# fixstars/cuda-bundle-adjustment

Hardware: AMD Instinct MI355X
Metric: edges/sec (edge-iterations/s = E x LM iterations / wall, graph resident in HBM, every timed 10-iteration run from its own perturbed start) + 10-iter LM wall-clock (contract_wall: initialize()+optimize(10) after warm-up, C++ API) on KITTI-00-shaped graph; per-iter chi2 vs g2o-faithful oracle (higher is better)
Workload: dtype f64; 1 GPU; ba_kitti00-shaped synthetic stereo graph, 10-iteration LM runs, Huber; poses=1332, landmarks=133383, edges=561116, graphs=1, parallelism=single GPU

## Files before the change

### cuda-bundle-adjustment_amd/csrc/ba_edge.hip

```cpp

#include "ba_device.hpp"

namespace cubahip
{

__device__ __forceinline__ void residual_chi2_body(const DeviceGraph& g, Scalar* parts, Scalar* per_edge, int bid, int nb)
{
	Scalar acc = 0;
	for (int e = g.e_begin + bid * 256 + threadIdx.x; e < g.e_end; e += nb * 256)
	{
		const int pe = g.e_pose[e];
		const bool stereo = (pe & STEREO_BIT) != 0;
		const int ip = pe & ~STEREO_BIT;
		const int il = g.e_lm[e];
		Scalar q[4], t[3], cam[5], Xw[3], meas[3], r[3], Xc[3];
		load_pose(g, ip, q, t, cam);
#pragma unroll
		for (int i = 0; i < 3; i++) Xw[i] = g.Xw[3 * (size_t)il + i];
		meas[0] = g.e_mu[e]; meas[1] = g.e_mv[e]; meas[2] = g.e_mr[e];
		const Scalar ee = g.e_w[e] * edge_residual(q, t, cam, Xw, meas, stereo, r, Xc);
		const int kind = stereo ? g.rk[1].kind : g.rk[0].kind;
		const Scalar delta = stereo ? g.rk[1].delta : g.rk[0].delta;
		acc += robust_rho(kind, delta, ee);
		if (per_edge) per_edge[e] = ee;
	}
	acc = wave_sum(acc);
	__shared__ Scalar part[4];
	if ((threadIdx.x & 63) == 0) part[threadIdx.x >> 6] = acc;
	__syncthreads();
	if (threadIdx.x == 0) parts[bid] = part[0] + part[1] + part[2] + part[3];
}

__global__ __launch_bounds__(256) void residual_chi2_kernel(DeviceGraph g, Scalar* parts, Scalar* per_edge)
{
	residual_chi2_body(g, parts, per_edge, blockIdx.x, gridDim.x);
}

void launch_residual_chi2(const DeviceGraph& g, Scalar* parts, Scalar* slots, Scalar* per_edge, hipStream_t st, const DevicePoseFactors* pf)
{
	const int n = g.e_end - g.e_begin;
	const int grid = n > 0 ? min((n + 255) / 256, 2048) : 0;
	if (grid > 0) hipLaunchKernelGGL(residual_chi2_kernel, dim3(grid), dim3(256), 0, st, g, parts, per_edge);
	const int nPf = pose_factor_chi2_parts(pf);
	if (nPf > 0) launch_pose_factor_chi2(g, *pf, parts + grid, st);
	launch_reduce_parts(parts, grid + nPf, slots, st);
}

__device__ __forceinline__ void edge_hplT_x(const LaneEdge& le, const Scalar* xp, Scalar c[3])
{
	const EdgeLin& L = le.lin;
	Scalar v[3];
#pragma unroll
	for (int m = 0; m < 3; m++)
	{
		Scalar s = 0;
#pragma unroll
		for (int r = 0; r < 6; r++) s += L.JP[m][r] * xp[r];
		v[m] = le.wr * s;
	}
#pragma unroll
	for (int k = 0; k < 3; k++) c[k] = L.JL[0][k] * v[0] + L.JL[1][k] * v[1] + L.JL[2][k] * v[2];
}

__device__ __forceinline__ Scalar finish_landmark(const DeviceSystem& sys, int il, const Scalar csum[3], Scalar lambda)
{
	const Scalar* ls = sys.lm_sys + 9 * (size_t)il;
	Scalar inv[6], bl[3], cl[3], xl[3];
#pragma unroll
	for (int k = 0; k < 6; k++) inv[k] = ls[k];
#pragma unroll
	for (int k = 0; k < 3; k++) { bl[k] = ls[6 + k]; cl[k] = bl[k] - csum[k]; }
	Scalar sc = 0;
#pragma unroll
	for (int i = 0; i < 3; i++)
	{
		xl[i] = inv[sym3_idx(i, 0)] * cl[0] + inv[sym3_idx(i, 1)] * cl[1] + inv[sym3_idx(i, 2)] * cl[2];
		sys.xl[3 * (size_t)il + i] = xl[i];
		sc += xl[i] * (lambda * xl[i] + bl[i]);
	}
	return sc;
}

__global__ __launch_bounds__(LIN_BLOCK) void back_substitute_kernel(DeviceGraph g, DeviceStructure st, DeviceSystem sys, Scalar lambda)
{
	__shared__ Scalar lds_all[(LIN_BLOCK / WAVE) * WAVE * 3];
	const int lane = threadIdx.x & 63;
	const int wv = threadIdx.x >> 6;
	const int wave = blockIdx.x * (LIN_BLOCK / WAVE) + wv;
	if (wave >= st.nWaves) return;
	Scalar* lds = lds_all + wv * WAVE * 3;
	const int lm0 = st.wave_lm[2 * wave], lm1 = st.wave_lm[2 * wave + 1];
	const int e0 = g.lm_ptr[lm0], e1 = g.lm_ptr[lm1];
	const int e = e0 + lane;
	const bool valid = e < e1;
	int il = lm0, seg0 = 0, seg1 = 0;
	Scalar c[3] = { 0, 0, 0 };
	if (valid)
	{
		il = g.e_lm[e];
		if (il < g.Lf)
		{
			seg0 = g.lm_ptr[il] - e0;
			seg1 = g.lm_ptr[il + 1] - e0;
			const int ip = g.e_pose[e] & ~STEREO_BIT;
			if (ip < g.Pf)
			{
				LaneEdge le;
				linearize_edge(g, e, le);
				Scalar xp[6];
#pragma unroll
				for (int r = 0; r < 6; r++) xp[r] = sys.xp[6 * (size_t)ip + r];
				edge_hplT_x(le, xp, c);
			}
		}
	}
	const bool lmFree = valid && il < g.Lf;
#pragma unroll
	for (int k = 0; k < 3; k++) lds[lane * 3 + k] = c[k];
	wave_lds_sync();
	Scalar sc = 0;
	if (lmFree && lane == seg0)
	{
		Scalar cs[3] = { 0, 0, 0 };
		for (int j = seg0; j < seg1; j++)
		{
			cs[0] += lds[j * 3 + 0]; cs[1] += lds[j * 3 + 1]; cs[2] += lds[j * 3 + 2];
		}
		sc = finish_landmark(sys, il, cs, lambda);
	}
	sc = wave_sum(sc);
	if (lane == 0) sys.parts[wave] = sc;
}

__global__ __launch_bounds__(256) void big_back_substitute_kernel(DeviceGraph g, DeviceStructure st, DeviceSystem sys, Scalar lambda)
{
	__shared__ Scalar red[4][3];
	const int il = st.big_lm[blockIdx.x];
	if (il >= g.Lf)
	{
		if (threadIdx.x == 0) sys.parts[st.nWaves + blockIdx.x] = 0;
		return;
	}
	const int e0 = g.lm_ptr[il], e1 = g.lm_ptr[il + 1];
	Scalar acc[3] = { 0, 0, 0 };
	for (int e = e0 + threadIdx.x; e < e1; e += 256)
	{
		const int ip = g.e_pose[e] & ~STEREO_BIT;
		if (ip >= g.Pf) continue;
		LaneEdge le;
		linearize_edge(g, e, le);
		Scalar xp[6], c[3];
#pragma unroll
		for (int r = 0; r < 6; r++) xp[r] = sys.xp[6 * (size_t)ip + r];
		edge_hplT_x(le, xp, c);
		acc[0] += c[0]; acc[1] += c[1]; acc[2] += c[2];
	}
#pragma unroll
	for (int k = 0; k < 3; k++) acc[k] = wave_sum(acc[k]);
	if ((threadIdx.x & 63) == 0)
#pragma unroll
		for (int k = 0; k < 3; k++) red[threadIdx.x >> 6][k] = acc[k];
	__syncthreads();
	if (threadIdx.x == 0)
	{
		Scalar cs[3];
#pragma unroll
		for (int k = 0; k < 3; k++) cs[k] = red[0][k] + red[1][k] + red[2][k] + red[3][k];
		sys.parts[st.nWaves + blockIdx.x] = finish_landmark(sys, il, cs, lambda);
	}
}

static void launch_back_substitute_kernels(const DeviceGraph& g, const DeviceStructure& st, const DeviceSystem& sys, Scalar lambda, hipStream_t s)
{
	if (st.nWaves > 0)
	{
		const int grid = (st.nWaves + (LIN_BLOCK / WAVE) - 1) / (LIN_BLOCK / WAVE);
		hipLaunchKernelGGL(back_substitute_kernel, dim3(grid), dim3(LIN_BLOCK), 0, s, g, st, sys, lambda);
	}
	if (st.nBig > 0)
		hipLaunchKernelGGL(big_back_substitute_kernel, dim3(st.nBig), dim3(256), 0, s, g, st, sys, lambda);
}

void launch_back_substitute(const DeviceGraph& g, const DeviceStructure& st, const DeviceSystem& sys, Scalar lambda, hipStream_t s)
{
	if (g.Lf <= 0) return;
	launch_back_substitute_kernels(g, st, sys, lambda, s);
	launch_reduce_parts(sys.parts, st.nWaves + st.nBig, sys.slots + NSLOT, s);
}

__device__ __forceinline__ void pose_scale_body(const DeviceGraph& g, const DeviceSystem& sys, Scalar lambda, Scalar* parts, int bid, int nb)
{
	Scalar acc = 0;
	for (int i = bid * 256 + threadIdx.x; i < g.Pf * 6; i += nb * 256)
	{
		const Scalar x = sys.xp[i];
		acc += x * (lambda * x + sys.bp[i]);
	}
	acc = wave_sum(acc);
	if ((threadIdx.x & 63) == 0) parts[bid * 4 + (threadIdx.x >> 6)] = acc;
}

__global__ __launch_bounds__(256) void pose_scale_kernel(DeviceGraph g, DeviceSystem sys, Scalar lambda, Scalar* parts)
{
	pose_scale_body(g, sys, lambda, parts, blockIdx.x, gridDim.x);
}

__device__ __forceinline__ void lm_decide(double* st, Scalar* lamOut, double* ring, int ok, double sumLm, double Fhat, double sumPose)
{
#pragma clang fp contract(off)
	const double F = st[0], lam = st[1], nu = st[2];
	const bool halt = st[3] != 0.0;
	const int trial = (int)st[4];
	const double scale = (ok ? sumLm + sumPose : 0.0) + 1e-3;
	const double rho = ok ? (F - Fhat) / scale : -1.0;
	const bool acc = !halt && rho > 0;
	double lamN = lam, nuN = nu, Fn = F, rej = st[6];
	bool haltN = halt;
	if (!halt)
	{
		if (acc)
		{
			const double t = 2 * rho - 1;
			const double a = 1 - t * t * t;
			lamN = lam * fmax(1. / 3, fmin(a, 2. / 3));
			nuN = 2; Fn = Fhat; rej = 0;
		}
		else
		{
			lamN = lam * nu; nuN = nu * 2; rej += 1;
			if (!(rho < 0) && rho <= 0) haltN = true;
			if (rej >= st[7]) haltN = true;
			if (!(rho < 0)) rej = 0;
		}
		if (!(fabs(lamN) <= 1.7e308)) haltN = true;
	}
	double* rec = ring + (size_t)(trial % LM_RING) * LM_REC;
	rec[0] = ok ? Fhat : 0.0; rec[1] = scale; rec[2] = rho; rec[3] = lamN; rec[4] = Fn; rec[5] = acc ? 1.0 : 0.0; rec[6] = haltN ? 1.0 : 0.0; rec[7] = st[8] + (double)(trial + 1);
	st[0] = Fn; st[1] = lamN; st[2] = nuN; st[3] = haltN ? 1.0 : 0.0; st[4] = (double)(trial + 1); st[5] = acc ? 1.0 : 0.0; st[6] = rej;
	lamOut[0] = (Scalar)lamN;
}

__device__ __forceinline__ void reduce_report_body(const DeviceSystem& sys, const Scalar* pA, int nA, Scalar* oA, const Scalar* pB, int nB, Scalar* oB,
	const Scalar* pC, int nC, Scalar* oC, double* lmState, Scalar* lmLam, double* lmRing)
{
	__shared__ Scalar sh[3][16];
	const Scalar vA = wave_sum(parts_thread_sum(pA, nA)), vB = wave_sum(parts_thread_sum(pB, nB)), vC = wave_sum(parts_thread_sum(pC, nC));
	if ((threadIdx.x & 63) == 0) { sh[0][threadIdx.x >> 6] = vA; sh[1][threadIdx.x >> 6] = vB; sh[2][threadIdx.x >> 6] = vC; }
	__syncthreads();
	if (threadIdx.x < 64)
	{
		const bool in = threadIdx.x < 16;
		const Scalar tA = wave_sum(in ? sh[0][threadIdx.x] : Scalar(0)), tB = wave_sum(in ? sh[1][threadIdx.x] : Scalar(0)), tC = wave_sum(in ? sh[2][threadIdx.x] : Scalar(0));
		store_slot_group(oA, tA); store_slot_group(oB, tB); store_slot_group(oC, tC);
		if (lmState && threadIdx.x == 0) lm_decide(lmState, lmLam, lmRing, 1, (double)tA, (double)tB, (double)tC);
	}
	__threadfence_system();
	asm volatile("s_waitcnt vmcnt(0) lgkmcnt(0)" ::: "memory");
	__syncthreads();
	if (threadIdx.x == 0 && sys.host_flags) publish_report(sys);
}


__global__ __launch_bounds__(1024) void reduce_report_kernel(DeviceSystem sys, const Scalar* pA, int nA, Scalar* oA, const Scalar* pB, int nB, Scalar* oB,
	const Scalar* pC, int nC, Scalar* oC, double* lmState, Scalar* lmLam, double* lmRing)
{
	reduce_report_body(sys, pA, nA, oA, pB, nB, oB, pC, nC, oC, lmState, lmLam, lmRing);
}

__global__ __launch_bounds__(1024) void reduce_report_batch_kernel(const BatchEntry* __restrict__ tab)
{
	const BatchEntry& e = tab[blockIdx.x];
	const BatchTrial& t = e.t;
	if (!t.reportOn) return;
	reduce_report_body(e.sys, t.scParts, t.nA, e.sys.slots + NSLOT, t.chiParts, t.nA, e.sys.slots, t.scaleParts, 4 * t.nScale, e.sys.slots + 3 * NSLOT, t.lmState, t.lmLam, t.lmRing);
}

__global__ __launch_bounds__(256) void landmark_scale_kernel(DeviceGraph g, DeviceSystem sys, Scalar lambda, Scalar* parts)
{
	Scalar acc = 0;
	for (int i = blockIdx.x * 256 + threadIdx.x; i < g.Lf * 3; i += gridDim.x * 256)
	{
		const Scalar x = sys.xl[i];
		acc += x * (lambda * x + sys.lm_sys[9 * (size_t)(i / 3) + 6 + (i % 3)]);
	}
	acc = wave_sum(acc);
	if ((threadIdx.x & 63) == 0) parts[blockIdx.x * 4 + (threadIdx.x >> 6)] = acc;
}

void launch_pose_scale(const DeviceGraph& g, const DeviceSystem& sys, Scalar lambda, Scalar* slots, hipStream_t s)
{
	const int grid = g.Pf > 0 ? min((g.Pf * 6 + 255) / 256, 256) : 0;
	if (grid > 0) hipLaunchKernelGGL(pose_scale_kernel, dim3(grid), dim3(256), 0, s, g, sys, lambda, sys.parts);
	launch_reduce_parts(sys.parts, grid * 4, slots, s);
}

void launch_landmark_scale(const DeviceGraph& g, const DeviceSystem& sys, Scalar lambda, Scalar* slots, hipStream_t s)
{
	const int grid = g.Lf > 0 ? min((g.Lf * 3 + 255) / 256, 1024) : 0;
	if (grid > 0) hipLaunchKernelGGL(landmark_scale_kernel, dim3(grid), dim3(256), 0, s, g, sys, lambda, sys.parts);
	launch_reduce_parts(sys.parts, grid * 4, slots, s);
}

__global__ __launch_bounds__(256) void update_state_kernel(DeviceGraph g, DeviceSystem sys, int poseBlocks)
{
	if ((int)blockIdx.x < poseBlocks)
	{
		const int i = blockIdx.x * 256 + threadIdx.x;
		if (i >= g.Pf) return;
		Scalar upd[6], q[4], t[3];
#pragma unroll
		for (int k = 0; k < 6; k++) upd[k] = sys.xp[6 * (size_t)i + k];
#pragma unroll
		for (int k = 0; k < 4; k++) q[k] = g.q[4 * (size_t)i + k];
#pragma unroll
		for (int k = 0; k < 3; k++) t[k] = g.t[3 * (size_t)i + k];
		pose_exp_update(upd, q, t);
#pragma unroll
		for (int k = 0; k < 4; k++) g.q[4 * (size_t)i + k] = q[k];
#pragma unroll
		for (int k = 0; k < 3; k++) g.t[3 * (size_t)i + k] = t[k];
		return;
	}
	const int i = (blockIdx.x - poseBlocks) * 256 + threadIdx.x;
	if (i < g.Lf * 3) g.Xw[i] += sys.xl[i];
}

void launch_update_state(const DeviceGraph& g, const DeviceSystem& sys, hipStream_t s)
{
	const int pb = (g.Pf + 255) / 256, lb = (g.Lf * 3 + 255) / 256;
	if (pb + lb > 0) hipLaunchKernelGGL(update_state_kernel, dim3(pb + lb), dim3(256), 0, s, g, sys, pb);
}

__device__ __forceinline__ Scalar finish_landmark_x(const DeviceSystem& sys, int il, const Scalar csum[3], Scalar lambda, Scalar xl[3])
{
	const Scalar* ls = sys.lm_sys + 9 * (size_t)il;
	Scalar inv[6], bl[3], cl[3];
#pragma unroll
	for (int k = 0; k < 6; k++) inv[k] = ls[k];
#pragma unroll
	for (int k = 0; k < 3; k++) { bl[k] = ls[6 + k]; cl[k] = bl[k] - csum[k]; }
	Scalar sc = 0;
#pragma unroll
	for (int i = 0; i < 3; i++)
	{
		xl[i] = inv[sym3_idx(i, 0)] * cl[0] + inv[sym3_idx(i, 1)] * cl[1] + inv[sym3_idx(i, 2)] * cl[2];
		sys.xl[3 * (size_t)il + i] = xl[i];
		sc += xl[i] * (lambda * xl[i] + bl[i]);
	}
	return sc;
}

__device__ __forceinline__ Scalar updated_edge_rho(const DeviceGraph& g, const Scalar q0[4], const Scalar t0[3], const Scalar cam[5], const Scalar upd[6], bool poseFree,
	const Scalar Xn[3], const Scalar meas[3], Scalar w, bool stereo)
{
	Scalar q[4] = { q0[0], q0[1], q0[2], q0[3] }, t[3] = { t0[0], t0[1], t0[2] }, r[3], Xc[3];
	if (poseFree) pose_exp_update(upd, q, t);
	const Scalar ee = w * edge_residual(q, t, cam, Xn, meas, stereo, r, Xc);
	return robust_rho(stereo ? g.rk[1].kind : g.rk[0].kind, stereo ? g.rk[1].delta : g.rk[0].delta, ee);
}

__device__ __forceinline__ void update_pose_rows(const DeviceGraph& g, const DeviceSystem& sys, const Scalar* __restrict__ old, int i)
{
	Scalar upd[6], q[4], t[3];
#pragma unroll
	for (int k = 0; k < 6; k++) upd[k] = sys.xp[6 * (size_t)i + k];
#pragma unroll
	for (int k = 0; k < 4; k++) q[k] = old[4 * (size_t)i + k];
#pragma unroll
	for (int k = 0; k < 3; k++) t[k] = old[4 * (size_t)g.Pt + 3 * (size_t)i + k];
	pose_exp_update(upd, q, t);
#pragma unroll
	for (int k = 0; k < 4; k++) g.q[4 * (size_t)i + k] = q[k];
#pragma unroll
	for (int k = 0; k < 3; k++) g.t[3 * (size_t)i + k] = t[k];
}

__device__ __forceinline__ void trial_tail_body(const DeviceGraph& g, const DeviceStructure& st, const DeviceSystem& sys, Scalar lambda,
	const Scalar* __restrict__ old, Scalar* __restrict__ scParts, Scalar* __restrict__ chiParts, int nLmGroups, int poseBlocks, Scalar* __restrict__ scaleParts, int nScale)
{
	lambda = launch_lambda(sys, lambda);
	if ((int)blockIdx.x >= nLmGroups)
	{
		const int b = blockIdx.x - nLmGroups;
		if (b < poseBlocks)
		{
			const int i = b * LIN_BLOCK + threadIdx.x;
			if (i < g.Pf) update_pose_rows(g, sys, old, i);
		}
		else pose_scale_body(g, sys, lambda, scaleParts, b - poseBlocks, nScale);
		return;
	}
	__shared__ Scalar lds_all[(LIN_BLOCK / WAVE) * WAVE * 3];
	__shared__ Scalar wpart[2][LIN_BLOCK / WAVE];
	const int lane = threadIdx.x & 63;
	const int wv = threadIdx.x >> 6;
	const int wave = blockIdx.x * (LIN_BLOCK / WAVE) + wv;
	const bool waveOn = wave < st.nWaves;
	Scalar* lds = lds_all + wv * WAVE * 3;
	const Scalar* qo = old; const Scalar* to = old + 4 * (size_t)g.Pt; const Scalar* Xo = old + 7 * (size_t)g.Pt;
	const int lm0 = waveOn ? st.wave_lm[2 * wave] : 0, lm1 = waveOn ? st.wave_lm[2 * wave + 1] : 0;
	const int e0 = waveOn ? g.lm_ptr[lm0] : 0, e1 = waveOn ? g.lm_ptr[lm1] : 0;
	const int e = e0 + lane;
	const bool valid = waveOn && e < e1;
	int il = lm0, ip = 0, seg0 = 0, seg1 = 0;
	bool stereo = false, poseFree = false;
	Scalar q[4] = { 0, 0, 0, 1 }, t[3] = { 0, 0, 0 }, cam[5] = { 1, 1, 0, 0, 0 }, Xw[3] = { 0, 0, 1 }, meas[3] = { 0, 0, 0 }, xp[6] = { 0, 0, 0, 0, 0, 0 }, w = 0;
	Scalar c[3] = { 0, 0, 0 };
	if (valid)
	{
		const int pe = g.e_pose[e];
		stereo = (pe & STEREO_BIT) != 0;
		ip = pe & ~STEREO_BIT;
		il = g.e_lm[e];
		poseFree = ip < g.Pf;
#pragma unroll
		for (int i = 0; i < 4; i++) q[i] = qo[4 * (size_t)ip + i];
#pragma unroll
		for (int i = 0; i < 3; i++) t[i] = to[3 * (size_t)ip + i];
#pragma unroll
		for (int i = 0; i < 5; i++) cam[i] = g.cam[5 * (size_t)ip + i];
#pragma unroll
		for (int i = 0; i < 3; i++) Xw[i] = Xo[3 * (size_t)il + i];
		meas[0] = g.e_mu[e]; meas[1] = g.e_mv[e]; meas[2] = g.e_mr[e];
		w = g.e_w[e];
		if (poseFree)
		{
#pragma unroll
			for (int r = 0; r < 6; r++) xp[r] = sys.xp[6 * (size_t)ip + r];
		}
		if (il < g.Lf)
		{
			seg0 = g.lm_ptr[il] - e0;
			seg1 = g.lm_ptr[il + 1] - e0;
			if (poseFree)
			{
				LaneEdge le;
				Scalar Xc[3];
				const Scalar ss = edge_residual(q, t, cam, Xw, meas, stereo, le.lin.r, Xc);
				le.wr = w * robust_weight(stereo ? g.rk[1].kind : g.rk[0].kind, stereo ? g.rk[1].delta : g.rk[0].delta, w * ss);
				const Rot3 R = quat_to_rot(q[0], q[1], q[2], q[3]);
				edge_jacobians(Xc, R, cam, stereo, le.lin);
				edge_hplT_x(le, xp, c);
			}
		}
	}
	const bool lmFree = valid && il < g.Lf;
#pragma unroll
	for (int k = 0; k < 3; k++) lds[lane * 3 + k] = c[k];
	wave_lds_sync();
	Scalar sc = 0, xl[3] = { 0, 0, 0 };
	if (lmFree && lane == seg0)
	{
		Scalar cs[3] = { 0, 0, 0 };
		for (int j = seg0; j < seg1; j++)
		{
			cs[0] += lds[j * 3 + 0]; cs[1] += lds[j * 3 + 1]; cs[2] += lds[j * 3 + 2];
		}
		sc = finish_landmark_x(sys, il, cs, lambda, xl);
#pragma unroll
		for (int k = 0; k < 3; k++) g.Xw[3 * (size_t)il + k] = Xw[k] + xl[k];
	}
	wave_lds_sync();
	if (lmFree && lane == seg0)
	{
#pragma unroll
		for (int k = 0; k < 3; k++) lds[lane * 3 + k] = xl[k];
	}
	wave_lds_sync();
	Scalar rho = 0;
	if (valid)
	{
		Scalar Xn[3] = { Xw[0], Xw[1], Xw[2] };
		if (lmFree)
		{
#pragma unroll
			for (int k = 0; k < 3; k++) Xn[k] = Xw[k] + lds[seg0 * 3 + k];
		}
		rho = updated_edge_rho(g, q, t, cam, xp, poseFree, Xn, meas, w, stereo);
	}
	sc = wave_sum(sc); rho = wave_sum(rho);
	if (lane == 0) { wpart[0][wv] = sc; wpart[1][wv] = rho; }
	__syncthreads();
	if (threadIdx.x == 0)
	{
		scParts[blockIdx.x] = (wpart[0][0] + wpart[0][1]) + (wpart[0][2] + wpart[0][3]);
		chiParts[blockIdx.x] = (wpart[1][0] + wpart[1][1]) + (wpart[1][2] + wpart[1][3]);
	}
}


__global__ __launch_bounds__(LIN_BLOCK) void trial_tail_kernel(DeviceGraph g, DeviceStructure st, DeviceSystem sys, Scalar lambda,
	const Scalar* __restrict__ old, Scalar* __restrict__ scParts, Scalar* __restrict__ chiParts, int nLmGroups, int poseBlocks, Scalar* __restrict__ scaleParts, int nScale)
{
	trial_tail_body(g, st, sys, lambda, old, scParts, chiParts, nLmGroups, poseBlocks, scaleParts, nScale);
}

__global__ __launch_bounds__(LIN_BLOCK) void trial_tail_batch_kernel(const BatchEntry* __restrict__ tab)
{
	const BatchEntry& e = tab[blockIdx.y];
	const BatchTrial& t = e.t;
	if (blockIdx.x >= t.tailGrid) return;
	trial_tail_body(e.g, e.st, e.sys, Scalar(-1), t.old, t.scParts, t.chiParts, t.nLm, t.poseBlocks, t.scaleParts, t.nScale);
}

__global__ __launch_bounds__(256) void big_trial_tail_kernel(DeviceGraph g, DeviceStructure st, DeviceSystem sys, Scalar lambda,
	const Scalar* __restrict__ old, Scalar* __restrict__ scParts, Scalar* __restrict__ chiParts)
{
	__shared__ Scalar red[4][3];
	__shared__ Scalar xsh[3];
	__shared__ Scalar rsh[4];
	lambda = launch_lambda(sys, lambda);
	DeviceGraph go = g;
	go.q = const_cast<Scalar*>(old); go.t = go.q + 4 * (size_t)g.Pt; go.Xw = go.q + 7 * (size_t)g.Pt;
	const int il = st.big_lm[blockIdx.x];
	const int e0 = g.lm_ptr[il], e1 = g.lm_ptr[il + 1];
	const bool lmFree = il < g.Lf;
	Scalar acc[3] = { 0, 0, 0 };
	if (lmFree)
	{
		for (int e = e0 + threadIdx.x; e < e1; e += 256)
		{
			const int ip = g.e_pose[e] & ~STEREO_BIT;
			if (ip >= g.Pf) continue;
			LaneEdge le;
			linearize_edge(go, e, le);
			Scalar xp[6], c[3];
#pragma unroll
			for (int r = 0; r < 6; r++) xp[r] = sys.xp[6 * (size_t)ip + r];
			edge_hplT_x(le, xp, c);
			acc[0] += c[0]; acc[1] += c[1]; acc[2] += c[2];
		}
	}
#pragma unroll
	for (int k = 0; k < 3; k++) acc[k] = wave_sum(acc[k]);
	if ((threadIdx.x & 63) == 0)
#pragma unroll
		for (int k = 0; k < 3; k++) red[threadIdx.x >> 6][k] = acc[k];
	__syncthreads();
	if (threadIdx.x == 0)
	{
		Scalar xl[3] = { 0, 0, 0 }, sc = 0;
		if (lmFree)
		{
			Scalar cs[3];
#pragma unroll
			for (int k = 0; k < 3; k++) cs[k] = red[0][k] + red[1][k] + red[2][k] + red[3][k];
			sc = finish_landmark_x(sys, il, cs, lambda, xl);
#pragma unroll
			for (int k = 0; k < 3; k++) g.Xw[3 * (size_t)il + k] = go.Xw[3 * (size_t)il + k] + xl[k];
		}
		scParts[blockIdx.x] = sc;
#pragma unroll
		for (int k = 0; k < 3; k++) xsh[k] = xl[k];
	}
	__syncthreads();
	Scalar Xn[3];
#pragma unroll
	for (int k = 0; k < 3; k++) Xn[k] = go.Xw[3 * (size_t)il + k] + xsh[k];
	Scalar rho = 0;
	for (int e = e0 + threadIdx.x; e < e1; e += 256)
	{
		const int pe = g.e_pose[e];
		const bool stereo = (pe & STEREO_BIT) != 0;
		const int ip = pe & ~STEREO_BIT;
		Scalar q[4], t[3], cam[5], meas[3], xp[6];
		load_pose(go, ip, q, t, cam);
		meas[0] = g.e_mu[e]; meas[1] = g.e_mv[e]; meas[2] = g.e_mr[e];
		const bool poseFree = ip < g.Pf;
#pragma unroll
		for (int r = 0; r < 6; r++) xp[r] = poseFree ? sys.xp[6 * (size_t)ip + r] : Scalar(0);
		rho += updated_edge_rho(g, q, t, cam, xp, poseFree, Xn, meas, g.e_w[e], stereo);
	}
	rho = wave_sum(rho);
	if ((threadIdx.x & 63) == 0) rsh[threadIdx.x >> 6] = rho;
	__syncthreads();
	if (threadIdx.x == 0) chiParts[blockIdx.x] = (rsh[0] + rsh[1]) + (rsh[2] + rsh[3]);
}

size_t trial_tail_parts(const DeviceGraph& g, const DeviceStructure& st, int factorParts)
{
	const size_t a = (size_t)(st.nWaves + LIN_BLOCK / WAVE - 1) / (LIN_BLOCK / WAVE) + st.nBig;
	const size_t nA = (a + 63) / 64 * 64;
	return nA + (a + factorParts + 63) / 64 * 64 + 4 * 256 + 64;
}

void launch_trial_tail_fused(const DeviceGraph& g, const DeviceStructure& st, const DeviceSystem& sys, Scalar lambda, const Scalar* old, hipStream_t s,
	const LmDevice* decide, const DevicePoseFactors* pf)
{
	const int nLm = (st.nWaves + LIN_BLOCK / WAVE - 1) / (LIN_BLOCK / WAVE);
	const int nA = nLm + st.nBig;
	const int nPf = pose_factor_chi2_parts(pf);
	Scalar* scParts = sys.parts;
	Scalar* chiParts = sys.parts + (size_t)(nA + 63) / 64 * 64;
	Scalar* scaleParts = chiParts + (size_t)(nA + nPf + 63) / 64 * 64;
	const int poseBlocks = (g.Pf + LIN_BLOCK - 1) / LIN_BLOCK;
	const int nScale = g.Pf > 0 ? min((g.Pf * 6 + 255) / 256, 256) : 0;
	if (nLm + poseBlocks + nScale > 0)
		hipLaunchKernelGGL(trial_tail_kernel, dim3(nLm + poseBlocks + nScale), dim3(LIN_BLOCK), 0, s, g, st, sys, lambda, old, scParts, chiParts, nLm, poseBlocks, scaleParts, nScale);
	if (st.nBig > 0) hipLaunchKernelGGL(big_trial_tail_kernel, dim3(st.nBig), dim3(256), 0, s, g, st, sys, lambda, old, scParts + nLm, chiParts + nLm);
	if (nPf > 0) launch_pose_factor_chi2(g, *pf, chiParts + nA, s);
	hipLaunchKernelGGL(reduce_report_kernel, dim3(1), dim3(1024), 0, s, sys, scParts, nA, sys.slots + NSLOT, chiParts, nA + nPf, sys.slots, scaleParts, 4 * nScale, sys.slots + 3 * NSLOT,
		decide ? decide->state : (double*)nullptr, decide ? decide->lam : (Scalar*)nullptr, decide ? decide->ring : (double*)nullptr);
}

void batch_fill_tail(const DeviceGraph& g, const DeviceStructure& st, const DeviceSystem& sys, const Scalar* old, const LmDevice& lm, Scalar* state, size_t stateCount, BatchTrial& t)
{
	const int nLm = (st.nWaves + LIN_BLOCK / WAVE - 1) / (LIN_BLOCK / WAVE);
	const int nA = nLm + st.nBig;
	t.scParts = sys.parts;
	t.chiParts = sys.parts + (size_t)(nA + 63) / 64 * 64;
	t.scaleParts = t.chiParts + (size_t)(nA + 63) / 64 * 64;
	t.poseBlocks = (g.Pf + LIN_BLOCK - 1) / LIN_BLOCK;
	t.nScale = g.Pf > 0 ? min((g.Pf * 6 + 255) / 256, 256) : 0;
	t.nLm = nLm; t.nA = nA; t.old = old;
	t.tailGrid = (unsigned)(nLm + t.poseBlocks + t.nScale);
	t.lmState = lm.state; t.lmLam = lm.lam; t.lmRing = lm.ring; t.reportOn = 1;
	t.state = state; t.stateCount = stateCount;
	t.restoreGrid = (unsigned)std::min<size_t>(512, (stateCount + 255) / 256);
}

__global__ void lm_decide_failed_kernel(DeviceSystem sys, double* lmState, Scalar* lmLam, double* lmRing)
{
	if (threadIdx.x != 0) return;
	lm_decide(lmState, lmLam, lmRing, 0, 0.0, 0.0, 0.0);
	__threadfence_system();
	if (sys.host_flags) publish_report(sys);
}

void launch_lm_decide_failed(const DeviceSystem& sys, const LmDevice& lm, hipStream_t s)
{
	hipLaunchKernelGGL(lm_decide_failed_kernel, dim3(1), dim3(64), 0, s, sys, lm.state, lm.lam, lm.ring);
}

__global__ __launch_bounds__(256) void restore_if_rejected_batch_kernel(const BatchEntry* __restrict__ tab)
{
	const BatchTrial& t = tab[blockIdx.y].t;
	if (blockIdx.x >= t.restoreGrid || t.lmState[5] != 0.0) return;
	const size_t stride = (size_t)t.restoreGrid * 256;
	const Scalar* __restrict__ backup = t.backupDst;
	Scalar* __restrict__ state = t.state;
	for (size_t i = (size_t)blockIdx.x * 256 + threadIdx.x; i < t.stateCount; i += stride) state[i] = backup[i];
}

__global__ __launch_bounds__(256) void restore_if_rejected_kernel(Scalar* __restrict__ state, const Scalar* __restrict__ backup, size_t count, const double* lmState)
{
	if (lmState[5] != 0.0) return;
	const size_t stride = (size_t)gridDim.x * 256;
	for (size_t i = (size_t)blockIdx.x * 256 + threadIdx.x; i < count; i += stride) state[i] = backup[i];
}

void launch_restore_if_rejected(Scalar* state, const Scalar* backup, size_t count, const LmDevice& lm, hipStream_t s)
{
	const unsigned grid = (unsigned)std::min<size_t>(512, (count + 255) / 256);
	if (grid) hipLaunchKernelGGL(restore_if_rejected_kernel, dim3(grid), dim3(256), 0, s, state, backup, count, lm.state);
}

void launch_batch_tail(const BatchEntry* tab, int n, unsigned tailGridMax, unsigned restoreGridMax, hipStream_t s)
{
	if (tailGridMax) hipLaunchKernelGGL(trial_tail_batch_kernel, dim3(tailGridMax, n), dim3(LIN_BLOCK), 0, s, tab);
	hipLaunchKernelGGL(reduce_report_batch_kernel, dim3(n), dim3(1024), 0, s, tab);
	if (restoreGridMax) hipLaunchKernelGGL(restore_if_rejected_batch_kernel, dim3(restoreGridMax, n), dim3(256), 0, s, tab);
}

}
```

### cuda-bundle-adjustment_amd/csrc/ba_kernels.hpp

```cpp
#pragma once

#include <hip/hip_runtime.h>
#include <cstdint>
#include <vector>

#include "ba_math.hpp"

namespace cubahip
{

constexpr int PCG_SETUP_POSES = 64;
constexpr int NSLOT = 16;
constexpr int WAVE = 64;
constexpr int LIN_BLOCK = 256;
constexpr int STEREO_BIT = 0x40000000;

struct DeviceGraph
{
	int Pt = 0, Pf = 0, Lt = 0, Lf = 0, E = 0;
	int e_begin = 0, e_end = 0;
	Scalar *q = nullptr, *t = nullptr, *cam = nullptr, *Xw = nullptr;
	int *e_pose = nullptr, *e_lm = nullptr;
	Scalar *e_mu = nullptr, *e_mv = nullptr, *e_mr = nullptr, *e_w = nullptr;
	int* lm_ptr = nullptr;
	RobustKernel rk[2] = { { 0, 0 }, { 0, 0 } };
};

constexpr int BP_HEAVY = 64;

struct DeviceStructure
{
	int nWaves = 0;
	int* wave_lm = nullptr;
	int nBig = 0;
	int* big_lm = nullptr;
	int nblk = 0;
	int *hsc_rowptr = nullptr, *hsc_colind = nullptr;
	int *adj_ptr = nullptr, *adj_blk = nullptr, *adj_col = nullptr;
	int2* ell = nullptr;
	int ell_m = 0, ell_over = 0;
	int* hsc_blkrow = nullptr;
	int nOd = 0;
	int nDiagProd = 0;
	int* od_blocks = nullptr;
	int inv_rows8 = 1;
	int nHeavy = 0;
	int *prod_ea = nullptr, *prod_eb = nullptr;
	const int *prod_beg = nullptr, *prod_end = nullptr, *pe_beg = nullptr, *pe_end = nullptr;
	int* prod_lm = nullptr;
	int* pe_edge = nullptr;
	int nCb = 0;
	int *cb_I = nullptr, *cb_J = nullptr, *cb_ptr = nullptr, *cb_blk = nullptr;
	Scalar *cb_wi = nullptr, *cb_wj = nullptr;
	Scalar* e_rec = nullptr;
	int mixed = 0;
};

int spmv_rows_for(int Pf);

struct DeviceSystem
{
	Scalar* hsc = nullptr;
	Scalar* bsc = nullptr;
	Scalar* bp = nullptr;
	Scalar* lm_sys = nullptr;
	Scalar* lm_inv = nullptr;
	Scalar* xp = nullptr;
	Scalar* xl = nullptr;
	Scalar* parts = nullptr;
	Scalar* slots = nullptr;
	unsigned long long* maxdiag = nullptr;
	int* fail = nullptr;
	Scalar *minv = nullptr, *r = nullptr, *z = nullptr, *p0 = nullptr, *p1 = nullptr, *ap = nullptr;
	Scalar *rz = nullptr, *pq = nullptr;
	int rzStride = 0, pqStride = 0;
	int nrz0 = 0, nrz = 0, npq = 0;
	int* done = nullptr;
	int* iters = nullptr;
	int* host_flags = nullptr;
	int* ticket = nullptr;
	int* kbase = nullptr;
	int agg = 0;
	int nc = 0;
	Scalar inv_agg = 0;
	int cl = 1;
	Scalar* acinv = nullptr;
	float* acinv32 = nullptr;
	Scalar* gj_pivots = nullptr;
	Scalar* rc = nullptr;
	Scalar* hrow = nullptr;
	int spmv_rows = 2;
	Scalar* qpart = nullptr;
	Scalar* r2 = nullptr;
	const Scalar* lam_dev = nullptr;
	int upper = 0;
	Scalar* tq = nullptr;
	int* lowpos = nullptr;
};

enum { POSE_FACTOR_KERNEL_NONE = 0, POSE_FACTOR_KERNEL_HUBER = 1, POSE_FACTOR_KERNEL_TUKEY = 2, POSE_FACTOR_KERNEL_CAUCHY = 3 };

struct DevicePriors
{
	int n = 0;
	int nPoses = 0;
	const int* pose_ptr = nullptr;
	const int* pose_id = nullptr;
	const int* pose = nullptr;
	const Scalar *qbar = nullptr, *tbar = nullptr;
	const Scalar* info = nullptr;
	Scalar* chi = nullptr;
	const int* rk_kind = nullptr;
	const Scalar* rk_delta = nullptr;
};

constexpr int REL_REC = 90;
struct DeviceRelPoses
{
	int n = 0;
	int nActive = 0;
	int nBlocks = 0;
	int nPoses = 0;
	const int *pose_i = nullptr, *pose_j = nullptr;
	const int* blk_ptr = nullptr;
	const int* blk_id = nullptr;
	const int* pose_ptr = nullptr;
	const int* pose_id = nullptr;
	const int* pose_item = nullptr;
	const Scalar *q = nullptr, *t = nullptr;
	const Scalar* info = nullptr;
	Scalar* rec = nullptr;
	Scalar* chi = nullptr;
	const int* rk_kind = nullptr;
	const Scalar* rk_delta = nullptr;
};

struct DevicePoseFactors { DevicePriors priors; DeviceRelPoses rel; };
void launch_pose_factor_linearize(const DeviceGraph& g, const DeviceStructure& st, const DeviceSystem& sys, const DevicePoseFactors& pf, int mode, hipStream_t s);
void launch_pose_factor_chi2(const DeviceGraph& g, const DevicePoseFactors& pf, Scalar* parts, hipStream_t s);
int pose_factor_chi2_parts(const DevicePoseFactors* pf);

void launch_residual_chi2(const DeviceGraph& g, Scalar* parts, Scalar* slots, Scalar* per_edge, hipStream_t st, const DevicePoseFactors* pf = nullptr);

struct BlockPassRange { int begin, end, heavy; };
void launch_linearize_dm(const DeviceGraph& g, const DeviceStructure& st, const DeviceSystem& sys, int mode, Scalar lambda, hipStream_t s,
	const Scalar* backupSrc = nullptr, Scalar* backupDst = nullptr, size_t backupCount = 0, const BlockPassRange* range = nullptr);
void launch_block_pass(const DeviceGraph& g, const DeviceStructure& st, const DeviceSystem& sys, const BlockPassRange& range, hipStream_t s);

void launch_pose_maxdiag(const DeviceGraph& g, const DeviceStructure& st, const DeviceSystem& sys, hipStream_t s);

void launch_back_substitute(const DeviceGraph& g, const DeviceStructure& st, const DeviceSystem& sys, Scalar lambda, hipStream_t s);

void launch_pose_scale(const DeviceGraph& g, const DeviceSystem& sys, Scalar lambda, Scalar* slots, hipStream_t s);
struct LmDevice;
void launch_trial_tail_fused(const DeviceGraph& g, const DeviceStructure& st, const DeviceSystem& sys, Scalar lambda, const Scalar* old, hipStream_t s,
	const LmDevice* decide = nullptr, const DevicePoseFactors* pf = nullptr);
size_t trial_tail_parts(const DeviceGraph& g, const DeviceStructure& st, int factorParts = 0);
constexpr int LM_REC = 8, LM_RING = 64;
struct LmDevice { double* state = nullptr; Scalar* lam = nullptr; double* ring = nullptr; };
void launch_lm_decide_failed(const DeviceSystem& sys, const LmDevice& lm, hipStream_t s);
void launch_restore_if_rejected(Scalar* state, const Scalar* backup, size_t count, const LmDevice& lm, hipStream_t s);
void launch_landmark_scale(const DeviceGraph& g, const DeviceSystem& sys, Scalar lambda, Scalar* slots, hipStream_t s);

void launch_update_state(const DeviceGraph& g, const DeviceSystem& sys, hipStream_t s);

void launch_pcg_setup(const DeviceGraph& g, const DeviceStructure& st, const DeviceSystem& sys, Scalar lambda, hipStream_t s);
void launch_pcg_spmv(const DeviceGraph& g, const DeviceStructure& st, const DeviceSystem& sys, int k, int maxIter, Scalar tol2, hipStream_t s);
void launch_pcg_update(const DeviceGraph& g, const DeviceStructure& st, const DeviceSystem& sys, int k, int maxIter, Scalar tol2, hipStream_t s);
Scalar* launch_coarse_setup(const DeviceGraph& g, const DeviceStructure& st, const DeviceSystem& sys, Scalar* work0, Scalar* work1, hipStream_t s, hipEvent_t assembled = nullptr);
Scalar* launch_dense_inverse(Scalar* work0, Scalar* work1, int n, Scalar* pivots, hipStream_t s);
void launch_coarse_finish(const Scalar* swept, Scalar* dst, int n, hipStream_t s);
struct GjJob { Scalar* buf[2]; Scalar* piv[2]; int n, tiles; };
void launch_coarse_assemble(const DeviceGraph& g, const DeviceStructure& st, const DeviceSystem& sys, Scalar* work0, hipStream_t s);
void launch_dense_inverse_batch(const GjJob* jobs, int m, int nMax, hipStream_t s);
void launch_pcg2_fused(const DeviceGraph& g, const DeviceSystem& sys, int k, int kOut, int maxIter, Scalar tol2, int doUpdate, hipStream_t s);
int spmv_upper_grid(int Pf);
int pcg_rows_max_aggregate();
int pcg_rows_entries_per_thread(const DeviceSystem& sys);
void launch_build_lowpos(const DeviceGraph& g, const DeviceStructure& st, int* lowpos, hipStream_t s);
void launch_pcg_upper_iteration(const DeviceGraph& g, const DeviceStructure& st, const DeviceSystem& sys, int k, int maxIter, Scalar tol2, hipStream_t s, int which = 7);
void launch_pcg_advance(const DeviceSystem& sys, int n, hipStream_t s, Scalar tol2 = Scalar(-1));
void launch_coarse_to_fp32(const Scalar* swept, float* dst, int n, hipStream_t s);
void launch_pcg_iteration(const DeviceGraph& g, const DeviceStructure& st, const DeviceSystem& sys, int k, int maxIter, Scalar tol2, hipStream_t s);

struct LmDevice;
struct BatchTrial
{
	unsigned lmGroups = 0, lmGrid = 0; const Scalar* backupSrc = nullptr; Scalar* backupDst = nullptr; size_t backupCount = 0;
	int poseGroups = 0; unsigned schurGrid = 0;
	int nSetup = 0; size_t expandTotal = 0; unsigned nExpand = 0; const Scalar* copySrc = nullptr; Scalar* copyDst = nullptr; size_t copyPairs = 0; unsigned setupGrid = 0;
	int fusedOn = 0;
	const Scalar* old = nullptr; Scalar *scParts = nullptr, *chiParts = nullptr, *scaleParts = nullptr; int nLm = 0, poseBlocks = 0, nScale = 0; unsigned tailGrid = 0; int nA = 0;
	double* lmState = nullptr; Scalar* lmLam = nullptr; double* lmRing = nullptr; int reportOn = 0;
	Scalar* state = nullptr; size_t stateCount = 0; unsigned restoreGrid = 0;
};
struct BatchEntry
{
	DeviceGraph g; DeviceStructure st; DeviceSystem sys;
	int maxIter = 0;
	int gridSpmv = 0;
	BatchTrial t;
};
void batch_fill_linearize(const DeviceGraph& g, const DeviceStructure& st, const Scalar* backupSrc, Scalar* backupDst, size_t backupCount, BatchTrial& t);
void launch_batch_linearize(const BatchEntry* tab, int n, unsigned lmGridMax, unsigned schurGridMax, bool mixed, hipStream_t s);
void batch_fill_setup(const DeviceGraph& g, const DeviceStructure& st, const DeviceSystem& sys, const Scalar* copySrc, Scalar* copyDst, size_t copyCount, BatchTrial& t);
void launch_batch_setup(const BatchEntry* tab, int n, unsigned gridMax, hipStream_t s);
void launch_batch_first_precond(const BatchEntry* tab, int n, const DeviceSystem& sys0, int ncMax, size_t ldsMax, Scalar tol2, hipStream_t s);
void batch_fill_tail(const DeviceGraph& g, const DeviceStructure& st, const DeviceSystem& sys, const Scalar* old, const LmDevice& lm, Scalar* state, size_t stateCount, BatchTrial& t);
void launch_batch_tail(const BatchEntry* tab, int n, unsigned tailGridMax, unsigned restoreGridMax, hipStream_t s);
int batch_kernel_class(const DeviceGraph& g, const DeviceSystem& sys);
size_t batch_pcg2_lds_bytes(const DeviceSystem& sys);
void launch_pcg_batch_iteration(const BatchEntry* tab, int n, const DeviceGraph& g0, const DeviceSystem& sys0, int gridSpmvMax, int ncMax, size_t ldsMax, int k, Scalar tol2, hipStream_t s);
void launch_pcg_batch_advance(const BatchEntry* tab, int n, int iters, hipStream_t s, Scalar tol2);

hipError_t graph_add_pcg_chunk(hipGraph_t graph, const DeviceGraph& g, const DeviceStructure& st, const DeviceSystem& sys, int chunk, int maxIter, Scalar tol2, int report);

void launch_hsc_expand(const DeviceGraph& g, const DeviceStructure& st, const DeviceSystem& sys, hipStream_t s);
void launch_pcg_setup_expand(const DeviceGraph& g, const DeviceStructure& st, const DeviceSystem& sys, Scalar lambda, hipStream_t s,
	const Scalar* copySrc = nullptr, Scalar* copyDst = nullptr, size_t copyCount = 0);

constexpr int SC_T = 32;
constexpr int SC_TP = 5;
constexpr int SC_TT = SC_T * SC_T;

struct SparseCholPlan
{
	int Pf = 0, T = 0, nTiles = 0, nLevels = 0, slack = 0;
	std::vector<int> posOfSeg, segOfPos;
	std::vector<int> colPtr;
	std::vector<int> rowIdx, colOfTile;
	std::vector<int> gPtr;
	std::vector<int> gather;
	std::vector<int> wgRec;
	std::vector<int> lvlPtr, lvlTiles;
	std::vector<int> lvlColPtr, lvlCols;
	std::vector<int> blkTile;
	long long entries = 0;
	size_t tileBytes() const { return sizeof(Scalar) * (size_t)SC_TT * ((size_t)2 * nTiles + 1); }
	double secondsEstimate() const;
};
bool sparse_chol_plan(int Pf, const int* rowptr, const int* colind, int slack, size_t maxTiles, SparseCholPlan& out);

struct SparseChol
{
	Scalar* tiles = nullptr;
	Scalar* tilesT = nullptr;
	Scalar* y = nullptr;
	Scalar* rinv = nullptr;
	const int *colPtr = nullptr, *rowIdx = nullptr, *colOfTile = nullptr, *gPtr = nullptr, *gather = nullptr;
	const int *wgRec = nullptr, *lvlCols = nullptr, *blkTile = nullptr, *posOfSeg = nullptr;
	int* fail = nullptr;
	int T = 0, Pf = 0, nTiles = 0;
};
void launch_sparse_chol_fill(const DeviceStructure& st, const DeviceSystem& sys, const SparseChol& d, hipStream_t s);
void launch_sparse_chol_solve(const SparseChol& d, const SparseCholPlan& plan, Scalar* x, hipStream_t s);
void launch_sparse_chol_factor(const SparseChol& d, const SparseCholPlan& plan, hipStream_t s);

struct SelInvPlan
{
	int nLevels = 0;
	std::vector<int> stepPtr;
	std::vector<int> offRec;
	std::vector<int> colStepPtr, cols;
	std::vector<int> gather;
	long long products = 0;
	size_t sigmaBytes() const;
	int nTiles = 0;
};
bool selinv_plan(const SparseCholPlan& p, SelInvPlan& out);

struct SelInv
{
	Scalar* sigma = nullptr;
	const int *offRec = nullptr, *gather = nullptr, *cols = nullptr;
};
void launch_selinv(const SparseChol& d, const SparseCholPlan& plan, const SelInvPlan& sp, const SelInv& v, hipStream_t s);
void launch_selinv_extract(const DeviceStructure& st, const SparseChol& d, const SelInv& v, Scalar* pose_cov, Scalar* blk_cov, int Pf, hipStream_t s);
void launch_landmark_covariance(const DeviceGraph& g, const DeviceStructure& st, const DeviceSystem& sys, const SparseChol& d, const SelInv& v,
	Scalar* w_scratch, Scalar* lm_cov, hipStream_t s);

void launch_diag_inverse(const SparseChol& d, hipStream_t s);
void launch_edge_w(const DeviceGraph& g, Scalar* W, hipStream_t s);

struct PairRequest
{
	int nBlocks = 0;
	std::vector<int> rhsPtr, rhsPos;
	std::vector<int> leftPtr, leftPos;
	std::vector<int> poseRec;
	std::vector<int> lmRec;
	std::vector<int> pairRec;
};
void pair_pack(const SparseCholPlan& p, int n, const int* kindA, const int* idxA, const int* kindB, const int* idxB,
	const std::vector<int>& lmPtr, const std::vector<int>& ePose, PairRequest& rq);
struct PairPlan
{
	int b0 = 0, b1 = 0, nLevels = 0, T = 0;
	std::vector<int> fwdPtr, fwdCols;
	std::vector<int> bwdPtr, bwdCols;
	std::vector<int> slotPtr, slotCols;
	std::vector<int> slotOf;
	std::vector<int> fLvlPtr, fRec;
	std::vector<int> fGather;
	std::vector<int> bLvlPtr, bRec;
	std::vector<int> bGather;
	size_t slots() const { return slotCols.size(); }
};
size_t pair_block_slots(const SparseCholPlan& p, const PairRequest& rq, int b);
bool pair_plan(const SparseCholPlan& p, const PairRequest& rq, int b0, int b1, PairPlan& out);
struct PairDev
{
	Scalar* X = nullptr;
	const int *fRec = nullptr, *fGather = nullptr, *bRec = nullptr, *bGather = nullptr, *slotOf = nullptr, *rhsPos = nullptr;
	int T = 0;
};

void launch_collect_eval(const DeviceSystem& sys, Scalar* out3, hipStream_t s);

void launch_pcg_report(const DeviceSystem& sys, hipStream_t s);

}
```

### cuda-bundle-adjustment_amd/csrc/ba_linearize.hip

```cpp

#include "ba_device.hpp"

namespace cubahip
{

constexpr int REC = 8;

__device__ __forceinline__ double tag_encode(int tag, double) { return __longlong_as_double((long long)tag); }
__device__ __forceinline__ float tag_encode(int tag, float) { return __int_as_float(tag); }
__device__ __forceinline__ int tag_decode(double v) { return (int)__double_as_longlong(v); }
__device__ __forceinline__ int tag_decode(float v) { return __float_as_int(v); }
__device__ __forceinline__ bool sign_flag(double v) { return __double_as_longlong(v) < 0; }
__device__ __forceinline__ bool sign_flag(float v) { return __float_as_int(v) < 0; }
__device__ __forceinline__ double abs_value(double v) { return __builtin_fabs(v); }
__device__ __forceinline__ float abs_value(float v) { return __builtin_fabsf(v); }

template <typename ET>
__device__ __forceinline__ void write_record(Scalar* base, size_t e, const Scalar Xc[3], Scalar wr, const Scalar r[3], int il, bool stereo)
{
	ET* rec = reinterpret_cast<ET*>(base) + REC * e;
	const ET w = (ET)wr;
	rec[0] = (ET)Xc[0]; rec[1] = (ET)Xc[1]; rec[2] = (ET)Xc[2]; rec[3] = stereo ? -w : w;
	rec[4] = (ET)r[0]; rec[5] = (ET)r[1]; rec[6] = (ET)r[2];
	rec[7] = tag_encode(il, ET());
}

template <typename ET>
__device__ __forceinline__ void load_pose_as(const DeviceGraph& g, int ip, ET q[4], ET cam[5])
{
#pragma unroll
	for (int i = 0; i < 4; i++) q[i] = (ET)g.q[4 * (size_t)ip + i];
#pragma unroll
	for (int i = 0; i < 5; i++) cam[i] = (ET)g.cam[5 * (size_t)ip + i];
}

template <int MODE, typename ET>
__device__ __forceinline__ void lm_pass_body(const DeviceGraph& g, const DeviceStructure& st, const DeviceSystem& sys, Scalar lambda,
	unsigned nLmGroups, const Scalar* __restrict__ backupSrc, Scalar* __restrict__ backupDst, size_t backupCount, unsigned gridX)
{
	__shared__ Scalar lds_all[(LIN_BLOCK / WAVE) * WAVE * 9];
	if (blockIdx.x >= nLmGroups)
	{
		const size_t stride = (size_t)(gridX - nLmGroups) * LIN_BLOCK;
		for (size_t i = (size_t)(blockIdx.x - nLmGroups) * LIN_BLOCK + threadIdx.x; i < backupCount; i += stride) backupDst[i] = backupSrc[i];
		return;
	}
	lambda = launch_lambda(sys, lambda);
	const int lane = threadIdx.x & 63;
	const int wv = threadIdx.x >> 6;
	const int wave = blockIdx.x * (LIN_BLOCK / WAVE) + wv;
	if (wave >= st.nWaves) return;
	Scalar* lds = lds_all + wv * WAVE * 9;
	const int lm0 = st.wave_lm[2 * wave], lm1 = st.wave_lm[2 * wave + 1];
	const int e0 = g.lm_ptr[lm0], e1 = g.lm_ptr[lm1];
	const int e = e0 + lane;
	const bool valid = e < e1;
	int il = lm0, seg0 = 0, seg1 = 0;
	Scalar h[9] = { 0, 0, 0, 0, 0, 0, 0, 0, 0 };
	if (valid)
	{
		const int pe = g.e_pose[e];
		const bool stereo = (pe & STEREO_BIT) != 0;
		const int ip = pe & ~STEREO_BIT;
		il = g.e_lm[e];
		Scalar q[4], t[3], cam[5], Xw[3], meas[3], Xc[3];
		EdgeLin L;
		load_pose(g, ip, q, t, cam);
#pragma unroll
		for (int i = 0; i < 3; i++) Xw[i] = g.Xw[3 * (size_t)il + i];
		meas[0] = g.e_mu[e]; meas[1] = g.e_mv[e]; meas[2] = g.e_mr[e];
		const Scalar w = g.e_w[e];
		const Scalar ss = edge_residual(q, t, cam, Xw, meas, stereo, L.r, Xc);
		const int kind = stereo ? g.rk[1].kind : g.rk[0].kind;
		const Scalar delta = stereo ? g.rk[1].delta : g.rk[0].delta;
		const Scalar wr = w * robust_weight(kind, delta, w * ss);
		write_record<ET>(st.e_rec, (size_t)e, Xc, wr, L.r, il, stereo);
		if (il < g.Lf)
		{
			const Rot3 R = quat_to_rot(q[0], q[1], q[2], q[3]);
			edge_jacobians(Xc, R, cam, stereo, L);
#pragma unroll
			for (int i = 0; i < 3; i++)
			{
#pragma unroll
				for (int j = i; j < 3; j++)
					h[sym3_idx(i, j)] = wr * (L.JL[0][i] * L.JL[0][j] + L.JL[1][i] * L.JL[1][j] + L.JL[2][i] * L.JL[2][j]);
				h[6 + i] = wr * (L.JL[0][i] * L.r[0] + L.JL[1][i] * L.r[1] + L.JL[2][i] * L.r[2]);
			}
			seg0 = g.lm_ptr[il] - e0;
			seg1 = g.lm_ptr[il + 1] - e0;
		}
	}
#pragma unroll
	for (int k = 0; k < 9; k++) lds[lane * 9 + k] = h[k];
	wave_lds_sync();
	const bool head = valid && il < g.Lf && lane == seg0;
	Scalar m = 0;
	if (head)
	{
		Scalar H[9] = { 0, 0, 0, 0, 0, 0, 0, 0, 0 };
		for (int j = seg0; j < seg1; j++)
#pragma unroll
			for (int k = 0; k < 9; k++) H[k] += lds[j * 9 + k];
		Scalar* ls = sys.lm_sys + 9 * (size_t)il;
		if (MODE == 0)
		{
#pragma unroll
			for (int k = 0; k < 9; k++) ls[k] = H[k];
			m = fmax(H[0], fmax(H[3], H[5]));
		}
		else
		{
			Scalar inv[6];
			H[0] += lambda; H[3] += lambda; H[5] += lambda;
			sym3_inverse(H, inv);
#pragma unroll
			for (int k = 0; k < 6; k++) ls[k] = inv[k];
			if (st.inv_rows8)
			{
				Scalar* li = sys.lm_inv + 8 * (size_t)il;
#pragma unroll
				for (int k = 0; k < 6; k++) li[k] = inv[k];
				li[6] = 0; li[7] = 0;
			}
#pragma unroll
			for (int k = 0; k < 3; k++) ls[6 + k] = H[6 + k];
		}
	}
	if (MODE == 0)
	{
		m = wave_max(m);
		if (lane == 0) atomic_max_nonneg(sys.maxdiag + (wave & 63), m);
	}
}


template <int MODE, typename ET>
__global__ __launch_bounds__(LIN_BLOCK) void lm_pass_kernel(DeviceGraph g, DeviceStructure st, DeviceSystem sys, Scalar lambda,
	unsigned nLmGroups, const Scalar* __restrict__ backupSrc, Scalar* __restrict__ backupDst, size_t backupCount)
{
	lm_pass_body<MODE, ET>(g, st, sys, lambda, nLmGroups, backupSrc, backupDst, backupCount, gridDim.x);
}

template <typename ET>
__global__ __launch_bounds__(LIN_BLOCK) void lm_pass_batch_kernel(const BatchEntry* __restrict__ tab)
{
	const BatchEntry& e = tab[blockIdx.y];
	if (blockIdx.x >= e.t.lmGrid) return;
	lm_pass_body<1, ET>(e.g, e.st, e.sys, Scalar(-1), e.t.lmGroups, e.t.backupSrc, e.t.backupDst, e.t.backupCount, e.t.lmGrid);
}

template <int MODE, typename ET>
__global__ __launch_bounds__(256) void big_lm_pass_kernel(DeviceGraph g, DeviceStructure st, DeviceSystem sys, Scalar lambda)
{
	__shared__ Scalar red[4][9];
	lambda = launch_lambda(sys, lambda);
	const int il = st.big_lm[blockIdx.x];
	const int e0 = g.lm_ptr[il], e1 = g.lm_ptr[il + 1];
	Scalar acc[9] = { 0, 0, 0, 0, 0, 0, 0, 0, 0 };
	for (int e = e0 + threadIdx.x; e < e1; e += 256)
	{
		LaneEdge le;
		linearize_edge(g, e, le);
		Scalar q[4], t[3], cam[5], Xw[3], Xc[3];
		load_pose(g, le.ip, q, t, cam);
#pragma unroll
		for (int i = 0; i < 3; i++) Xw[i] = g.Xw[3 * (size_t)il + i];
		quat_rotate(q, Xw, Xc);
		Xc[0] += t[0]; Xc[1] += t[1]; Xc[2] += t[2];
		write_record<ET>(st.e_rec, (size_t)e, Xc, le.wr, le.lin.r, il, le.stereo);
		if (il < g.Lf)
		{
			const EdgeLin& L = le.lin;
#pragma unroll
			for (int i = 0; i < 3; i++)
			{
#pragma unroll
				for (int j = i; j < 3; j++)
					acc[sym3_idx(i, j)] += le.wr * (L.JL[0][i] * L.JL[0][j] + L.JL[1][i] * L.JL[1][j] + L.JL[2][i] * L.JL[2][j]);
				acc[6 + i] += le.wr * (L.JL[0][i] * L.r[0] + L.JL[1][i] * L.r[1] + L.JL[2][i] * L.r[2]);
			}
		}
	}
#pragma unroll
	for (int k = 0; k < 9; k++) acc[k] = wave_sum(acc[k]);
	if ((threadIdx.x & 63) == 0)
#pragma unroll
		for (int k = 0; k < 9; k++) red[threadIdx.x >> 6][k] = acc[k];
	__syncthreads();
	if (threadIdx.x == 0 && il < g.Lf)
	{
		Scalar H[9];
#pragma unroll
		for (int k = 0; k < 9; k++) H[k] = red[0][k] + red[1][k] + red[2][k] + red[3][k];
		Scalar* ls = sys.lm_sys + 9 * (size_t)il;
		if (MODE == 0)
		{
#pragma unroll
			for (int k = 0; k < 9; k++) ls[k] = H[k];
			atomic_max_nonneg(sys.maxdiag, fmax(H[0], fmax(H[3], H[5])));
		}
		else
		{
			Scalar inv[6];
			H[0] += lambda; H[3] += lambda; H[5] += lambda;
			sym3_inverse(H, inv);
#pragma unroll
			for (int k = 0; k < 6; k++) ls[k] = inv[k];
			if (st.inv_rows8)
			{
				Scalar* li = sys.lm_inv + 8 * (size_t)il;
#pragma unroll
				for (int k = 0; k < 6; k++) li[k] = inv[k];
				li[6] = 0; li[7] = 0;
			}
#pragma unroll
			for (int k = 0; k < 3; k++) ls[6 + k] = H[6 + k];
		}
	}
}

template <typename ET>
struct CameraFrameEdge { ET X[3]; ET k00, k02, k11, k12, k22; ET d00, d02, d11, d12, d22; ET w; bool stereo; };

template <typename ET>
__device__ __forceinline__ void camera_frame_edge(const ET* rec, const ET cam[5], CameraFrameEdge<ET>& c)
{
	const ET X = rec[0], Y = rec[1], Z = rec[2], ws = rec[3];
	c.stereo = sign_flag(ws);
	c.w = abs_value(ws);
	c.X[0] = X; c.X[1] = Y; c.X[2] = Z;
	const ET invZ = 1 / Z, invZZ = invZ * invZ;
	c.d00 = -cam[0] * invZ; c.d02 = cam[0] * X * invZZ; c.d11 = -cam[1] * invZ; c.d12 = cam[1] * Y * invZZ;
	c.d22 = c.stereo ? c.d02 - cam[4] * invZZ : ET(0);
	c.k00 = c.w * (c.stereo ? 2 * c.d00 * c.d00 : c.d00 * c.d00);
	c.k02 = c.w * (c.d00 * c.d02 + (c.stereo ? c.d00 * c.d22 : ET(0)));
	c.k11 = c.w * c.d11 * c.d11; c.k12 = c.w * c.d11 * c.d12;
	c.k22 = c.w * (c.d02 * c.d02 + c.d12 * c.d12 + c.d22 * c.d22);
}

template <typename ET>
__device__ __forceinline__ void camera_frame_m(const CameraFrameEdge<ET>& c, const Rot3T<ET>& R, ET (&M)[3][3])
{
#pragma unroll
	for (int j = 0; j < 3; j++)
	{
		M[0][j] = c.k00 * R.m[0][j] + c.k02 * R.m[2][j];
		M[1][j] = c.k11 * R.m[1][j] + c.k12 * R.m[2][j];
		M[2][j] = c.k02 * R.m[0][j] + c.k12 * R.m[1][j] + c.k22 * R.m[2][j];
	}
}

template <int MODE, typename ET>
__device__ __forceinline__ void pose_pass_body(const DeviceGraph& g, const DeviceStructure& st, const DeviceSystem& sys, int bid)
{
	const int lane = threadIdx.x & 63;
	const int ip = bid * 4 + (threadIdx.x >> 6);
	if (ip >= g.Pf) return;
	ET q[4], cam[5];
	load_pose_as<ET>(g, ip, q, cam);
	const Rot3T<ET> R = quat_to_rot(q[0], q[1], q[2], q[3]);
	Scalar acc[33];
#pragma unroll
	for (int k = 0; k < 33; k++) acc[k] = 0;
	const int p1 = st.pe_end[ip];
	for (int p = st.pe_beg[ip] + lane; p < p1; p += 64)
	{
		const ET* rec = reinterpret_cast<const ET*>(st.e_rec) + REC * (size_t)st.pe_edge[p];
		CameraFrameEdge<ET> c;
		camera_frame_edge<ET>(rec, cam, c);
		const ET r0 = rec[4], r1 = rec[5], r2 = c.stereo ? rec[6] : ET(0);
		const int il = tag_decode(rec[7]);
		ET S[6] = { c.k00, 0, c.k02, c.k11, c.k12, c.k22 };
		ET v[3] = { c.w * c.d00 * (r0 + r2), c.w * c.d11 * r1, c.w * (c.d02 * r0 + c.d12 * r1 + c.d22 * r2) };
		ET vs[3] = { v[0], v[1], v[2] };
		if (MODE == 1 && il < g.Lf)
		{
			const Scalar* ls = sys.lm_sys + 9 * (size_t)il;
			ET M[3][3], P[3][3], inv[6], bl[3];
#pragma unroll
			for (int k = 0; k < 6; k++) inv[k] = (ET)ls[k];
#pragma unroll
			for (int k = 0; k < 3; k++) bl[k] = (ET)ls[6 + k];
			camera_frame_m<ET>(c, R, M);
#pragma unroll
			for (int i = 0; i < 3; i++)
#pragma unroll
				for (int k = 0; k < 3; k++)
					P[i][k] = M[i][0] * inv[sym3_idx(0, k)] + M[i][1] * inv[sym3_idx(1, k)] + M[i][2] * inv[sym3_idx(2, k)];
#pragma unroll
			for (int i = 0; i < 3; i++)
			{
#pragma unroll
				for (int j = i; j < 3; j++)
					S[sym3_idx(i, j)] -= P[i][0] * M[j][0] + P[i][1] * M[j][1] + P[i][2] * M[j][2];
				vs[i] -= P[i][0] * bl[0] + P[i][1] * bl[1] + P[i][2] * bl[2];
			}
		}
		const ET X = c.X[0], Y = c.X[1], Z = c.X[2];
		ET U[3][3];
#pragma unroll
		for (int j = 0; j < 3; j++)
		{
			const ET s0 = S[sym3_idx(0, j)], s1 = S[sym3_idx(1, j)], s2 = S[sym3_idx(2, j)];
			U[0][j] = Y * s2 - Z * s1;
			U[1][j] = Z * s0 - X * s2;
			U[2][j] = X * s1 - Y * s0;
		}
#pragma unroll
		for (int i = 0; i < 3; i++)
		{
			const ET t[3] = { Y * U[i][2] - Z * U[i][1], Z * U[i][0] - X * U[i][2], X * U[i][1] - Y * U[i][0] };
#pragma unroll
			for (int j = i; j < 3; j++) acc[j * (j + 1) / 2 + i] += (Scalar)t[j];
#pragma unroll
			for (int j = 0; j < 3; j++) acc[(3 + j) * (4 + j) / 2 + i] += (Scalar)U[i][j];
#pragma unroll
			for (int j = i; j < 3; j++) acc[(3 + j) * (4 + j) / 2 + 3 + i] += (Scalar)S[sym3_idx(i, j)];
		}
		acc[21] += (Scalar)(Y * v[2] - Z * v[1]); acc[22] += (Scalar)(Z * v[0] - X * v[2]); acc[23] += (Scalar)(X * v[1] - Y * v[0]);
		acc[24] += (Scalar)v[0]; acc[25] += (Scalar)v[1]; acc[26] += (Scalar)v[2];
		if (MODE == 1)
		{
			acc[27] += (Scalar)(Y * vs[2] - Z * vs[1]); acc[28] += (Scalar)(Z * vs[0] - X * vs[2]); acc[29] += (Scalar)(X * vs[1] - Y * vs[0]);
			acc[30] += (Scalar)vs[0]; acc[31] += (Scalar)vs[1]; acc[32] += (Scalar)vs[2];
		}
	}
#pragma unroll
	for (int k = 0; k < 33; k++) acc[k] = wave_sum(acc[k]);
	if (lane == 0)
	{
		Scalar* blk = sys.hsc + 36 * (size_t)st.hsc_rowptr[ip];
#pragma unroll
		for (int c = 0; c < 6; c++)
		{
#pragma unroll
			for (int r = 0; r <= c; r++) blk[c * 6 + r] = acc[c * (c + 1) / 2 + r];
			sys.bp[6 * (size_t)ip + c] = acc[21 + c];
			if (MODE == 1) sys.bsc[6 * (size_t)ip + c] = acc[27 + c];
		}
	}
}

constexpr int BP_GROUP = 16;

template <int MODE, typename ET>
__global__ __launch_bounds__(256) void pose_pass_kernel(DeviceGraph g, DeviceStructure st, DeviceSystem sys)
{
	pose_pass_body<MODE, ET>(g, st, sys, blockIdx.x);
}

template <typename ET>
struct ProductOperand { ET X[3]; ET M[3][3]; };

template <typename ET>
__device__ __forceinline__ void product_operand(const ET* rec, const Rot3T<ET>& R, const ET cam[5], ProductOperand<ET>& o)
{
	CameraFrameEdge<ET> c;
	camera_frame_edge<ET>(rec, cam, c);
	o.X[0] = c.X[0]; o.X[1] = c.X[1]; o.X[2] = c.X[2];
	camera_frame_m<ET>(c, R, o.M);
}

template <typename ET>
__device__ __forceinline__ void product_accumulate(const ProductOperand<ET>& A, const ProductOperand<ET>& B, const ET inv[6], ET (&T)[6][6])
{
	ET P[3][3], W[3][6];
#pragma unroll
	for (int i = 0; i < 3; i++)
#pragma unroll
		for (int k = 0; k < 3; k++)
			P[i][k] = A.M[i][0] * inv[sym3_idx(0, k)] + A.M[i][1] * inv[sym3_idx(1, k)] + A.M[i][2] * inv[sym3_idx(2, k)];
#pragma unroll
	for (int i = 0; i < 3; i++)
	{
#pragma unroll
		for (int j = 0; j < 3; j++) W[i][3 + j] = P[i][0] * B.M[j][0] + P[i][1] * B.M[j][1] + P[i][2] * B.M[j][2];
		W[i][0] = B.X[1] * W[i][5] - B.X[2] * W[i][4];
		W[i][1] = B.X[2] * W[i][3] - B.X[0] * W[i][5];
		W[i][2] = B.X[0] * W[i][4] - B.X[1] * W[i][3];
	}
#pragma unroll
	for (int c = 0; c < 6; c++)
	{
		T[0][c] += A.X[1] * W[2][c] - A.X[2] * W[1][c];
		T[1][c] += A.X[2] * W[0][c] - A.X[0] * W[2][c];
		T[2][c] += A.X[0] * W[1][c] - A.X[1] * W[0][c];
		T[3][c] += W[0][c]; T[4][c] += W[1][c]; T[5][c] += W[2][c];
	}
}

template <typename ET, int GROUP>
__device__ __forceinline__ void block_pass_group(const DeviceGraph& g, const DeviceStructure& st, const DeviceSystem& sys, int grp, int gl)
{
	const int blk0 = grp >= 0 ? st.od_blocks[grp] : -1;
	const bool on = blk0 >= 0;
	const int blk = on ? blk0 : 0;
	const int a = on ? st.hsc_blkrow[blk] : 0, b = on ? st.hsc_colind[blk] : 0;
	ET qa[4], cama[5], qb[4], camb[5];
	load_pose_as<ET>(g, a, qa, cama);
	load_pose_as<ET>(g, b, qb, camb);
	const Rot3T<ET> Ra = quat_to_rot(qa[0], qa[1], qa[2], qa[3]);
	const Rot3T<ET> Rb = quat_to_rot(qb[0], qb[1], qb[2], qb[3]);
	ET T[6][6];
#pragma unroll
	for (int r = 0; r < 6; r++)
#pragma unroll
		for (int c = 0; c < 6; c++) T[r][c] = 0;
	const ET* recs = reinterpret_cast<const ET*>(st.e_rec);
	const int p1 = on ? st.prod_end[blk] : 0;
	for (int p = (on ? st.prod_beg[blk] : 0) + gl; p < p1; p += GROUP)
	{
		const ET* ra = recs + REC * (size_t)st.prod_ea[p];
		const ET* rb = recs + REC * (size_t)st.prod_eb[p];
		const Scalar* li = st.inv_rows8 ? sys.lm_inv + 8 * (size_t)st.prod_lm[p] : sys.lm_sys + 9 * (size_t)st.prod_lm[p];
		ET inv[6];
#pragma unroll
		for (int k = 0; k < 6; k++) inv[k] = (ET)li[k];
		ProductOperand<ET> A, B;
		product_operand<ET>(ra, Ra, cama, A);
		product_operand<ET>(rb, Rb, camb, B);
		product_accumulate<ET>(A, B, inv, T);
	}
	Scalar Ts[6][6];
#pragma unroll
	for (int r = 0; r < 6; r++)
#pragma unroll
		for (int c = 0; c < 6; c++)
		{
			Scalar v = (Scalar)T[r][c];
			if (GROUP == 64) v = wave_sum(v);
			else { v += __shfl_xor(v, 1); v += __shfl_xor(v, 2); v += __shfl_xor(v, 4); v += __shfl_xor(v, 8); }
			Ts[r][c] = v;
		}
	if (!on) return;
	Scalar* dst = sys.hsc + 36 * (size_t)blk;
	if (a != b)
	{
#pragma unroll
		for (int c = 0; c < 6; c++)
#pragma unroll
			for (int r = 0; r < 6; r++)
				if (GROUP == 64 ? (c * 6 + r) == gl : (c * 6 + r) % GROUP == gl) dst[c * 6 + r] = -Ts[r][c];
	}
	else if (gl == 0)
	{
#pragma unroll
		for (int c = 0; c < 6; c++)
#pragma unroll
			for (int r = 0; r <= c; r++) dst[c * 6 + r] -= Ts[r][c] + Ts[c][r];
	}
}

__host__ __device__ __forceinline__ int block_pass_heavy_groups(int nHeavy) { return (nHeavy + 3) / 4; }
__host__ __device__ __forceinline__ int block_pass_groups(int nOd, int nHeavy) { return block_pass_heavy_groups(nHeavy) + ((nOd - nHeavy) * BP_GROUP + 255) / 256; }

template <typename ET>
__device__ __forceinline__ void block_pass_body(const DeviceGraph& g, const DeviceStructure& st, const DeviceSystem& sys, int bid)
{
	const int nh = block_pass_heavy_groups(st.nHeavy);
	if (bid < nh)
	{
		const int grp = bid * 4 + (threadIdx.x >> 6);
		block_pass_group<ET, 64>(g, st, sys, grp < st.nHeavy ? grp : -1, threadIdx.x & 63);
	}
	else
	{
		const int grp = st.nHeavy + ((bid - nh) * 256 + threadIdx.x) / BP_GROUP;
		block_pass_group<ET, BP_GROUP>(g, st, sys, grp < st.nOd ? grp : -1, threadIdx.x & (BP_GROUP - 1));
	}
}

template <typename ET>
__global__ __launch_bounds__(256) void block_pass_kernel(DeviceGraph g, DeviceStructure st, DeviceSystem sys)
{
	block_pass_body<ET>(g, st, sys, blockIdx.x);
}

template <typename ET>
__global__ __launch_bounds__(256) void schur_pass_kernel(DeviceGraph g, DeviceStructure st, DeviceSystem sys, int nPoseGroups)
{
	if ((int)blockIdx.x < nPoseGroups) pose_pass_body<1, ET>(g, st, sys, blockIdx.x);
	else block_pass_body<ET>(g, st, sys, blockIdx.x - nPoseGroups);
}

template <typename ET>
__global__ __launch_bounds__(256) void schur_pass_batch_kernel(const BatchEntry* __restrict__ tab)
{
	const BatchEntry& e = tab[blockIdx.y];
	if (blockIdx.x >= e.t.schurGrid) return;
	if ((int)blockIdx.x < e.t.poseGroups) pose_pass_body<1, ET>(e.g, e.st, e.sys, blockIdx.x);
	else block_pass_body<ET>(e.g, e.st, e.sys, blockIdx.x - e.t.poseGroups);
}

static DeviceStructure block_pass_view(const DeviceStructure& st, const BlockPassRange& r)
{
	DeviceStructure v = st;
	v.od_blocks = st.od_blocks + r.begin; v.nOd = r.end - r.begin; v.nHeavy = r.heavy;
	return v;
}

template <typename ET>
static void launch_linearize_dm_t(const DeviceGraph& g, const DeviceStructure& stAll, const DeviceSystem& sys, int mode, Scalar lambda, hipStream_t s,
	const Scalar* backupSrc, Scalar* backupDst, size_t backupCount, const BlockPassRange* range)
{
	const DeviceStructure st = range ? block_pass_view(stAll, *range) : stAll;
	if (st.nWaves > 0)
	{
		const unsigned grid = (st.nWaves + (LIN_BLOCK / WAVE) - 1) / (LIN_BLOCK / WAVE);
		const unsigned nCopy = backupSrc ? (unsigned)std::min<size_t>(512, (backupCount + LIN_BLOCK - 1) / LIN_BLOCK) : 0;
		if (mode == 0) hipLaunchKernelGGL((lm_pass_kernel<0, ET>), dim3(grid + nCopy), dim3(LIN_BLOCK), 0, s, g, st, sys, lambda, grid, backupSrc, backupDst, backupCount);
		else hipLaunchKernelGGL((lm_pass_kernel<1, ET>), dim3(grid + nCopy), dim3(LIN_BLOCK), 0, s, g, st, sys, lambda, grid, backupSrc, backupDst, backupCount);
	}
	else if (backupSrc && backupCount)
		(void)hipMemcpyAsync(backupDst, backupSrc, backupCount * sizeof(Scalar), hipMemcpyDeviceToDevice, s);
	if (st.nBig > 0)
	{
		if (mode == 0) hipLaunchKernelGGL((big_lm_pass_kernel<0, ET>), dim3(st.nBig), dim3(256), 0, s, g, st, sys, lambda);
		else hipLaunchKernelGGL((big_lm_pass_kernel<1, ET>), dim3(st.nBig), dim3(256), 0, s, g, st, sys, lambda);
	}
	const int nbp = block_pass_groups(st.nOd, st.nHeavy);
	if (mode == 1 && g.Pf > 0 && st.nOd > 0 && st.nDiagProd == 0)
	{
		const int np = (g.Pf + 3) / 4;
		hipLaunchKernelGGL((schur_pass_kernel<ET>), dim3(np + nbp), dim3(256), 0, s, g, st, sys, np);
		return;
	}
	if (g.Pf > 0)
	{
		if (mode == 0) hipLaunchKernelGGL((pose_pass_kernel<0, ET>), dim3((g.Pf + 3) / 4), dim3(256), 0, s, g, st, sys);
		else hipLaunchKernelGGL((pose_pass_kernel<1, ET>), dim3((g.Pf + 3) / 4), dim3(256), 0, s, g, st, sys);
	}
	if (mode == 1 && st.nOd > 0)
		hipLaunchKernelGGL((block_pass_kernel<ET>), dim3(nbp), dim3(256), 0, s, g, st, sys);
}

void launch_linearize_dm(const DeviceGraph& g, const DeviceStructure& st, const DeviceSystem& sys, int mode, Scalar lambda, hipStream_t s,
	const Scalar* backupSrc, Scalar* backupDst, size_t backupCount, const BlockPassRange* range)
{
	if (st.mixed && sizeof(Scalar) == 8) launch_linearize_dm_t<float>(g, st, sys, mode, lambda, s, backupSrc, backupDst, backupCount, range);
	else launch_linearize_dm_t<Scalar>(g, st, sys, mode, lambda, s, backupSrc, backupDst, backupCount, range);
}

void batch_fill_linearize(const DeviceGraph& g, const DeviceStructure& st, const Scalar* backupSrc, Scalar* backupDst, size_t backupCount, BatchTrial& t)
{
	t.lmGroups = (st.nWaves + (LIN_BLOCK / WAVE) - 1) / (LIN_BLOCK / WAVE);
	const unsigned nCopy = backupSrc ? (unsigned)std::min<size_t>(512, (backupCount + LIN_BLOCK - 1) / LIN_BLOCK) : 0;
	t.lmGrid = t.lmGroups + nCopy;
	t.backupSrc = backupSrc; t.backupDst = backupDst; t.backupCount = backupCount;
	t.poseGroups = (g.Pf + 3) / 4;
	t.schurGrid = (unsigned)(t.poseGroups + block_pass_groups(st.nOd, st.nHeavy));
}

void launch_batch_linearize(const BatchEntry* tab, int n, unsigned lmGridMax, unsigned schurGridMax, bool mixed, hipStream_t s)
{
	if (mixed && sizeof(Scalar) == 8)
	{
		hipLaunchKernelGGL((lm_pass_batch_kernel<float>), dim3(lmGridMax, n), dim3(LIN_BLOCK), 0, s, tab);
		hipLaunchKernelGGL((schur_pass_batch_kernel<float>), dim3(schurGridMax, n), dim3(256), 0, s, tab);
	}
	else
	{
		hipLaunchKernelGGL((lm_pass_batch_kernel<Scalar>), dim3(lmGridMax, n), dim3(LIN_BLOCK), 0, s, tab);
		hipLaunchKernelGGL((schur_pass_batch_kernel<Scalar>), dim3(schurGridMax, n), dim3(256), 0, s, tab);
	}
}

void launch_block_pass(const DeviceGraph& g, const DeviceStructure& stAll, const DeviceSystem& sys, const BlockPassRange& range, hipStream_t s)
{
	if (range.end <= range.begin) return;
	const DeviceStructure st = block_pass_view(stAll, range);
	const int nbp = block_pass_groups(st.nOd, st.nHeavy);
	if (st.mixed && sizeof(Scalar) == 8) hipLaunchKernelGGL((block_pass_kernel<float>), dim3(nbp), dim3(256), 0, s, g, st, sys);
	else hipLaunchKernelGGL((block_pass_kernel<Scalar>), dim3(nbp), dim3(256), 0, s, g, st, sys);
}

__global__ __launch_bounds__(256) void pose_maxdiag_kernel(DeviceGraph g, DeviceStructure st, DeviceSystem sys)
{
	const int i = blockIdx.x * 256 + threadIdx.x;
	Scalar m = 0;
	if (i < g.Pf * 6)
	{
		const int p = i / 6, k = i % 6;
		m = sys.hsc[36 * (size_t)st.hsc_rowptr[p] + k * 7];
	}
	m = wave_max(m);
	if ((threadIdx.x & 63) == 0) atomic_max_nonneg(sys.maxdiag, m);
}

void launch_pose_maxdiag(const DeviceGraph& g, const DeviceStructure& st, const DeviceSystem& sys, hipStream_t s)
{
	if (g.Pf <= 0) return;
	hipLaunchKernelGGL(pose_maxdiag_kernel, dim3((g.Pf * 6 + 255) / 256), dim3(256), 0, s, g, st, sys);
}

}
```

### cuda-bundle-adjustment_amd/csrc/ba_lm.hip

```cpp
#include "ba_solver.hpp"

using namespace cubahip;

void cuba_hip_solver::graphWorker()
{
	(void)hipSetDevice(device);
	std::unique_lock<std::mutex> lk(gb.m);
	for (;;)
	{
		gb.cv.wait(lk, [&] { return gb.stop || !gb.jobs.empty() || !gb.trash.empty(); });
		if (gb.stop) return;
		if (gb.jobs.empty())
		{
			std::vector<hipGraphExec_t> t; t.swap(gb.trash);
			gb.busy = true;
			lk.unlock();
			for (hipGraphExec_t e : t) (void)hipGraphExecDestroy(e);
			lk.lock();
			gb.busy = false;
			gb.cv.notify_all();
			continue;
		}
		GraphJob j = gb.jobs.front(); gb.jobs.pop_front();
		gb.busy = true;
		lk.unlock();
		const auto t0 = Clock::now();
		hipGraph_t graph = nullptr; hipGraphExec_t exec = nullptr;
		bool ok = hipGraphCreate(&graph, 0) == hipSuccess && graph_add_pcg_chunk(graph, j.g, j.st, j.sys, j.chunk, j.maxIter, j.tol2, 1) == hipSuccess &&
			hipGraphInstantiate(&exec, graph, nullptr, nullptr, 0) == hipSuccess;
		if (graph) (void)hipGraphDestroy(graph);
		if (!ok) (void)hipGetLastError();
		const double dt = std::chrono::duration<double>(Clock::now() - t0).count();
		lk.lock();
		gb.busy = false;
		if (ok && j.gen == gb.gen) { gb.ready[std::make_pair(j.chunk, j.acinv)] = exec; gb.builds++; gb.seconds.store(gb.seconds.load() + dt); }
		else if (exec) (void)hipGraphExecDestroy(exec);
		gb.cv.notify_all();
	}
}

hipGraphExec_t cuba_hip_solver::pcgGraphIfReady(int chunk, int maxIter, Scalar tol2)
{
	if (pcgGraphTol2 != tol2 || pcgGraphMaxIter != maxIter) { dropPcgGraph(); pcgGraphTol2 = tol2; pcgGraphMaxIter = maxIter; }
	const auto key = std::make_pair(chunk, (const Scalar*)sys.acinv);
	auto it = pcgGraphs.find(key);
	if (it != pcgGraphs.end()) return it->second;
	std::lock_guard<std::mutex> lk(gb.m);
	for (auto& kv : gb.ready) pcgGraphs[kv.first] = kv.second;
	gb.ready.clear();
	it = pcgGraphs.find(key);
	if (it != pcgGraphs.end()) return it->second;
	if (!gb.requested.count(key))
	{
		gb.requested[key] = 1;
		gb.jobs.push_back(GraphJob{ chunk, (const Scalar*)sys.acinv, g, st, sys, maxIter, tol2, gb.gen });
		if (!gb.th.joinable()) gb.th = std::thread([this] { graphWorker(); });
		gb.cv.notify_all();
	}
	return nullptr;
}

void cuba_hip_solver::dropPcgGraph()
{
	{
		std::lock_guard<std::mutex> lk(gb.m);
		gb.gen++;
		gb.jobs.clear(); gb.requested.clear();
		const bool offload = gb.th.joinable() && !gb.stop;
		for (auto& kv : gb.ready) { if (offload) gb.trash.push_back(kv.second); else (void)hipGraphExecDestroy(kv.second); }
		gb.ready.clear();
		for (auto& kv : pcgGraphs) { if (offload) gb.trash.push_back(kv.second); else (void)hipGraphExecDestroy(kv.second); }
		if (offload && !gb.trash.empty()) gb.cv.notify_all();
	}
	pcgGraphs.clear();
	batchRequests.clear();
	graphsOrderedFor = nullptr;
}

void cuba_hip_solver::ensureOverlapObjects()
{
	if (gjStream) return;
	int prioLow = 0, prioHigh = 0;
	HIP_TRY(hipDeviceGetStreamPriorityRange(&prioLow, &prioHigh));
	HIP_TRY(hipStreamCreateWithPriority(&gjStream, hipStreamNonBlocking, prioLow));
	HIP_TRY(hipEventCreateWithFlags(&evSetup, hipEventDisableTiming));
	HIP_TRY(hipEventCreateWithFlags(&evAssembled, hipEventDisableTiming));
	HIP_TRY(hipEventCreateWithFlags(&evInverse, hipEventDisableTiming));
	HIP_TRY(hipEventCreateWithFlags(&evFirstInv, hipEventDisableTiming));
	HIP_TRY(hipEventRecord(evFirstInv, gjStream));
}

void cuba_hip_solver::waitReport()
{
	volatile int* flags = (volatile int*)((char*)h_pinned + 1024);
	{
		const auto t0 = Clock::now();
		for (long spins = 0; flags[3] != expectedTicket; spins++)
			if ((spins & 0xfff) == 0xfff && std::chrono::duration<double>(Clock::now() - t0).count() > 2.0) break;
		if (flags[3] == expectedTicket)
		{
			std::atomic_thread_fence(std::memory_order_acquire);
			return;
		}
	}
	sync();
	std::atomic_thread_fence(std::memory_order_acquire);
	expectedTicket = flags[3];
}

void cuba_hip_solver::downloadAsDouble(const Scalar* dsrc, double* hdst, size_t n)
{
	if (!n) return;
	if (sizeof(Scalar) == sizeof(double))
	{
		HIP_TRY(hipMemcpyAsync(hdst, dsrc, n * sizeof(double), hipMemcpyDeviceToHost, stream));
		sync();
		return;
	}
	std::vector<Scalar> tmp(n);
	HIP_TRY(hipMemcpyAsync(tmp.data(), dsrc, n * sizeof(Scalar), hipMemcpyDeviceToHost, stream));
	sync();
	for (size_t i = 0; i < n; i++) hdst[i] = (double)tmp[i];
}

void cuba_hip_solver::uploadFromDouble(Scalar* ddst, const double* hsrc, size_t n)
{
	if (!n) return;
	std::vector<Scalar> tmp(hsrc, hsrc + n);
	HIP_TRY(hipMemcpyAsync(ddst, tmp.data(), n * sizeof(Scalar), hipMemcpyHostToDevice, stream));
	sync();
}

double cuba_hip_solver::computeErrors()
{
	need();
	StageTimer tm(this, 2);
	launch_residual_chi2(g, d_parts.data(), slotsDev, nullptr, stream, poseFactors());
	return readSlots(0);
}

void cuba_hip_solver::linearize(int mode, double lam, bool withBackup)
{
	waitAssembled();
	const bool parts = mode == 1 && !redParts.empty();
	launch_linearize_dm(g, st, sys, mode, lam, stream, withBackup ? d_state.data() : nullptr, d_backup.data(), d_state.size(), parts ? &redParts[0].od : nullptr);
	if (parts && !partsByCaller)
		for (size_t c = 1; c < redParts.size(); c++) launch_block_pass(g, st, sys, redParts[c].od, stream);
	if (poseFactors()) launch_pose_factor_linearize(g, st, sys, pf, mode, stream);
}

void cuba_hip_solver::schurPart(int part, size_t ranges[4])
{
	need();
	if (part < 0 || part >= schurParts()) throw ArgError{ "cuba_hip_schur_part: no such part" };
	if (part == 0)
	{
		StageTimer tm(this, 4);
		zeroReduced();
		partsByCaller = true;
		try { linearize(1, lambda, false); } catch (...) { partsByCaller = false; throw; }
		partsByCaller = false;
	}
	else
	{
		StageTimer tm(this, 4);
		launch_block_pass(g, st, sys, redParts[part].od, stream);
	}
	const size_t nblk = (size_t)st.nblk;
	ranges[0] = redParts.empty() ? 0 : 36 * redParts[part].blkBegin;
	ranges[1] = redParts.empty() ? 36 * nblk : 36 * (redParts[part].blkEnd - redParts[part].blkBegin);
	ranges[2] = part == 0 ? 36 * nblk : 0;
	ranges[3] = part == 0 ? d_red.size() - 36 * nblk : 0;
}

void cuba_hip_solver::assemble()
{
	need();
	StageTimer tm(this, 3);
	zeroReduced(true);
	d_maxdiag.zero(stream);
	linearize(0, 0.0);
}

void cuba_hip_solver::maxDiagonalParts(double* posePart, double* lmPart)
{
	need();
	const double* hD = (const double*)hostStage();
	HIP_TRY(hipMemcpyAsync(hostStage(), d_maxdiag.data(), 8 * 64, hipMemcpyDeviceToHost, stream));
	sync();
	double v = 0;
	for (int i = 0; i < 64; i++) v = std::max(v, hD[i]);
	*lmPart = v;
	d_maxdiag.zero(stream);
	launch_pose_maxdiag(g, st, sys, stream);
	HIP_TRY(hipMemcpyAsync(hostStage(), d_maxdiag.data(), 8 * 64, hipMemcpyDeviceToHost, stream));
	sync();
	v = 0;
	for (int i = 0; i < 64; i++) v = std::max(v, hD[i]);
	*posePart = v;
}

void cuba_hip_solver::scaleParts(double lam, double* posePart, double* lmPart)
{
	need();
	launch_pose_scale(g, sys, lam, slotsDev + 3 * NSLOT, stream);
	launch_landmark_scale(g, sys, lam, slotsDev + 2 * NSLOT, stream);
	sync();
	double a = 0, b = 0;
	for (int i = 0; i < NSLOT; i++) { b += slot(2 * NSLOT + i); a += slot(3 * NSLOT + i); }
	*posePart = a; *lmPart = b;
}

double cuba_hip_solver::maxDiagonal()
{
	need();
	StageTimer tm(this, 3);
	zeroReduced(true);
	d_maxdiag.zero(stream);
	linearize(0, 0.0);
	launch_pose_maxdiag(g, st, sys, stream);
	HIP_TRY(hipMemcpyAsync(hostStage(), d_maxdiag.data(), 8 * 64, hipMemcpyDeviceToHost, stream));
	sync();
	double v = 0;
	for (int i = 0; i < 64; i++) v = std::max(v, ((const double*)hostStage())[i]);
	return v;
}

void cuba_hip_solver::schur(bool withBackup)
{
	need();
	StageTimer tm(this, 4);
	zeroReduced();
	linearize(1, lambda, withBackup);
}

bool cuba_hip_solver::solveReduced() { return retryWithFp64Inverse(solveReducedOnce()); }

bool cuba_hip_solver::retryWithFp64Inverse(bool ok)
{
	if (ok || !lastSolveBrokeDown || lastFailCode != 2 || !fp32Inverse() || sys.agg <= 0) return ok;
	precondFp32 = false; sys.acinv32 = nullptr;
	dropPcgGraph();
	coarseValid = false; firstInvValid = false; firstInvPending = false;
	cntFp32Fallbacks++;
	if (std::getenv("CUBA_HIP_DEBUG")) std::fprintf(stderr, "[cuba_hip] PCG broke down with the fp32-stored coarse inverse: repeating the solve with fp64 storage\n");
	const int64_t directBefore = cntDirect;
	const bool ok2 = solveReducedOnce();
	if (!ok2 || cntDirect != directBefore)
	{
		precondFp32 = true; sys.acinv32 = d_coarse32[0].data();
		dropPcgGraph();
		coarseValid = false; firstInvValid = false; firstInvPending = false;
	}
	return ok2;
}

int cuba_hip_solver::pcgBudget(int maxIter) const
{
	const int it = directAfter > 0 ? directAfter : std::min(384, std::max(128, Pf / 4));
	return std::min(maxIter, std::max(4, it / 4 * 4));
}

bool cuba_hip_solver::ensureDirectPlan()
{
	if (directPlanValid) return !directRefused;
	const auto t0 = Clock::now();
	ensureHostPattern();
	if (!sparse_chol_plan(Pf, h_rowptr.data(), h_colind.data(), directSlack, (size_t)std::max(1, directMaxTiles), directPlan))
	{
		directPlanValid = true; directRefused = true;
		char buf[200];
		std::snprintf(buf, sizeof buf, "exact reduced solve unavailable: the factor of the %d-pose reduced matrix needs more than direct_max_tiles = %d tiles", Pf, directMaxTiles);
		lastError = buf;
		return false;
	}
	const SparseCholPlan& p = directPlan;
	{
		size_t freeB = 0, totalB = 0;
		const size_t have = sizeof(Scalar) * (d_scTiles.size() + d_scTilesT.size());
		if (hipMemGetInfo(&freeB, &totalB) == hipSuccess && p.tileBytes() > have && p.tileBytes() - have > freeB)
		{
			directPlanValid = true; directRefused = true;
			char buf[200];
			std::snprintf(buf, sizeof buf, "exact reduced solve unavailable: the factor of the %d-pose reduced matrix needs %.1f MB, %.1f MB of device memory are free",
				Pf, p.tileBytes() / 1e6, freeB / 1e6);
			lastError = buf;
			return false;
		}
		(void)hipGetLastError();
	}
	std::vector<int> ints;
	auto put = [&](const std::vector<int>& v) { const size_t o = ints.size(); ints.insert(ints.end(), v.begin(), v.end()); while (ints.size() % 4) ints.push_back(0); return o; };
	const size_t oColPtr = put(p.colPtr), oRowIdx = put(p.rowIdx), oColOf = put(p.colOfTile), oGPtr = put(p.gPtr), oGather = put(p.gather),
		oWgRec = put(p.wgRec), oLvlCols = put(p.lvlCols), oBlkTile = put(p.blkTile), oPos = put(p.posOfSeg);
	d_scInts.upload(ints, stream);
	d_scTiles.resize((size_t)SC_TT * ((size_t)p.nTiles + 1)); d_scTilesT.resize((size_t)SC_TT * std::max(1, p.nTiles));
	d_scY.resize((size_t)SC_T * p.T); d_scRinv.resize((size_t)SC_T * p.T); d_scFail.resize(1);
	sync();
	SparseChol& d = directDev;
	d.tiles = d_scTiles.data(); d.tilesT = d_scTilesT.data(); d.y = d_scY.data(); d.rinv = d_scRinv.data(); d.fail = d_scFail.data();
	const int* base = d_scInts.data();
	d.colPtr = base + oColPtr; d.rowIdx = base + oRowIdx; d.colOfTile = base + oColOf; d.gPtr = base + oGPtr; d.gather = base + oGather;
	d.wgRec = base + oWgRec; d.lvlCols = base + oLvlCols; d.blkTile = base + oBlkTile; d.posOfSeg = base + oPos;
	d.T = p.T; d.Pf = Pf; d.nTiles = p.nTiles;
	directPlanValid = true;
	directPlanBuilds++;
	directPlanSeconds = std::chrono::duration<double>(Clock::now() - t0).count();
	if (std::getenv("CUBA_HIP_DEBUG"))
		std::fprintf(stderr, "[cuba_hip] exact reduced solve, symbolic phase: %d poses -> %d tile columns, %d tiles (%.1f MB), %d levels, %lld tile products, slack %d, %.2f ms\n",
			Pf, p.T, p.nTiles, p.tileBytes() / 1e6, p.nLevels, p.entries, p.slack, 1e3 * directPlanSeconds);
	return true;
}

bool cuba_hip_solver::solveDirect()
{
	if (!ensureDirectPlan()) return false;
	const auto t0 = Clock::now();
	launch_sparse_chol_fill(st, sys, directDev, stream);
	launch_sparse_chol_solve(directDev, directPlan, sys.xp, stream);
	int* hflag = (int*)hostStage();
	HIP_TRY(hipMemcpyAsync(hflag, directDev.fail, sizeof(int), hipMemcpyDeviceToHost, stream));
	sync();
	directSeconds = std::chrono::duration<double>(Clock::now() - t0).count();
	cntDirect++;
	directSticky = true;
	coarseValid = false;
	if (std::getenv("CUBA_HIP_DEBUG"))
		std::fprintf(stderr, "[cuba_hip] exact reduced solve: %d unknowns, %.3f ms, lambda %.3e%s\n", 6 * Pf, 1e3 * directSeconds, lambda, *hflag ? " -- NON-POSITIVE PIVOT" : "");
	if (*hflag)
	{
		cntDirectFailed++;
		lastError = "exact reduced solve: non-positive pivot (the damped reduced matrix is not positive definite)";
		return false;
	}
	return true;
}

bool cuba_hip_solver::solveBegin(SolveCtx& sc)
{
	lastSolveBrokeDown = false;
	need();
	if (Pf == 0) { sc.result = true; return true; }
	const int maxIter = sc.maxIter = maxIterAlloc;
	const Scalar tol2 = sc.tol2 = pcgTol * pcgTol;
	if (failDirty) { d_fail.zero(stream); failDirty = false; }
	const bool twoLevel = sc.twoLevel = sys.agg > 0;
	const bool direct = sc.direct = directUsable();
	if (direct && (directSticky || directAlways))
	{
		launch_pcg_setup(g, st, sys, lambda, stream);
		failDirty = true;
		coarseValid = false;
		if (pcgHistory.size() >= 65536) pcgHistory.erase(pcgHistory.begin(), pcgHistory.begin() + 32768);
		pcgHistory.push_back(0);
		sc.result = solveDirect();
		return true;
	}
	sc.budget = direct && !acceptUnconverged ? pcgBudget(maxIter) : maxIter;
	const size_t invCount = (size_t)36 * sys.cl * sys.cl * sys.nc * sys.nc;
	bool takeInverse = false;
	if (twoLevel && coarseValid && pendingInv >= 0)
	{
		HIP_TRY(hipStreamWaitEvent(stream, evInverse, 0));
		takeInverse = true; pendingInv = -1;
	}
	const bool deferred = sc.deferLaunch && twoLevel && coarseValid;
	{
		const bool f32 = fp32Inverse();
		const Scalar* cpSrc = !takeInverse ? nullptr : f32 ? reinterpret_cast<const Scalar*>(d_coarse32[1].data()) : d_coarse[0].data();
		Scalar* cpDst = f32 ? reinterpret_cast<Scalar*>(d_coarse32[0].data()) : d_coarse[2].data();
		const size_t cpCount = f32 ? inv32Count() / 2 : invCount;
		if (deferred) { sc.deferred = true; sc.copySrc = cpSrc; sc.copyDst = cpDst; sc.copyCount = cpCount; }
		else launch_pcg_setup_expand(g, st, sys, lambda, stream, cpSrc, cpDst, cpCount);
	}
	if (twoLevel)
	{
		const int gjSteps = (6 * sys.cl * sys.nc + 31) / 32, first = gjSteps & 1;
		{
			ensureOverlapObjects();
			const size_t invBytes = sizeof(Scalar) * (size_t)36 * sys.cl * sys.cl * sys.nc * sys.nc;
			if (!coarseValid && heuristics && firstInvValid)
			{
				HIP_TRY(hipStreamWaitEvent(stream, evFirstInv, 0));
				if (fp32Inverse()) HIP_TRY(hipMemcpyAsync(d_coarse32[0].data(), d_firstInv32.data(), inv32Count() * sizeof(float), hipMemcpyDeviceToDevice, stream));
				else HIP_TRY(hipMemcpyAsync(d_coarse[2].data(), d_firstInv.data(), invBytes, hipMemcpyDeviceToDevice, stream));
				pendingInv = -1;
				coarseValid = true; sideAge = overlapPeriod(); firstInvPending = true;
			}
			else if (!coarseValid)
			{
				drainInversion();
				(void)launch_coarse_setup(g, st, sys, d_coarse[first].data(), d_coarse[1 - first].data(), stream);
				if (fp32Inverse()) launch_coarse_to_fp32(d_coarse[0].data(), d_coarse32[0].data(), 6 * sys.cl * sys.nc, stream);
				else launch_coarse_finish(d_coarse[0].data(), d_coarse[2].data(), 6 * sys.cl * sys.nc, stream);
				coarseValid = true; cntCoarseRefresh++; cntCoarseInline++; sideAge = 0;
				if (heuristics)
				{
					if (fp32Inverse()) d_firstInv32.resize(inv32Count()); else d_firstInv.resize(invCount);
					sideAge = overlapPeriod(); firstInvPending = true;
				}
			}
			sys.acinv = d_coarse[2].data();
			const bool regular = ++sideAge >= overlapPeriod();
			if (regular) sideAge = 0;
			if (regular)
			{
				if (!deferred) HIP_TRY(hipEventRecord(evSetup, stream));
				if (sc.deferCoarse)
				{
					sc.deferCoarse->push_back(CoarseJob{ this, first, firstInvPending, !deferred });
					if (firstInvPending) { firstInvPending = false; firstInvValid = true; }
				}
				else
				{
					HIP_TRY(hipStreamWaitEvent(gjStream, evSetup, 0));
					(void)launch_coarse_setup(g, st, sys, d_coarse[first].data(), d_coarse[1 - first].data(), gjStream, evAssembled);
					if (fp32Inverse()) launch_coarse_to_fp32(d_coarse[0].data(), d_coarse32[1].data(), 6 * sys.cl * sys.nc, gjStream);
					else launch_coarse_finish(d_coarse[0].data(), d_coarse[0].data(), 6 * sys.cl * sys.nc, gjStream);
					if (firstInvPending)
					{
						if (fp32Inverse()) HIP_TRY(hipMemcpyAsync(d_firstInv32.data(), d_coarse32[1].data(), inv32Count() * sizeof(float), hipMemcpyDeviceToDevice, gjStream));
						else HIP_TRY(hipMemcpyAsync(d_firstInv.data(), d_coarse[0].data(), invBytes, hipMemcpyDeviceToDevice, gjStream));
						HIP_TRY(hipEventRecord(evFirstInv, gjStream));
						firstInvPending = false; firstInvValid = true;
					}
					HIP_TRY(hipEventRecord(evInverse, gjStream));
				}
				pendingInv = 0;
				assemblePending = true; cntCoarseRefresh++;
			}
		}
		if (!deferred) launch_pcg2_fused(g, sys, 0, 0, maxIter, tol2, 0, stream);
	}
	const bool graphs = sc.graphs = useGraph && !sc.batched && g_liveHandles.load(std::memory_order_relaxed) <= 1;
	if (useGraph && !graphs && (!pcgGraphs.empty() || graphsOrderedFor)) dropPcgGraph();
	if (graphs && pcgGraphs.empty() && graphsOrderedFor != (const void*)sys.acinv)
	{
		for (int c = 64; c >= 4; c /= 2) (void)pcgGraphIfReady(c, maxIter, tol2);
		graphsOrderedFor = (const void*)sys.acinv;
	}
	sc.hInts = (volatile int*)((char*)h_pinned + 1024);
	sc.tSolve0 = Clock::now();
	int predicted = 32;
	if (runIters.size() >= 2)
	{
		const double a = runIters[runIters.size() - 2], b = runIters.back();
		const double lin = b + std::max(0.0, b - a), geo = b * std::min(1.35, std::max(1.0, b / std::max(1.0, a)));
		predicted = (int)std::max(lin, geo) + 1;
	}
	else if (runIters.size() == 1) predicted = (int)(1.35 * runIters[0]) + 2;
	else if (firstSolveIters > 0) predicted = firstSolveIters + 1;
	{
		const size_t k = runIters.size();
		if (heuristics && k < prevRunIters.size() && std::equal(runIters.begin(), runIters.end(), prevRunIters.begin())) predicted = prevRunIters[k];
	}
	sc.predicted = predicted;
	return false;
}

bool cuba_hip_solver::solveBrokeDown(SolveCtx& sc)
{
	lastSolveBrokeDown = true; lastFailCode = sc.hInts[0];
	cntPcgIters += sc.hInts[1]; coarseValid = false; firstInvValid = false; firstInvPending = false; failDirty = true;
	if (sc.direct && lastFailCode != 1 && !(lastFailCode == 2 && fp32Inverse() && sc.twoLevel))
	{
		if (pcgHistory.size() >= 65536) pcgHistory.erase(pcgHistory.begin(), pcgHistory.begin() + 32768);
		pcgHistory.push_back(-sc.hInts[1]);
		d_fail.zero(stream); failDirty = false;
		return solveDirect();
	}
	return false;
}

bool cuba_hip_solver::solveReducedOnce()
{
	StageTimer tm(this, 6);
	SolveCtx sc;
	if (solveBegin(sc)) return sc.result;
	const int maxIter = sc.maxIter; const Scalar tol2 = sc.tol2; const bool graphs = sc.graphs; const int predicted = sc.predicted;
	bool converged = false;
	int k0 = 0, looks = 0, eagerIters = 0;
	int target = (predicted + 3) / 4 * 4;
	while (k0 < sc.budget && !converged)
	{
		int todo = std::max(4, std::min(target, sc.budget) - k0);
		while (todo > 0)
		{
			int c = graphs ? 256 : todo;
			for (; graphs && c > 4 && c > todo; c >>= 1) {}
			if (graphs && todo > c && todo % 4 == 0 && todo <= 128 && pcgGraphMaxIter == maxIter && pcgGraphTol2 == tol2)
			{
				if ((pcgGraphs.count(std::make_pair(todo, (const Scalar*)sys.acinv)) || ++batchRequests[todo] >= 2) && pcgGraphIfReady(todo, maxIter, tol2)) c = todo;
			}
			hipGraphExec_t exec = graphs ? pcgGraphIfReady(c, maxIter, tol2) : nullptr;
			if (exec) { HIP_TRY(hipGraphLaunch(exec, stream)); noteReport(); }
			else
			{
				for (int k = 0; k < c; k++) enqueuePcgIteration(k, maxIter, tol2, stream);
				launch_pcg_advance(sys, c, stream, tol2); noteReport();
				if (graphs) { eagerIters += c; cntPcgPlain += c; }
			}
			k0 += c; todo -= c;
		}
		waitReport();
		if (sc.hInts[0] != 0) return solveBrokeDown(sc);
		if (sc.hInts[2] != 0 || sc.hInts[1] < std::min(k0, maxIter)) converged = true;
		target = k0 + ((looks == 0 && k0 <= 96) ? 4 : std::max(8, k0 / 8 / 4 * 4));
		looks++; cntPcgLooks++; cntHostLooks++;
	}
	sc.converged = converged; sc.k0 = k0; sc.looks = looks; sc.eagerIters = eagerIters;
	return solveEnd(sc);
}

bool cuba_hip_solver::solveEnd(SolveCtx& sc)
{
	const int maxIter = sc.maxIter; const bool direct = sc.direct; const bool converged = sc.converged;
	const int k0 = sc.k0, looks = sc.looks, eagerIters = sc.eagerIters, predicted = sc.predicted;
	const auto tSolve1 = Clock::now();
	if (std::getenv("CUBA_HIP_DEBUG"))
	{
		std::vector<Scalar> part((size_t)std::max(1, sys.nrz0));
		HIP_TRY(hipMemcpyAsync(part.data(), sys.rz, sizeof(Scalar) * part.size(), hipMemcpyDeviceToHost, stream));
		sync();
		double rz0 = 0; for (Scalar v : part) rz0 += (double)v;
		std::fprintf(stderr, "[cuba_hip] PCG: %d iterations, %d enqueued (%d as plain launches), %d host looks (prediction %d), lambda %.3e, r0.z0 %.6e, solve %.3f ms, graphs built so far %lld\n",
			sc.hInts[1], k0, eagerIters, looks, predicted, lambda, rz0, 1e3 * std::chrono::duration<double>(tSolve1 - sc.tSolve0).count(), (long long)gb.builds.load());
	}
	const int itersDone = sc.itersDone >= 0 ? sc.itersDone : sc.hInts[1];
	cntPcgIters += itersDone; cntPcgEnqueued += k0;
	if (runIters.empty()) firstSolveIters = itersDone;
	runIters.push_back(itersDone);
	if (pcgHistory.size() >= 65536) pcgHistory.erase(pcgHistory.begin(), pcgHistory.begin() + 32768);
	pcgHistory.push_back(converged ? itersDone : -itersDone);
	if (!converged)
	{
		cntPcgUnconverged++;
		coarseValid = false;
		if (direct && !acceptUnconverged) return solveDirect();
		char buf[160];
		std::snprintf(buf, sizeof buf, "PCG stopped at max_iter = %d without reaching pcg_tol = %g", maxIter, pcgTol);
		lastError = buf;
		return acceptUnconverged;
	}
	return true;
}

void cuba_hip_solver::backSubstitute()
{
	need();
	StageTimer tm(this, 4);
	launch_back_substitute(g, st, sys, lambda, stream);
}

bool cuba_hip_solver::solve()
{
	schur();
	if (!solveReduced()) return false;
	backSubstitute();
	return true;
}

void cuba_hip_solver::update()
{
	need();
	StageTimer tm(this, 7);
	launch_update_state(g, sys, stream);
}

double cuba_hip_solver::computeScale(double lam)
{
	need();
	double a = 0, b = 0;
	scaleParts(lam, &a, &b);
	return a + b;
}

void cuba_hip_solver::lmRunBegin(LmRun& r, int niter, double* chi2Out)
{
	const double tau = 1e-5;
	if (!h_lmRing)
	{
		HIP_TRY(hipHostMalloc((void**)&h_lmRing, sizeof(double) * LM_RING * LM_REC, hipHostMallocMapped | hipHostMallocCoherent));
		HIP_TRY(hipHostGetDevicePointer((void**)&lmRingDev, h_lmRing, 0));
	}
	coarseValid = false;
	startRunHistory();
	r = LmRun();
	r.niter = niter; r.chi2Out = chi2Out; r.stop = niter <= 0;
	r.F = computeErrors();
	r.lam = tau * maxDiagonal();
	{
		double* st8 = reinterpret_cast<double*>(hostStage());
		st8[0] = r.F; st8[1] = r.lam; st8[2] = 2.0; st8[3] = 0.0; st8[4] = 0.0; st8[5] = 1.0; st8[6] = 0.0; st8[7] = (double)LmRun::maxq;
		r.tagBase = 65536.0 * (double)(++lmRunNonce); st8[8] = r.tagBase;
		Scalar* l1 = reinterpret_cast<Scalar*>(st8 + 12);
		l1[0] = (Scalar)r.lam;
		HIP_TRY(hipMemcpyAsync(d_lmState.data(), st8, sizeof(double) * 9, hipMemcpyHostToDevice, stream));
		HIP_TRY(hipMemcpyAsync(d_lamS.data(), l1, sizeof(Scalar), hipMemcpyHostToDevice, stream));
	}
	r.lm.state = d_lmState.data(); r.lm.lam = d_lamS.data(); r.lm.ring = lmRingDev;
}

void cuba_hip_solver::lmAbsorb(LmRun& r, int upto)
{
	std::atomic_thread_fence(std::memory_order_acquire);
	for (; r.seen < upto && !r.stop; r.seen++)
	{
		const volatile double* rec = h_lmRing + (size_t)(r.seen % LM_RING) * LM_REC;
		const double tag = r.tagBase + (double)(r.seen + 1);
		if (rec[7] != tag)
		{
			cntLateRecords++;
			sync();
			std::atomic_thread_fence(std::memory_order_acquire);
			if (rec[7] != tag) throw StateError{ "the device's decision record of an LM trial never arrived" };
		}
		const bool acc = rec[5] != 0.0;
		const double rho = rec[2];
		r.lam = rec[3]; r.F = rec[4];
		if (acc) r.rejRun = 0; else r.rejRun++;
		const bool iterationEnds = acc || r.rejRun == LmRun::maxq || !(rho < 0);
		if (!iterationEnds) continue;
		if (r.chi2Out) r.chi2Out[r.done] = r.F;
		r.done++;
		if (r.done == r.niter || r.rejRun == LmRun::maxq || rho <= 0 || !std::isfinite(r.lam)) r.stop = true;
		r.rejRun = 0;
	}
}

bool cuba_hip_solver::lmBeforeTrial(LmRun& r)
{
	if (r.stop) return false;
	if (r.enq > r.seen)
	{
		const bool safe = r.done + 1 < r.niter && r.rejRun + 1 < LmRun::maxq;
		if (!safe) { waitReport(); cntHostLooks++; lmAbsorb(r, r.enq); if (r.stop) return false; }
	}
	cntTrials++;
	lambda = -1.0;
	return true;
}

bool cuba_hip_solver::lmAfterSolveHost(LmRun& r)
{
	lmAbsorb(r, r.enq);
	if (r.stop) { cntTrials--; return false; }
	return true;
}

bool cuba_hip_solver::lmAfterSolve(LmRun& r, bool ok)
{
	if (!lmAfterSolveHost(r)) return false;
	if (ok) launch_trial_tail_fused(g, st, sys, (Scalar)-1, d_backup.data(), stream, &r.lm, poseFactors());
	else launch_lm_decide_failed(sys, r.lm, stream);
	noteReport();
	launch_restore_if_rejected(d_state.data(), d_backup.data(), d_state.size(), r.lm, stream);
	r.enq++;
	(void)hipStreamQuery(stream);
	return true;
}

int cuba_hip_solver::lmRunEnd(LmRun& r)
{
	if (r.seen < r.enq) { waitReport(); cntHostLooks++; lmAbsorb(r, r.enq); }
	lambda = r.lam;
	return r.done;
}

int cuba_hip_solver::optimizeDeviceDecision(int niter, double* chi2Out)
{
	LmRun r;
	lmRunBegin(r, niter, chi2Out);
	while (lmBeforeTrial(r))
	{
		schur(true);
		const bool ok = solveReduced();
		if (!lmAfterSolve(r, ok)) break;
	}
	return lmRunEnd(r);
}

bool cuba_hip_solver::fullyBatchable() const
{
	return batchable() && st.nBig == 0 && st.nDiagProd == 0 && st.nOd > 0 && st.nWaves > 0 && redParts.empty() && !poseFactors();
}

bool cuba_hip_solver::batchable() const
{
	return !profile && partHi < 0 && Pf > 0 && Lf > 0 && E > 0 && trial_tail_parts(g, st, poseFactorParts()) <= d_parts.size() && batch_kernel_class(g, sys) >= 0;
}

void cuba_hip_solver::launchCoarseJobs(std::vector<CoarseJob>& jobs, hipEvent_t common)
{
	if (jobs.empty()) return;
	ensureOverlapObjects();
	hipStream_t side = gjStream;
	const int m = (int)jobs.size();
	if (!h_gjTab) { HIP_TRY(hipHostMalloc((void**)&h_gjTab, sizeof(GjJob) * CUBA_HIP_BATCH_MAX, hipHostMallocDefault)); HIP_TRY(hipEventCreateWithFlags(&evGjTab, hipEventDisableTiming)); HIP_TRY(hipEventRecord(evGjTab, side)); }
	d_gjTab.resize(sizeof(GjJob) * CUBA_HIP_BATCH_MAX);
	HIP_TRY(hipEventSynchronize(evGjTab));
	int nMax = 0;
	for (int a = 0; a < m; a++)
	{
		cuba_hip_solver* h = jobs[a].h;
		const int Nc = 6 * h->sys.cl * h->sys.nc;
		HIP_TRY(hipStreamWaitEvent(side, jobs[a].ownEvent || !common ? h->evSetup : common, 0));
		launch_coarse_assemble(h->g, h->st, h->sys, h->d_coarse[jobs[a].first].data(), side);
		GjJob& j = h_gjTab[a];
		j.buf[0] = h->d_coarse[jobs[a].first].data(); j.buf[1] = h->d_coarse[1 - jobs[a].first].data();
		j.piv[0] = h->sys.gj_pivots; j.piv[1] = h->sys.gj_pivots + 32 * 32;
		j.n = Nc; j.tiles = (Nc + 31) / 32;
		nMax = std::max(nMax, Nc);
	}
	for (int a = 0; a < m; a++) HIP_TRY(hipEventRecord(jobs[a].h->evAssembled, side));
	HIP_TRY(hipMemcpyAsync(d_gjTab.data(), h_gjTab, sizeof(GjJob) * m, hipMemcpyHostToDevice, side));
	HIP_TRY(hipEventRecord(evGjTab, side));
	launch_dense_inverse_batch(reinterpret_cast<const GjJob*>(d_gjTab.data()), m, nMax, side);
	for (int a = 0; a < m; a++)
	{
		cuba_hip_solver* h = jobs[a].h;
		const int Nc = 6 * h->sys.cl * h->sys.nc;
		const size_t invBytes = sizeof(Scalar) * (size_t)Nc * Nc;
		if (h->fp32Inverse()) launch_coarse_to_fp32(h->d_coarse[0].data(), h->d_coarse32[1].data(), Nc, side);
		else launch_coarse_finish(h->d_coarse[0].data(), h->d_coarse[0].data(), Nc, side);
		if (jobs[a].firstInvCopy)
		{
			if (h->fp32Inverse()) HIP_TRY(hipMemcpyAsync(h->d_firstInv32.data(), h->d_coarse32[1].data(), h->inv32Count() * sizeof(float), hipMemcpyDeviceToDevice, side));
			else HIP_TRY(hipMemcpyAsync(h->d_firstInv.data(), h->d_coarse[0].data(), invBytes, hipMemcpyDeviceToDevice, side));
			HIP_TRY(hipEventRecord(h->evFirstInv, side));
		}
		HIP_TRY(hipEventRecord(h->evInverse, side));
	}
	jobs.clear();
}

static int cuba_hip_optimize_batch_full(cuba_hip_solver** hs, int n, int niter, double* chi2, int* nDone)
{
	cuba_hip_solver* lead = hs[0];
	hipStream_t bs = lead->stream;
	struct StreamGuard
	{
		cuba_hip_solver** hs; int n; std::vector<hipStream_t> own;
		StreamGuard(cuba_hip_solver** h, int m, hipStream_t s) : hs(h), n(m), own((size_t)m)
		{
			for (int i = 0; i < n; i++) { own[i] = hs[i]->stream; (void)hipStreamSynchronize(own[i]); hs[i]->stream = s; }
		}
		~StreamGuard() { if (n > 0) (void)hipStreamSynchronize(hs[0]->stream); for (int i = 0; i < n; i++) hs[i]->stream = own[i]; }
	} streamGuard(hs, n, bs);
	std::vector<cuba_hip_solver::LmRun> runs((size_t)n);
	std::vector<cuba_hip_solver::SolveCtx> ctx((size_t)n);
	lead->ensureOverlapObjects();
	std::vector<cuba_hip_solver::CoarseJob> coarseJobs;
	if (lead->h_batchTab && lead->batchTabEntries < 3 * CUBA_HIP_BATCH_MAX) { (void)hipHostFree(lead->h_batchTab); lead->h_batchTab = nullptr; }
	if (!lead->h_batchTab) { HIP_TRY(hipHostMalloc((void**)&lead->h_batchTab, sizeof(BatchEntry) * CUBA_HIP_BATCH_MAX * 3, hipHostMallocDefault)); lead->batchTabEntries = 3 * CUBA_HIP_BATCH_MAX; }
	lead->d_batchTab.resize(sizeof(BatchEntry) * CUBA_HIP_BATCH_MAX * 3);
	BatchEntry* hTab[3]; const BatchEntry* dTab[3];
	for (int k = 0; k < 3; k++) { hTab[k] = lead->h_batchTab + (size_t)k * CUBA_HIP_BATCH_MAX; dTab[k] = reinterpret_cast<const BatchEntry*>(lead->d_batchTab.data()) + (size_t)k * CUBA_HIP_BATCH_MAX; }
	auto upload = [&](int k, int m) { HIP_TRY(hipMemcpyAsync(const_cast<BatchEntry*>(dTab[k]), hTab[k], sizeof(BatchEntry) * m, hipMemcpyHostToDevice, bs)); };
	for (int i = 0; i < n; i++) hs[i]->lmRunBegin(runs[i], niter, chi2 ? chi2 + (size_t)i * niter : nullptr);
	const bool mixed = hs[0]->st.mixed != 0;
	std::vector<int> act;
	std::vector<char> okv((size_t)n), inPcg((size_t)n);
	int batchSolves = 0;
	for (;;)
	{
		act.clear();
		for (int i = 0; i < n; i++) if (hs[i]->lmBeforeTrial(runs[i])) act.push_back(i);
		if (act.empty()) break;
		const int m = (int)act.size();
		unsigned lmMax = 0, schurMax = 0;
		for (int a = 0; a < m; a++)
		{
			cuba_hip_solver* h = hs[act[a]];
			h->zeroReduced();
			BatchEntry& e = hTab[0][a];
			e = BatchEntry();
			e.g = h->g; e.st = h->st; e.sys = h->sys;
			batch_fill_linearize(h->g, h->st, h->d_state.data(), h->d_backup.data(), h->d_state.size(), e.t);
			lmMax = std::max(lmMax, e.t.lmGrid); schurMax = std::max(schurMax, e.t.schurGrid);
		}
		upload(0, m);
		launch_batch_linearize(dTab[0], m, lmMax, schurMax, mixed, bs);
		unsigned setupMax = 0; int gridSpmvMax = 0, ncMax = 0; size_t ldsMax = 0; int target = 4, budgetMax = 0, nPcg = 0, nFused = 0;
		Scalar tol2 = 0;
		for (int a = 0; a < m; a++)
		{
			const int i = act[a];
			cuba_hip_solver* h = hs[i];
			ctx[i] = cuba_hip_solver::SolveCtx(); ctx[i].batched = true; ctx[i].deferCoarse = &coarseJobs; ctx[i].deferLaunch = true;
			BatchEntry& e = hTab[1][a];
			e = BatchEntry();
			const bool finished = h->solveBegin(ctx[i]);
			e.g = h->g; e.st = h->st; e.sys = h->sys;
			if (finished) { okv[i] = ctx[i].result; inPcg[i] = 0; continue; }
			inPcg[i] = 1; nPcg++;
			tol2 = ctx[i].tol2;
			e.maxIter = ctx[i].maxIter;
			e.gridSpmv = (h->g.Pf + h->sys.spmv_rows - 1) / h->sys.spmv_rows;
			if (ctx[i].deferred) { batch_fill_setup(h->g, h->st, h->sys, ctx[i].copySrc, ctx[i].copyDst, ctx[i].copyCount, e.t); e.t.fusedOn = 1; nFused++; }
			setupMax = std::max(setupMax, e.t.setupGrid);
			gridSpmvMax = std::max(gridSpmvMax, e.gridSpmv); ncMax = std::max(ncMax, h->sys.nc); ldsMax = std::max(ldsMax, batch_pcg2_lds_bytes(h->sys));
			target = std::max(target, (ctx[i].predicted + 3) / 4 * 4); budgetMax = std::max(budgetMax, ctx[i].budget);
		}
		if (nPcg > 0)
		{
			upload(1, m);
			if (nFused > 0) launch_batch_setup(dTab[1], m, setupMax, bs);
			HIP_TRY(hipEventRecord(lead->evSetup, bs));
			lead->launchCoarseJobs(coarseJobs, lead->evSetup);
			if (nFused > 0) launch_batch_first_precond(dTab[1], m, lead->sys, ncMax, ldsMax, tol2, bs);
			int k0 = 0, looks = 0;
			std::vector<char> conv((size_t)n, 0), broke((size_t)n, 0);
			bool all = false;
			while (k0 < budgetMax && !all)
			{
				int todo = std::max(4, std::min(target, budgetMax) - k0);
				while (todo > 0)
				{
					const int c = todo;
					for (int k = 0; k < c; k++) launch_pcg_batch_iteration(dTab[1], m, lead->g, lead->sys, gridSpmvMax, ncMax, ldsMax, k, tol2, bs);
					launch_pcg_batch_advance(dTab[1], m, c, bs, tol2);
					for (int i : act) if (inPcg[i]) hs[i]->noteReport();
					k0 += c; todo -= c;
				}
				all = true;
				for (int i : act)
				{
					if (!inPcg[i]) continue;
					cuba_hip_solver* h = hs[i];
					h->waitReport();
					const volatile int* f = ctx[i].hInts;
					if (f[0] != 0) broke[i] = 1;
					else if (f[2] != 0 || f[1] < std::min(k0, ctx[i].maxIter)) conv[i] = 1;
					if (!broke[i] && !conv[i] && k0 < ctx[i].budget) all = false;
					h->cntPcgLooks++; h->cntHostLooks++;
				}
				target = k0 + ((looks == 0 && k0 <= 96) ? 4 : std::max(8, k0 / 8 / 4 * 4));
				looks++;
			}
			for (int i : act)
			{
				if (!inPcg[i]) continue;
				cuba_hip_solver::SolveCtx& sc = ctx[i];
				sc.k0 = std::min(k0, std::max(sc.budget, 4)); sc.looks = looks; sc.eagerIters = 0;
				sc.converged = conv[i] != 0 && sc.hInts[1] <= sc.budget;
				if (!sc.converged && !broke[i]) sc.itersDone = std::min((int)sc.hInts[1], sc.budget);
				okv[i] = hs[i]->retryWithFp64Inverse(broke[i] ? hs[i]->solveBrokeDown(sc) : hs[i]->solveEnd(sc));
			}
			batchSolves++;
		}
		else lead->launchCoarseJobs(coarseJobs, nullptr);
		unsigned tailMax = 0, restoreMax = 0;
		for (int a = 0; a < m; a++)
		{
			const int i = act[a];
			cuba_hip_solver* h = hs[i];
			BatchEntry& e = hTab[2][a];
			e = BatchEntry();
			e.g = h->g; e.st = h->st; e.sys = h->sys;
			if (!h->lmAfterSolveHost(runs[i])) continue;
			batch_fill_tail(h->g, h->st, h->sys, h->d_backup.data(), runs[i].lm, h->d_state.data(), h->d_state.size(), e.t);
			e.t.backupDst = h->d_backup.data();
			if (!okv[i])
			{
				launch_lm_decide_failed(h->sys, runs[i].lm, bs);
				e.t.tailGrid = 0; e.t.reportOn = 0;
			}
			tailMax = std::max(tailMax, e.t.tailGrid); restoreMax = std::max(restoreMax, e.t.restoreGrid);
			h->noteReport();
			runs[i].enq++;
		}
		upload(2, m);
		launch_batch_tail(dTab[2], m, tailMax, restoreMax, bs);
		(void)hipStreamQuery(bs);
	}
	for (int i = 0; i < n; i++) nDone[i] = hs[i]->lmRunEnd(runs[i]);
	return batchSolves;
}

int cuba_hip_optimize_batch_impl(cuba_hip_solver** hs, int n, int niter, double* chi2, int* nDone)
{
	bool together = n > 1;
	for (int i = 0; i < n; i++) hs[i]->need();
	for (int i = 0; i < n && together; i++)
		together = hs[i]->batchable() && hs[i]->device == hs[0]->device && batch_kernel_class(hs[i]->g, hs[i]->sys) == batch_kernel_class(hs[0]->g, hs[0]->sys) &&
			hs[i]->pcgTol == hs[0]->pcgTol && (i == 0 || hs[i]->stream != hs[0]->stream);
	if (!together)
	{
		for (int i = 0; i < n; i++) nDone[i] = hs[i]->optimize(niter, chi2 ? chi2 + (size_t)i * niter : nullptr);
		return 0;
	}
	bool full = true;
	for (int i = 0; i < n && full; i++) full = hs[i]->fullyBatchable() && hs[i]->st.mixed == hs[0]->st.mixed;
	if (full) return cuba_hip_optimize_batch_full(hs, n, niter, chi2, nDone);
	cuba_hip_solver* lead = hs[0];
	hipStream_t bs = lead->stream;
	std::vector<cuba_hip_solver::LmRun> runs((size_t)n);
	std::vector<cuba_hip_solver::SolveCtx> ctx((size_t)n);
	std::vector<hipEvent_t>& evJoin = lead->batchEvents;
	while ((int)evJoin.size() < n + 1) { hipEvent_t e; HIP_TRY(hipEventCreateWithFlags(&e, hipEventDisableTiming)); evJoin.push_back(e); }
	hipEvent_t evFork = evJoin[n];
	if (!lead->h_batchTab) { HIP_TRY(hipHostMalloc((void**)&lead->h_batchTab, sizeof(BatchEntry) * CUBA_HIP_BATCH_MAX * 3, hipHostMallocDefault)); lead->batchTabEntries = 3 * CUBA_HIP_BATCH_MAX; }
	lead->d_batchTab.resize(sizeof(BatchEntry) * CUBA_HIP_BATCH_MAX * 3);
	BatchEntry* hTab = lead->h_batchTab;
	const BatchEntry* dTab = reinterpret_cast<const BatchEntry*>(lead->d_batchTab.data());
	lead->ensureOverlapObjects();
	std::vector<cuba_hip_solver::CoarseJob> coarseJobs;
	for (int i = 0; i < n; i++) hs[i]->lmRunBegin(runs[i], niter, chi2 ? chi2 + (size_t)i * niter : nullptr);
	std::vector<int> act, inPcg;
	std::vector<char> okv((size_t)n);
	int batchSolves = 0;
	for (;;)
	{
		act.clear();
		for (int i = 0; i < n; i++) if (hs[i]->lmBeforeTrial(runs[i])) act.push_back(i);
		if (act.empty()) break;
		inPcg.clear();
		for (int i : act)
		{
			hs[i]->schur(true);
			ctx[i] = cuba_hip_solver::SolveCtx(); ctx[i].batched = true; ctx[i].deferCoarse = &coarseJobs;
			if (hs[i]->solveBegin(ctx[i])) okv[i] = ctx[i].result; else inPcg.push_back(i);
		}
		lead->launchCoarseJobs(coarseJobs);
		if (!inPcg.empty())
		{
			const int m = (int)inPcg.size();
			int gridSpmvMax = 0, ncMax = 0; size_t ldsMax = 0; int target = 4, budgetMax = 0;
			for (int a = 0; a < m; a++)
			{
				cuba_hip_solver* h = hs[inPcg[a]];
				BatchEntry& e = hTab[a];
				e.g = h->g; e.st = h->st; e.sys = h->sys; e.maxIter = ctx[inPcg[a]].maxIter;
				e.gridSpmv = (h->g.Pf + h->sys.spmv_rows - 1) / h->sys.spmv_rows;
				gridSpmvMax = std::max(gridSpmvMax, e.gridSpmv); ncMax = std::max(ncMax, h->sys.nc); ldsMax = std::max(ldsMax, batch_pcg2_lds_bytes(h->sys));
				target = std::max(target, (ctx[inPcg[a]].predicted + 3) / 4 * 4); budgetMax = std::max(budgetMax, ctx[inPcg[a]].budget);
				if (h != lead) { HIP_TRY(hipEventRecord(evJoin[a], h->stream)); HIP_TRY(hipStreamWaitEvent(bs, evJoin[a], 0)); }
			}
			HIP_TRY(hipMemcpyAsync(lead->d_batchTab.data(), hTab, sizeof(BatchEntry) * m, hipMemcpyHostToDevice, bs));
			const Scalar tol2 = ctx[inPcg[0]].tol2;
			int k0 = 0, looks = 0;
			std::vector<char> conv((size_t)m, 0), broke((size_t)m, 0);
			bool all = false;
			while (k0 < budgetMax && !all)
			{
				int todo = std::max(4, std::min(target, budgetMax) - k0);
				while (todo > 0)
				{
					const int c = todo;
					for (int k = 0; k < c; k++) launch_pcg_batch_iteration(dTab, m, lead->g, lead->sys, gridSpmvMax, ncMax, ldsMax, k, tol2, bs);
					launch_pcg_batch_advance(dTab, m, c, bs, tol2);
					for (int a = 0; a < m; a++) hs[inPcg[a]]->noteReport();
					k0 += c; todo -= c;
				}
				all = true;
				for (int a = 0; a < m; a++)
				{
					cuba_hip_solver* h = hs[inPcg[a]];
					h->waitReport();
					const volatile int* f = ctx[inPcg[a]].hInts;
					if (f[0] != 0) broke[a] = 1;
					else if (f[2] != 0 || f[1] < std::min(k0, ctx[inPcg[a]].maxIter)) conv[a] = 1;
					if (!broke[a] && !conv[a] && k0 < ctx[inPcg[a]].budget) all = false;
					h->cntPcgLooks++; h->cntHostLooks++;
				}
				target = k0 + ((looks == 0 && k0 <= 96) ? 4 : std::max(8, k0 / 8 / 4 * 4));
				looks++;
			}
			HIP_TRY(hipEventRecord(evFork, bs));
			for (int a = 0; a < m; a++)
			{
				const int i = inPcg[a];
				cuba_hip_solver* h = hs[i];
				if (h != lead) HIP_TRY(hipStreamWaitEvent(h->stream, evFork, 0));
				cuba_hip_solver::SolveCtx& sc = ctx[i];
				sc.k0 = std::min(k0, std::max(sc.budget, 4)); sc.looks = looks; sc.eagerIters = 0;
				sc.converged = conv[a] != 0 && sc.hInts[1] <= sc.budget;
				if (!sc.converged && !broke[a]) sc.itersDone = std::min((int)sc.hInts[1], sc.budget);
				okv[i] = h->retryWithFp64Inverse(broke[a] ? h->solveBrokeDown(sc) : h->solveEnd(sc));
// ... 180 lines not shown
```

### cuda-bundle-adjustment_amd/csrc/ba_setup.hip

```cpp
#include "ba_solver.hpp"

using namespace cubahip;

void cuba_hip_solver::finishValues()
{
	if (!valuesPending) return;
	valuesPending = false;
	HIP_TRY(hipStreamWaitEvent(stream, evValues, 0));
	topo::launch_gather_edges(d_perm.data(), d_rawEp.data(), d_rawEl.data(), d_rawDim.data(), d_rawMeas.data(), d_rawOmega.data(), E,
		nullptr, nullptr, d_mu.data(), d_mv.data(), d_mr.data(), d_w.data(), stream);
	sortedValuesValid = true;
}

void cuba_hip_solver::setGraph(int Pt_, int Pf_, int Lt_, int Lf_, const double* q, const double* t, const double* cam, const double* Xw,
	int E_, const int32_t* ep, const int32_t* el, const uint8_t* edim, const double* meas, const double* omega, bool deferValues, int ownLo, int ownHi)
{
	const bool ranged = ownHi >= 0;
	if (ranged && (ownLo < 0 || ownHi > Lt_ || ownLo > ownHi)) throw ArgError{ "bad landmark range" };
	if (ranged) deferValues = false;
	if (valuesPending) { HIP_TRY(hipStreamSynchronize(upStream)); valuesPending = false; sortedValuesValid = false; }
	deferredUpload = false;
	if (Pt_ < 0 || Lt_ < 0 || E_ < 0 || Pf_ < 0 || Pf_ > Pt_ || Lf_ < 0 || Lf_ > Lt_) throw ArgError{ "bad vertex counts" };
	if (Pt_ >= STEREO_BIT) throw ArgError{ "too many poses" };
	if (sizeof(Scalar) == 4 && Lt_ >= (1 << 23)) throw ArgError{ "fp32 build: at most 2^23 - 1 landmarks" };
// ... 359 lines not shown
			const uint32_t c = (uint32_t)(ent[x].key >> 32); const uint32_t id = (uint32_t)ent[x].key;
			if (c != last) { k++; h_colind[k] = (int)c; blkRow[k] = i; prodPtr[k] = (int)out; last = c; }
			if (!id) continue;
			if ((long long)id - 1 >= idLo && (long long)id - 1 < idHi) { prodEa[out] = ent[x].ea; prodEb[out] = ent[x].eb; out++; }
		}
	});
	prodPtr[nblk] = (int)nprodLocal;
	lap("structure: Hsc pattern + product blocks");
	std::vector<int> adjPtr(Pf + 1, 0);
	for (int i = 0; i < Pf; i++)
		for (int k = h_rowptr[i]; k < h_rowptr[i + 1]; k++)
		{
			adjPtr[i + 1]++;
			if (h_colind[k] != i) adjPtr[h_colind[k] + 1]++;
		}
	for (int i = 0; i < Pf; i++) adjPtr[i + 1] += adjPtr[i];
	std::vector<int> adjBlk(adjPtr[Pf]), adjCol(adjPtr[Pf]);
	{
		std::vector<int> cur(adjPtr.begin(), adjPtr.end() - 1);
		for (int i = 0; i < Pf; i++)
			for (int k = h_rowptr[i]; k < h_rowptr[i + 1]; k++)
			{
				const int j = h_colind[k];
				if (j != i) { adjBlk[cur[j]] = k | (int)0x80000000; adjCol[cur[j]] = i; cur[j]++; }
			}
		for (int i = 0; i < Pf; i++)
			for (int k = h_rowptr[i]; k < h_rowptr[i + 1]; k++) { adjBlk[cur[i]] = k; adjCol[cur[i]] = h_colind[k]; cur[i]++; }
	}
	lap("structure: adjacency");
	g.e_begin = h_lmptr[lo]; g.e_end = h_lmptr[hi];
	{
		int maxCnt = 0;
		for (int k = 0; k < nblk; k++) maxCnt = std::max(maxCnt, prodPtr[k + 1] - prodPtr[k]);
		std::vector<int> start(maxCnt + 2, 0);
		for (int k = 0; k < nblk; k++) { const int c = prodPtr[k + 1] - prodPtr[k]; if (c > 0) start[maxCnt - c + 1]++; }
		for (int c = 0; c <= maxCnt; c++) start[c + 1] += start[c];
		odBlocks.resize(start[maxCnt + 1]);
		for (int k = 0; k < nblk; k++) { const int c = prodPtr[k + 1] - prodPtr[k]; if (c > 0) odBlocks[start[maxCnt - c]++] = k; }
		if (rowGroupedBlocks(nprodLocal))
		{
			std::vector<int> cntOf(nblk);
			for (int k = 0; k < nblk; k++) cntOf[k] = prodPtr[k + 1] - prodPtr[k];
			odBlocks = rowGroupedOrder(blkRow.data(), h_colind.data(), cntOf.data(), nblk);
		}
	}
	lap("structure: product lists");
	std::vector<int> pePtr(Pf + 1, 0), peEdge;
	const bool wholeGraph = g.e_begin == 0 && g.e_end == E;
	if (!wholeGraph)
	{
		for (int i = g.e_begin; i < g.e_end; i++) if (h_epose[i] < Pf) pePtr[h_epose[i] + 1]++;
		for (int i = 0; i < Pf; i++) pePtr[i + 1] += pePtr[i];
		peEdge.resize(pePtr[Pf]);
		std::vector<int> cur(pePtr.begin(), pePtr.end() - 1);
		for (int i = g.e_begin; i < g.e_end; i++) if (h_epose[i] < Pf) peEdge[cur[h_epose[i]]++] = i;
	}
	lap("structure: pose edge lists");
	std::vector<int> waveLm, bigLm;
	{
		int start = -1, cnt = 0;
		auto flush = [&](int end) { if (start >= 0 && cnt > 0) { waveLm.push_back(start); waveLm.push_back(end); } start = -1; cnt = 0; };
		for (int l = lo; l < hi; l++)
		{
			if ((l - lo) % topo::WAVE_CHUNK == 0) flush(l);
			const int n = h_lmptr[l + 1] - h_lmptr[l];
			if (n > WAVE)
			{
				flush(l);
				bigLm.push_back(l);
				continue;
			}
			if (n == 0) continue;
			if (start >= 0 && cnt + n > WAVE) flush(l);
			if (start < 0) start = l;
			cnt += n;
		}
		flush(hi);
	}

	lap("structure: wave list");
	d_waveLm.upload(waveLm, stream); d_bigLm.upload(bigLm, stream);
	d_rowptr.upload(h_rowptr, stream); d_colind.upload(h_colind, stream);
	d_adjPtr.upload(adjPtr, stream); d_adjBlk.upload(adjBlk, stream); d_adjCol.upload(adjCol, stream);
	int ellM = 0, ellOver = 0;
	{
		int maxRow = 0;
		for (int i = 0; i < Pf; i++) maxRow = std::max(maxRow, adjPtr[i + 1] - adjPtr[i]);
		const int M = std::min(3, (maxRow + 19) / 20);
		ellM = M; ellOver = maxRow > 20 * M;
		std::vector<int2> ell((size_t)Pf * M * 20, int2{ 0, -1 });
		for (int i = 0; i < Pf; i++)
		{
			const int n = std::min(adjPtr[i + 1] - adjPtr[i], 20 * M);
			for (int e = 0; e < n; e++) ell[(size_t)i * M * 20 + e] = int2{ adjBlk[adjPtr[i] + e], adjCol[adjPtr[i] + e] };
		}
		d_ell.upload(ell, stream);
	}
	d_blkrow.upload(blkRow, stream); d_odBlocks.upload(odBlocks, stream); d_prodPtr.upload(prodPtr, stream);
	d_prodEa.upload(prodEa, stream); d_prodEb.upload(prodEb, stream); d_pePtr.upload(wholeGraph ? peAllPtr : pePtr, stream); d_peEdge.upload(wholeGraph ? peAll : peEdge, stream);
	const CoarseCfg cc = coarseConfig();
	allocSystem(nblk, cc);
	const int agg = cc.agg, cl = cc.cl, nc = cc.nc;
	lap("structure: uploads + allocs");
	std::vector<int> cbI, cbJ, cbPtr(1, 0), cbBlk, adjRow(adjBlk.size());
	std::vector<Scalar> cbWi, cbWj;
	auto weight = [&](int pose) {
		if (pose == Pf - 1 && Pf % agg == 1) return Scalar(0);
		return Scalar(2 * (pose % agg) + 1 - agg) / Scalar(agg);
	};
	for (int i = 0; i < Pf; i++) for (int a = adjPtr[i]; a < adjPtr[i + 1]; a++) adjRow[a] = i;
	if (nc > 0)
	{
		std::vector<uint64_t> ck; ck.reserve(adjBlk.size());
		for (int i = 0; i < Pf; i++)
			for (int a = adjPtr[i]; a < adjPtr[i + 1]; a++)
				ck.push_back(((uint64_t)((size_t)(i / agg) * nc + adjCol[a] / agg) << 32) | (uint32_t)a);
		std::sort(ck.begin(), ck.end());
		for (size_t x = 0; x < ck.size(); x++)
		{
			const int cbid = (int)(ck[x] >> 32);
			if (x == 0 || cbid != (int)(ck[x - 1] >> 32))
			{
				if (x) cbPtr.push_back((int)cbBlk.size());
				cbI.push_back(cbid / nc); cbJ.push_back(cbid % nc);
			}
			cbBlk.push_back(adjBlk[(uint32_t)ck[x]]);
			if (cl == 2) { cbWi.push_back(weight(adjRow[(uint32_t)ck[x]])); cbWj.push_back(weight(adjCol[(uint32_t)ck[x]])); }
		}
		cbPtr.push_back((int)cbBlk.size());
	}
	d_cbI.upload(cbI, stream); d_cbJ.upload(cbJ, stream); d_cbPtr.upload(cbPtr, stream); d_cbBlk.upload(cbBlk, stream); d_cbWi.upload(cbWi, stream); d_cbWj.upload(cbWj, stream);
	sync();
	lap("structure: coarse lists + sync");
	diagProdBlocks = 0; for (int k : odBlocks) diagProdBlocks += k >= 0 && blkRow[k] == h_colind[k];
	heavyBlocks = 0;
	if (!rowGroupedBlocks(nprodLocal))
		for (int k : odBlocks) heavyBlocks += prodPtr[k + 1] - prodPtr[k] > BP_HEAVY;
	publishStructure(nblk, (int)waveLm.size() / 2, (int)bigLm.size(), (int)odBlocks.size(), (int)cbI.size(), ellM, ellOver, cc);
	hostPatternValid = true;
	const double dt = std::chrono::duration<double>(Clock::now() - t0).count();
	prof[1] += 0.5 * dt; prof[5] += 0.5 * dt;
}

cuba_hip_solver::CoarseCfg cuba_hip_solver::coarseConfig() const
{
	int agg = pcgAggregate;
	const int cl = coarseLinear ? 2 : 1;
	const int ncMax = std::min(180, std::max(115, (Pf + 31) / 32));
	if (agg < 0) agg = cl == 2 ? (Pf >= 1320 ? std::max(16, (Pf + ncMax - 1) / ncMax) : std::max(6, (Pf + 27) / 55)) : std::max(12, (Pf + 159) / 160);
	const int spmvRows = spmv_rows_for(Pf);
	if (agg > 0) agg = (agg + spmvRows - 1) / spmvRows * spmvRows;
	int nc = agg > 0 ? (Pf + agg - 1) / agg : 0;
	int clOut = cl;
	const int aggMax = 600 / spmvRows * spmvRows;
	auto ncOf = [&](int a) { return (Pf + a - 1) / a; };
	auto fits = [&](int c, int a) { const int n = ncOf(a); return c * n <= 600 && sizeof(Scalar) * (12 * (size_t)c * n + 12 * (size_t)a + 200) <= 60 * 1024; };
	if (agg > aggMax) agg = aggMax;
	if (agg > 0)
	{
		bool ok = false;
		for (int c = cl; c >= 1 && !ok; c--)
		{
			int a = agg;
			while (a < aggMax && !fits(c, a)) a = std::min(aggMax, 2 * a);
			if (!fits(c, a))
			{
				int m = ((int)std::ceil(std::sqrt((double)c * Pf)) + spmvRows - 1) / spmvRows * spmvRows;
				m = std::min(aggMax, std::max(agg, m));
				if (fits(c, m)) a = m;
			}
			if (fits(c, a)) { agg = a; clOut = c; ok = true; }
		}
		if (!ok) agg = 0;
	}
	nc = agg > 0 ? ncOf(agg) : 0;
	if (nc < 2) { agg = 0; nc = 0; }
	return CoarseCfg{ agg, agg > 0 ? clOut : cl, nc, spmvRows };
}

void cuba_hip_solver::allocSystem(int nblk, const CoarseCfg& c)
{
	directRefused = false; directSticky = false; directPlanValid = false;
	d_red.resize((size_t)36 * nblk + (size_t)12 * Pf);
	d_lmSys.resize((size_t)9 * Lf); d_lmInv.resize((size_t)8 * std::max(Lf, 1)); d_erec.resize((size_t)8 * E); d_xp.resize((size_t)6 * Pf); d_xl.resize((size_t)3 * Lf);
	d_minv.resize((size_t)36 * Pf);
	d_r.resize((size_t)6 * Pf); d_z.resize((size_t)6 * Pf); d_p0.resize((size_t)6 * Pf); d_p1.resize((size_t)6 * Pf); d_ap.resize((size_t)6 * Pf);
	d_red.zero(stream); d_lmSys.zero(stream); d_lmInv.zero(stream); d_xp.zero(stream); d_xl.zero(stream);
	reducedZeroed = true;
	for (auto& b : d_coarse) b.resize((size_t)36 * c.cl * c.cl * c.nc * c.nc);
	{
		const size_t n = (size_t)6 * c.cl * c.nc;
		for (auto& b : d_coarse32) b.resize(fp32Inverse() ? n * ((n + 3) & ~(size_t)3) : 0);
	}
	d_rc.resize((size_t)12 * c.cl * c.nc); d_r2.resize((size_t)6 * Pf);
	maxIterAlloc = pcgMaxIter > 0 ? pcgMaxIter : std::min(32768, std::max(64, 4 * 6 * Pf));
	const int gridSetup = (Pf + PCG_SETUP_POSES - 1) / PCG_SETUP_POSES, gridUpd = (Pf + 39) / 40, gridSpmv = (Pf + c.spmvRows - 1) / c.spmvRows;
	rzStrideCfg = std::max(1, std::max(std::max(gridSetup, gridUpd), c.nc)); pqStrideCfg = std::max(1, gridSpmv);
	d_rz.resize((size_t)5 * rzStrideCfg); d_pq.resize((size_t)4 * pqStrideCfg);
}

std::vector<int> cuba_hip_solver::rowGroupedOrder(const int* blkRow, const int* blkCol, const int* cnt, int nblk) const
{
	const int tr = 4, tc = 4;
	const long long nColTiles = (Pf + tc - 1) / tc;
	(void)nColTiles;
	std::vector<int> val; val.reserve(nblk);
	std::vector<int> rest; rest.reserve(nblk);
	std::vector<int> chunkStart;
	for (int k0 = 0; k0 < nblk;)
	{
		const int band = blkRow[k0] / tr;
		int head[4], end[4], nr = 0, k = k0;
		while (k < nblk && blkRow[k] / tr == band)
		{
			const int r = blkRow[k], b = k;
			while (k < nblk && blkRow[k] == r) k++;
			head[nr] = b; end[nr] = k; nr++;
		}
		for (;;)
		{
			int ct = 0x7fffffff;
			for (int x = 0; x < nr; x++) if (head[x] < end[x]) ct = std::min(ct, blkCol[head[x]] / tc);
			if (ct == 0x7fffffff) break;
			int tile[16], nt = 0;
			for (int x = 0; x < nr; x++)
				while (head[x] < end[x] && blkCol[head[x]] / tc == ct) { if (cnt[head[x]] > 0) tile[nt++] = head[x]; head[x]++; }
			for (int a2 = 1; a2 < nt; a2++)
			{
				const int v = tile[a2]; int b2 = a2;
				while (b2 > 0 && cnt[tile[b2 - 1]] < cnt[v]) { tile[b2] = tile[b2 - 1]; b2--; }
				tile[b2] = v;
			}
			if (nt == 16) { chunkStart.push_back((int)val.size()); val.insert(val.end(), tile, tile + 16); }
			else rest.insert(rest.end(), tile, tile + nt);
		}
		k0 = k;
	}
	const size_t nWhole = chunkStart.size();
	const size_t n = (size_t)nblk + 1;
	for (size_t i = 0; i < rest.size(); i += 16)
	{
		const size_t e = std::min(rest.size(), i + 16);
		for (size_t a2 = i + 1; a2 < e; a2++)
		{
			const int v = rest[a2]; size_t b2 = a2;
			while (b2 > i && cnt[rest[b2 - 1]] < cnt[v]) { rest[b2] = rest[b2 - 1]; b2--; }
			rest[b2] = v;
		}
		chunkStart.push_back((int)(n + i));
	}
	const size_t nChunks = chunkStart.size();
	auto firstOf = [&](size_t c) { return chunkStart[c] < (int)n ? val[chunkStart[c]] : rest[chunkStart[c] - n]; };
	std::vector<std::pair<int, int>> byLen(nChunks);
	for (size_t c = 0; c < nChunks; c++) byLen[c] = std::make_pair(-cnt[firstOf(c)], (int)c);
	std::stable_sort(byLen.begin(), byLen.end(), [](const std::pair<int, int>& x, const std::pair<int, int>& y) { return x.first < y.first; });
	std::vector<int> od(nChunks * 16, -1);
	for (size_t o = 0; o < nChunks; o++)
	{
		const size_t c = (size_t)byLen[o].second;
		if (c < nWhole) for (int x = 0; x < 16; x++) od[o * 16 + x] = val[chunkStart[c] + x];
		else
		{
			const size_t b = (size_t)chunkStart[c] - n, e = std::min(rest.size(), b + 16);
			for (size_t x = b; x < e; x++) od[o * 16 + (x - b)] = rest[x];
		}
	}
	return od;
}

void cuba_hip_solver::publishStructure(int nblk, int nWaves, int nBig, int nOd, int nCb, int ellM, int ellOver, const CoarseCfg& c)
{
	const int agg = c.agg, cl = c.cl, nc = c.nc, spmvRows = c.spmvRows;
	const int gridSetup = (Pf + PCG_SETUP_POSES - 1) / PCG_SETUP_POSES, gridUpd = (Pf + 39) / 40, gridSpmv = (Pf + spmvRows - 1) / spmvRows;
	st = DeviceStructure();
	st.nWaves = nWaves; st.wave_lm = d_waveLm.data();
	st.nBig = nBig; st.big_lm = d_bigLm.data();
	st.nblk = nblk; st.hsc_rowptr = d_rowptr.data(); st.hsc_colind = d_colind.data();
	st.adj_ptr = d_adjPtr.data(); st.adj_blk = d_adjBlk.data(); st.adj_col = d_adjCol.data();
	st.ell = d_ell.data(); st.ell_m = ellM; st.ell_over = ellOver;
	st.hsc_blkrow = d_blkrow.data(); st.nOd = nOd; st.nDiagProd = diagProdBlocks; st.od_blocks = d_odBlocks.data(); st.nHeavy = std::min(heavyBlocks, nOd);
	if (d_prodEa.size() > ((size_t)1 << 19)) st.nHeavy = 0;
	st.inv_rows8 = Lf >= 250000;
	st.prod_ea = d_prodEa.data(); st.prod_eb = d_prodEb.data();
	if (!localRanges) fillProdLm();
	st.prod_lm = d_prodLm.data();
	st.prod_beg = localRanges ? d_prodBeg.data() : d_prodPtr.data(); st.prod_end = localRanges ? d_prodEnd.data() : d_prodPtr.data() + 1;
	st.pe_beg = localRanges ? d_peBeg.data() : d_pePtr.data(); st.pe_end = localRanges ? d_peEnd.data() : d_pePtr.data() + 1;
	st.pe_edge = d_peEdge.data(); st.e_rec = d_erec.data();
	st.nCb = nCb; st.cb_I = d_cbI.data(); st.cb_J = d_cbJ.data(); st.cb_ptr = d_cbPtr.data(); st.cb_blk = d_cbBlk.data(); st.cb_wi = d_cbWi.data(); st.cb_wj = d_cbWj.data();
	sys = DeviceSystem();
	sys.hsc = d_red.data(); sys.bsc = d_red.data() + (size_t)36 * nblk; sys.bp = sys.bsc + (size_t)6 * Pf;
	sys.lm_sys = d_lmSys.data(); sys.lm_inv = d_lmInv.data(); sys.xp = d_xp.data(); sys.xl = d_xl.data(); sys.slots = slotsDev; sys.host_flags = flagsDev; sys.parts = d_parts.data();
	sys.maxdiag = d_maxdiag.data(); sys.fail = d_fail.data();
	sys.minv = d_minv.data(); sys.r = d_r.data(); sys.z = d_z.data(); sys.p0 = d_p0.data(); sys.p1 = d_p1.data(); sys.ap = d_ap.data();
	sys.rz = d_rz.data(); sys.pq = d_pq.data(); sys.iters = d_iters.data(); sys.kbase = d_kbase.data(); sys.ticket = d_ticket.data();
	dropPcgGraph();
	firstInvValid = false; firstInvPending = false; prevRunIters.clear();
	sys.rzStride = rzStrideCfg; sys.pqStride = pqStrideCfg; sys.npq = gridSpmv;
	sys.nrz0 = agg > 0 ? nc : gridSetup; sys.nrz = agg > 0 ? nc : gridUpd; sys.done = d_done.data();
	coarseValid = false;
	d_qpart.resize(agg > 0 ? (size_t)(agg / spmvRows) * 6 * cl * nc : 1); d_gjPivots.resize(2 * 32 * 32); sys.gj_pivots = d_gjPivots.data();
	sys.qpart = d_qpart.data();
	d_qpart.zero(stream);
	d_lamS.resize(1); d_lmState.resize(16); sys.lam_dev = d_lamS.data();
	sys.upper = agg > 0 && agg <= pcg_rows_max_aggregate() && (spmvUpper < 0 ? spmvRows == 4 : spmvUpper != 0) ? 1 : 0;
	if (sys.upper)
	{
		d_tq.resize((size_t)6 * nblk); sys.tq = d_tq.data(); d_hrow.release(); sys.hrow = nullptr;
		d_lowpos.resize((size_t)nblk); sys.lowpos = d_lowpos.data();
		DeviceGraph gg; gg.Pf = Pf;
		launch_build_lowpos(gg, st, d_lowpos.data(), stream);
		sys.npq = spmv_upper_grid(Pf);
	}
	else
	{
		d_hrow.resize((size_t)36 * 20 * ellM * Pf); sys.hrow = d_hrow.data();
		d_hrow.zero(stream);
	}
	sys.spmv_rows = spmvRows;
	sys.agg = agg; sys.nc = nc; sys.cl = agg > 0 ? cl : 1; sys.inv_agg = agg > 0 ? Scalar(1) / Scalar(agg) : Scalar(0); sys.acinv = d_coarse[0].data(); sys.rc = d_rc.data(); sys.r2 = d_r2.data();
	sys.acinv32 = fp32Inverse() && agg > 0 ? d_coarse32[0].data() : nullptr;
	cutReductionParts();
	haveStructure = true;
	structRelPairs = h_relPairs; cntStructureBuilds++;
}

void cuba_hip_solver::cutReductionParts()
{
	redParts.clear();
	if (partHi < 0 || st.nblk <= 0 || st.nOd <= 0 || Pf <= 0) return;
	const size_t matrixBytes = (size_t)36 * st.nblk * sizeof(Scalar);
	const int want = redChunks > 0 ? redChunks : (int)std::min<size_t>(8, matrixBytes >> 23);
	if (want <= 1) return;
	std::vector<int> rowptr((size_t)Pf + 1), od((size_t)st.nOd);
	HIP_TRY(hipMemcpyAsync(rowptr.data(), d_rowptr.data(), sizeof(int) * rowptr.size(), hipMemcpyDeviceToHost, stream));
	HIP_TRY(hipMemcpyAsync(od.data(), d_odBlocks.data(), sizeof(int) * od.size(), hipMemcpyDeviceToHost, stream));
	sync();
	std::vector<int> cut{ 0 };
	for (int c = 1; c < want; c++)
	{
		const int target = (int)((long long)st.nblk * c / want);
		const int b = *std::lower_bound(rowptr.begin(), rowptr.end(), target);
		if (b > cut.back() && b < st.nblk) cut.push_back(b);
	}
	if (cut.size() < 2) return;
	cut.push_back(st.nblk);
	const int C = (int)cut.size() - 1;
	std::vector<std::vector<int>> lists(C);
	std::vector<int> heavy(C, 0);
	int c = 0;
	for (int i = 0; i < st.nOd; i++)
	{
		if (od[i] >= 0) c = (int)(std::upper_bound(cut.begin() + 1, cut.end(), od[i]) - (cut.begin() + 1));
		lists[c].push_back(od[i]);
		if (i < st.nHeavy) heavy[c]++;
	}
	od.clear();
	for (int k = 0; k < C; k++)
	{
		RedPart p;
		p.od.begin = (int)od.size(); od.insert(od.end(), lists[k].begin(), lists[k].end()); p.od.end = (int)od.size(); p.od.heavy = heavy[k];
		p.blkBegin = (size_t)cut[k]; p.blkEnd = (size_t)cut[k + 1];
		redParts.push_back(p);
	}
	d_odBlocks.upload(od, stream);
	sync();
}

void cuba_hip_solver::fillProdLm()
{
	d_prodLm.resize(d_prodEa.size());
	topo::launch_gather_int(d_prodEa.data(), d_elm.data(), d_prodEa.size(), d_prodLm.data(), stream);
}

void cuba_hip_solver::computeLandmarkOrder()
{
	d_lmFirst.resize(Lt); d_lmLast.resize(Lt); d_lmMap.resize(Lt); d_rawEl.resize(E);
	d_k64a.resize(std::max((size_t)Lf, d_k64a.size())); d_k64b.resize(std::max((size_t)Lf, d_k64b.size()));
	d_v32a.resize(std::max((size_t)Lf, d_v32a.size())); d_v32b.resize(std::max((size_t)Lf, d_v32b.size()));
	sortTemp((size_t)Lf);
	topo::launch_lm_first_last(d_rawEp.data(), d_rawElCaller.data(), E, Lt, d_lmFirst.data(), d_lmLast.data(), stream);
	topo::launch_lm_order_keys(d_lmFirst.data(), d_lmLast.data(), Lf, d_k64a.data(), d_v32a.data(), stream);
	HIP_TRY(topo::sort_u64_u32(d_topoTemp.data(), d_topoTemp.size(), d_k64a.data(), d_k64b.data(), d_v32a.data(), d_v32b.data(), (size_t)Lf, 64, stream));
	topo::launch_lm_order_map(d_v32b.data(), Lf, Lt, d_lmMap.data(), stream);
	topo::launch_remap_landmarks(d_rawElCaller.data(), d_lmMap.data(), E, d_rawEl.data(), stream);
	lmOrderActive = true;
	dropSnapshots();
}

void cuba_hip_solver::switchLandmarkOrder(bool on)
{
	if (on == lmOrderActive || !devTopology || E == 0 || d_rawElCaller.size() != (size_t)E) return;
	Scalar* X = d_state.data() + 7 * (size_t)Pt;
	if (lmOrderActive) landmarkRowsInPlace(X, Lt, 3, false);
	if (on) { computeLandmarkOrder(); landmarkRowsInPlace(X, Lt, 3, true); }
	else resetLandmarkOrder();
	runDeviceEdgeSort();
	sync();
	haveStructure = false; hostTopoValid = false; hostPatternValid = false;
}

void cuba_hip_solver::resetLandmarkOrder()
{
	d_rawEl.resize(E);
	if (E) HIP_TRY(hipMemcpyAsync(d_rawEl.data(), d_rawElCaller.data(), sizeof(int) * (size_t)E, hipMemcpyDeviceToDevice, stream));
	if (lmOrderActive) dropSnapshots();
	lmOrderActive = false;
}

void cuba_hip_solver::landmarkRowsInPlace(Scalar* rows, int nrows, int width, bool toInternal)
{
	const size_t n = (size_t)nrows * width;
	if (!n) return;
	d_rowTmp.resize(std::max(n, d_rowTmp.size()));
	HIP_TRY(hipMemcpyAsync(d_rowTmp.data(), rows, sizeof(Scalar) * n, hipMemcpyDeviceToDevice, stream));
	topo::launch_permute_rows(d_rowTmp.data(), rows, d_lmMap.data(), nrows, width, toInternal, stream);
}

const Scalar* cuba_hip_solver::landmarkRowsForCaller(const Scalar* rows, int nrows, int width)
{
	if (!lmOrderActive || nrows == 0) return rows;
	d_rowTmp.resize(std::max((size_t)nrows * width, d_rowTmp.size()));
	topo::launch_permute_rows(rows, d_rowTmp.data(), d_lmMap.data(), nrows, width, false, stream);
	return d_rowTmp.data();
}

void cuba_hip_solver::resetPoseOrder()
{
	if (reorderActive) dropSnapshots();
	reorderActive = false;
	priorSet.uploaded = false;
	poseNewOfOld.resize(Pf); poseOldOfNew.resize(Pf);
	for (int i = 0; i < Pf; i++) poseNewOfOld[i] = poseOldOfNew[i] = i;
}

void cuba_hip_solver::permuteStateRows(std::vector<Scalar>& state, std::vector<Scalar>& camv) const
{
	permutePoseArray(state.data(), 4, true);
	permutePoseArray(state.data() + 4 * (size_t)Pt, 3, true);
	permutePoseArray(camv.data(), 5, true);
}

void cuba_hip_solver::runDeviceEdgeSort(bool withValues)
{
	if (withValues && valuesPending) { valuesPending = false; HIP_TRY(hipStreamWaitEvent(stream, evValues, 0)); }
	d_mu.resize(E); d_mv.resize(E); d_mr.resize(E); d_w.resize(E);
	d_k64a.resize(E); d_k64b.resize(E); d_v32a.resize(E); d_perm.resize(E); d_counters.resize(topo::CNT_COUNT);
	d_epose.resize(E); d_elm.resize(E); d_lmptr.resize((size_t)Lt + 1);
	d_counters.zero(stream);
	topo::launch_edge_keys(d_rawEp.data(), d_rawEl.data(), d_rawDim.data(), E, Pt, Pf, Lt, Lf, d_k64a.data(), d_v32a.data(), d_counters.data(), stream);
	const size_t tb = topo::sort_temp_bytes(E);
	d_topoTemp.resize(std::max(tb, d_topoTemp.size()));
	HIP_TRY(topo::sort_u64_u32(d_topoTemp.data(), d_topoTemp.size(), d_k64a.data(), d_k64b.data(), d_v32a.data(), d_perm.data(), E, 32 + bitsFor(Lt), stream));
	topo::launch_gather_edges(d_perm.data(), d_rawEp.data(), d_rawEl.data(), d_rawDim.data(), d_rawMeas.data(), d_rawOmega.data(), E,
		d_epose.data(), d_elm.data(), withValues ? d_mu.data() : nullptr, d_mv.data(), d_mr.data(), d_w.data(), stream);
	topo::launch_segment_ptr(d_elm.data(), E, Lt, d_lmptr.data(), stream);
	if (withValues) sortedValuesValid = true;
}

std::vector<int> cuba_hip_solver::chainOrder(const std::vector<int>& rowptr, const std::vector<int>& colind, const std::vector<int>& prodPtr) const
{
	const int n = Pf;
	std::vector<int> adjP(n + 1, 0);
	for (int i = 0; i < n; i++)
		for (int k = rowptr[i]; k < rowptr[i + 1]; k++) if (colind[k] != i) { adjP[i + 1]++; adjP[colind[k] + 1]++; }
	for (int i = 0; i < n; i++) adjP[i + 1] += adjP[i];
	std::vector<int> adjJ(adjP[n]), adjW(adjP[n]), cur(adjP.begin(), adjP.end() - 1);
	std::vector<long long> deg(n, 0);
	for (int i = 0; i < n; i++)
		for (int k = rowptr[i]; k < rowptr[i + 1]; k++)
		{
			const int j = colind[k];
			if (j == i) continue;
			const int w = std::max(1, prodPtr[k + 1] - prodPtr[k]);
			adjJ[cur[i]] = j; adjW[cur[i]++] = w; adjJ[cur[j]] = i; adjW[cur[j]++] = w;
			deg[i] += w; deg[j] += w;
		}
	std::vector<char> visited(n, 0);
	std::vector<int> order; order.reserve(n);
	std::vector<std::pair<int, int>> heap;
	int at = -1;
	for (int i = 0; i < n; i++) if (deg[i] > 0 && (at < 0 || deg[i] < deg[at])) at = i;
	if (at < 0) at = 0;
	int nextUnvisited = 0;
	while ((int)order.size() < n)
	{
		visited[at] = 1; order.push_back(at);
		int best = -1, bw = -1;
		for (int x = adjP[at]; x < adjP[at + 1]; x++)
		{
			const int j = adjJ[x];
			if (visited[j]) continue;
			heap.emplace_back(adjW[x], -j); std::push_heap(heap.begin(), heap.end());
			if (adjW[x] > bw || (adjW[x] == bw && j < best)) { best = j; bw = adjW[x]; }
		}
		if (best >= 0) { at = best; continue; }
		at = -1;
		while (!heap.empty())
		{
			std::pop_heap(heap.begin(), heap.end());
			const int j = -heap.back().second; heap.pop_back();
			if (!visited[j]) { at = j; break; }
		}
		if (at < 0)
		{
			while (nextUnvisited < n && visited[nextUnvisited]) nextUnvisited++;
			if (nextUnvisited >= n) break;
			at = nextUnvisited;
		}
	}
	std::vector<int> newOfOld(n);
	for (int k = 0; k < n; k++) newOfOld[order[k]] = k;
	return newOfOld;
}

void cuba_hip_solver::applyPoseOrder(const std::vector<int>& newOfOld)
{
	std::vector<Scalar> state(d_state.size()), camv((size_t)5 * Pt);
	HIP_TRY(hipMemcpyAsync(state.data(), d_state.data(), sizeof(Scalar) * state.size(), hipMemcpyDeviceToHost, stream));
	HIP_TRY(hipMemcpyAsync(camv.data(), d_cam.data(), sizeof(Scalar) * camv.size(), hipMemcpyDeviceToHost, stream));
	sync();
	permutePoseArray(state.data(), 4, false); permutePoseArray(state.data() + 4 * (size_t)Pt, 3, false); permutePoseArray(camv.data(), 5, false);
	poseNewOfOld = newOfOld;
	reorderActive = false;
	priorSet.uploaded = false;
	for (int i = 0; i < Pf; i++) { poseOldOfNew[newOfOld[i]] = i; if (newOfOld[i] != i) reorderActive = true; }
	permuteStateRows(state, camv);
	d_state.upload(state, stream); d_cam.upload(camv, stream);
	d_poseMap.upload(poseNewOfOld, stream);
	topo::launch_remap_poses(d_rawEpCaller.data(), d_poseMap.data(), E, Pf, d_rawEp.data(), stream);
	if (lmOrderActive || landmarkOrderAllowed())
	{
		if (lmOrderActive) landmarkRowsInPlace(d_state.data() + 7 * (size_t)Pt, Lt, 3, false);
		computeLandmarkOrder();
		landmarkRowsInPlace(d_state.data() + 7 * (size_t)Pt, Lt, 3, true);
	}
	runDeviceEdgeSort();
	sync();
	dropSnapshots();
	haveStructure = false; hostTopoValid = false; hostPatternValid = false;
}

bool cuba_hip_solver::tryReorder(int nblk, int farBlocks)
{
	const int offDiag = nblk - Pf;
	if (!poseReorder || Pf < 48 || offDiag <= 0 || 2 * (long long)farBlocks < offDiag) return false;
	std::vector<int> rp((size_t)Pf + 1), ci(nblk), pp((size_t)nblk + 1);
	HIP_TRY(hipMemcpyAsync(rp.data(), d_rowptr.data(), sizeof(int) * rp.size(), hipMemcpyDeviceToHost, stream));
	HIP_TRY(hipMemcpyAsync(ci.data(), d_colind.data(), sizeof(int) * ci.size(), hipMemcpyDeviceToHost, stream));
	HIP_TRY(hipMemcpyAsync(pp.data(), d_prodPtr.data(), sizeof(int) * pp.size(), hipMemcpyDeviceToHost, stream));
	sync();
	const std::vector<int> order = chainOrder(rp, ci, pp);
	long long farNew = 0;
	for (int i = 0; i < Pf; i++)
		for (int k = rp[i]; k < rp[i + 1]; k++) farNew += std::abs(order[i] - order[ci[k]]) > farOffset();
	if (std::getenv("CUBA_HIP_DEBUG")) std::fprintf(stderr, "[cuba_hip] pose order: %d of %d off-diagonal blocks far from the diagonal, %lld after the walk\n", farBlocks, offDiag, farNew);
	if (2 * farNew >= farBlocks) return false;
	applyPoseOrder(order);
	return true;
}

void cuba_hip_solver::ensureHostTopology()
{
	if (hostTopoValid || !devTopology) return;
	std::vector<uint32_t> p32(E);
	h_lmptr.resize((size_t)Lt + 1);
	std::vector<int>&sPose = h_spose[topoSlot], &sLm = h_slm[topoSlot];
	sPose.resize(E); sLm.resize(E);
	if (E)
	{
		HIP_TRY(hipMemcpyAsync(p32.data(), d_perm.data(), sizeof(uint32_t) * E, hipMemcpyDeviceToHost, stream));
		HIP_TRY(hipMemcpyAsync(sPose.data(), d_epose.data(), sizeof(int) * E, hipMemcpyDeviceToHost, stream));
		HIP_TRY(hipMemcpyAsync(sLm.data(), d_elm.data(), sizeof(int) * E, hipMemcpyDeviceToHost, stream));
	}
	HIP_TRY(hipMemcpyAsync(h_lmptr.data(), d_lmptr.data(), sizeof(int) * ((size_t)Lt + 1), hipMemcpyDeviceToHost, stream));
	sync();
	perm.assign(p32.begin(), p32.end());
	h_epose.resize(E);
	for (int i = 0; i < E; i++) h_epose[i] = sPose[i] & ~STEREO_BIT;
	hostTopoValid = true;
}

void cuba_hip_solver::buildStructureDevice()
{
	const auto t0 = Clock::now();
	lap(nullptr);
	int* cnt = d_counters.data();
	d_counters.zero(stream);
	sortTemp((size_t)std::max(E, Lf + 1));
	d_lmNfree.resize(Lf); d_pairCount.resize((size_t)Lf + 1); d_lmPairBase.resize((size_t)Lf + 1);
	d_freeCount.resize((size_t)Lf + 1); d_freeScan.resize((size_t)Lf + 1);
	topo::launch_lm_pairs(d_lmptr.data(), d_epose.data(), Lf, Pf, d_lmNfree.data(), d_pairCount.data(), d_freeCount.data(), stream);
	HIP_TRY(topo::exclusive_scan_i64(d_topoTemp.data(), d_topoTemp.size(), d_pairCount.data(), d_lmPairBase.data(), (size_t)Lf + 1, stream));
	HIP_TRY(topo::exclusive_scan_i64(d_topoTemp.data(), d_topoTemp.size(), d_freeCount.data(), d_freeScan.data(), (size_t)Lf + 1, stream));
	d_k32a.resize(E); d_k32b.resize(E); d_v32a.resize(E); d_v32b.resize(E); d_tmpI0.resize(E);
	topo::launch_pose_keys(d_epose.data(), E, Pf, d_k32a.data(), d_v32a.data(), stream);
	HIP_TRY(topo::sort_u32_u32(d_topoTemp.data(), d_topoTemp.size(), d_k32a.data(), d_k32b.data(), d_v32a.data(), d_v32b.data(), E, bitsFor(Pf), stream));
	d_peEdge.resize(E); d_pePtr.resize((size_t)Pf + 1);
	topo::launch_copy_u32_to_int(d_v32b.data(), d_peEdge.data(), E, stream);
	topo::launch_copy_u32_to_int(d_k32b.data(), d_tmpI0.data(), E, stream);
	topo::launch_segment_ptr(d_tmpI0.data(), E, Pf, d_pePtr.data(), stream);
	const int lo = std::max(0, partLo), hi = partHi < 0 ? Lt : std::min(Lt, partHi);
	localRanges = partHi >= 0;
	const int nChunks = (hi - lo + topo::WAVE_CHUNK - 1) / topo::WAVE_CHUNK;
	d_chunk.resize((size_t)2 * std::max(1, nChunks));
	if (nChunks == 0) d_chunk.zero(stream);
	topo::launch_wave_count(d_lmptr.data(), lo, hi, d_chunk.data(), stream);
// ... 192 lines not shown
```

### cuda-bundle-adjustment_amd/csrc/ba_solver.hpp

```cpp
#pragma once

#include <algorithm>
#include <chrono>
#include <cmath>
#include <cstdarg>
#include <cstdio>
#include <cstdlib>
#include <cstring>
#include <numeric>
#include <string>
#include <thread>
#include <atomic>
#include <functional>
#include <condition_variable>
#include <deque>
#include <map>
#include <mutex>
#include <vector>

#include "../../include/cuba_hip.h"
#include "ba_kernels.hpp"
#include "host_pool.hpp"
#include "ba_structure.hpp"

// ... 233 lines not shown
	int overlapPeriod() const
	{
		const int Nc = 6 * sys.cl * sys.nc;
		return Nc <= 512 ? 1 : Nc <= 1024 ? 2 : 3;
	}
	hipStream_t gjStream = nullptr;
	hipEvent_t evSetup = nullptr, evAssembled = nullptr, evInverse = nullptr, evFirstInv = nullptr;
	int pendingInv = -1;
	bool assemblePending = false;
	void ensureOverlapObjects();
	void waitAssembled() { if (assemblePending) { HIP_TRY(hipStreamWaitEvent(stream, evAssembled, 0)); assemblePending = false; } }
	void drainInversion()
	{
		if (pendingInv >= 0) { HIP_TRY(hipStreamWaitEvent(stream, evInverse, 0)); pendingInv = -1; }
		assemblePending = false;
	}
	struct PatternEntry { uint64_t key; int ea, eb; };
	std::vector<PatternEntry> h_ent; std::vector<int> h_work[6];
	std::vector<double> h_chiSorted;
	std::vector<Scalar> h_stage[6];
	std::vector<int> h_inEp, h_inEl; std::vector<uint8_t> h_inDim;
	std::vector<int> h_spose[2], h_slm[2];
	int topoSlot = 0;
	std::vector<int> runIters;
	std::vector<int> prevRunIters;
	void startRunHistory() { if (!runIters.empty()) prevRunIters.swap(runIters); runIters.clear(); directSticky = false; }
	int firstSolveIters = 0;

	double lambda = 0;
	int maxIterAlloc = 0;
	long long nmul = 0;
	int64_t cntPcgIters = 0, cntTrials = 0, cntCoarseRefresh = 0, cntPcgLooks = 0, cntPcgEnqueued = 0, cntPcgUnconverged = 0;
	int64_t cntPcgPlain = 0;
	int64_t cntCoarseInline = 0;
	int64_t cntFp32Fallbacks = 0;
	int64_t cntUploads = 0;
	bool acceptUnconverged = false;
	std::vector<int> pcgHistory;
	double prof[CUBA_HIP_PROFILE_ITEMS] = { 0, 0, 0, 0, 0, 0, 0, 0 };

	~cuba_hip_solver()
	{
		{ std::lock_guard<std::mutex> lk(gb.m); gb.stop = true; gb.jobs.clear(); }
		gb.cv.notify_all();
		if (gb.th.joinable()) gb.th.join();
		for (hipGraphExec_t e : gb.trash) (void)hipGraphExecDestroy(e);
		gb.trash.clear();
		dropPcgGraph();
		if (gjStream) { (void)hipStreamSynchronize(gjStream); (void)hipStreamDestroy(gjStream); (void)hipEventDestroy(evSetup); (void)hipEventDestroy(evAssembled); (void)hipEventDestroy(evInverse); (void)hipEventDestroy(evFirstInv); }
		if (captureStream) (void)hipStreamDestroy(captureStream);
		if (upStream) { (void)hipStreamSynchronize(upStream); (void)hipStreamDestroy(upStream); (void)hipEventDestroy(evValues); }
		if (h_tileStage) (void)hipHostFree(h_tileStage);
		if (evTileInputs) (void)hipEventDestroy(evTileInputs);
		if (h_pinned) (void)hipHostFree(h_pinned);
		if (h_lmRing) (void)hipHostFree(h_lmRing);
		if (h_batchTab) (void)hipHostFree(h_batchTab);
		if (h_gjTab) { (void)hipHostFree(h_gjTab); (void)hipEventDestroy(evGjTab); }
		for (hipEvent_t e : batchEvents) (void)hipEventDestroy(e);
		if (ownStream && stream) (void)hipStreamDestroy(stream);
	}

	void sync() { HIP_TRY(hipStreamSynchronize(stream)); }

	bool failDirty = true;
	int expectedTicket = 0;
	bool hintSameEdges = false, hintSameValues = false;
	void noteReport() { expectedTicket++; }
	void waitReport();

	void downloadAsDouble(const Scalar* dsrc, double* hdst, size_t n);
	void uploadFromDouble(Scalar* ddst, const double* hsrc, size_t n);

	template <class F>
	static void parallelRows(int nrows, const std::vector<long long>& start, F&& fn)
	{
		const long long total = nrows > 0 ? start[nrows] - start[0] : 0;
		const int T = (int)std::min<long long>(HostPool::instance().maxThreads(), total / 50000 + 1);
		if (T <= 1) { for (int i = 0; i < nrows; i++) fn(i); return; }
		std::vector<int> cut(T + 1, 0);
		for (int t = 1; t < T; t++)
		{
			const long long target = start[0] + total * t / T;
			cut[t] = std::max(cut[t - 1], (int)(std::upper_bound(start.begin(), start.begin() + nrows + 1, target) - start.begin()) - 1);
		}
		cut[T] = nrows;
		HostPool::instance().run(T, [&](int t) { for (int i = cut[t]; i < cut[t + 1]; i++) fn(i); });
	}

	template <class F>
	static void parallelFor(int n, F&& fn)
	{
		const int T = (int)std::min<long long>(HostPool::instance().maxThreads(), n / 50000 + 1);
		if (T <= 1) { for (int i = 0; i < n; i++) fn(i); return; }
		HostPool::instance().run(T, [&](int t) {
			const int r0 = (int)((long long)n * t / T), r1 = (int)((long long)n * (t + 1) / T);
			for (int i = r0; i < r1; i++) fn(i);
		});
	}

	Clock::time_point lapT;
	void lap(const char* what)
	{
		static const bool on = std::getenv("CUBA_HIP_DEBUG") != nullptr;
		if (!on) return;
		const auto now = Clock::now();
		if (what) std::fprintf(stderr, "[cuba_hip] %-34s %7.2f ms\n", what, 1e3 * std::chrono::duration<double>(now - lapT).count());
		lapT = now;
	}

	struct StageTimer
	{
		cuba_hip_solver* s; int item; Clock::time_point t0;
		StageTimer(cuba_hip_solver* s_, int item_) : s(s_), item(item_)
		{
			if (s->profile) { s->sync(); t0 = Clock::now(); }
		}
		~StageTimer()
		{
			if (s->profile)
			{
				(void)hipStreamSynchronize(s->stream);
				s->prof[item] += std::chrono::duration<double>(Clock::now() - t0).count();
			}
		}
	};

	hipStream_t upStream = nullptr; hipEvent_t evValues = nullptr;
	bool valuesPending = false, deferredUpload = false;
	bool sortedValuesValid = false;
	int* h_tileStage = nullptr; size_t tileStageCap = 0; hipEvent_t evTileInputs = nullptr;
	void finishValues();
	void setGraph(int Pt_, int Pf_, int Lt_, int Lf_, const double* q, const double* t, const double* cam, const double* Xw,
		int E_, const int32_t* ep, const int32_t* el, const uint8_t* edim, const double* meas, const double* omega, bool deferValues = false,
		int ownLo = 0, int ownHi = -1);

	void buildStructure();

	struct CoarseCfg { int agg, cl, nc, spmvRows; };
	CoarseCfg coarseConfig() const;

	int rzStrideCfg = 1, pqStrideCfg = 1;
	void allocSystem(int nblk, const CoarseCfg& c);

	static bool rowGroupedBlocks(long long products) { return products > (1LL << 19); }
	std::vector<int> rowGroupedOrder(const int* blkRow, const int* blkCol, const int* cnt, int nblk) const;
	int diagProdBlocks = 0;
	int heavyBlocks = 0;
	void publishStructure(int nblk, int nWaves, int nBig, int nOd, int nCb, int ellM, int ellOver, const CoarseCfg& c);
	bool hostPatternValid = false;
	void fillProdLm();

	int farOffset() const { return std::max(24, Pf / 8); }
	void resetPoseOrder();
	template <class T>
	void permutePoseArray(T* a, int width, bool toInternal) const
	{
		if (!reorderActive) return;
		std::vector<T> tmp(a, a + (size_t)width * Pf);
		for (int old = 0; old < Pf; old++)
		{
			const int nw = poseNewOfOld[old];
			const T* src = tmp.data() + (size_t)width * (toInternal ? old : nw);
			T* dst = a + (size_t)width * (toInternal ? nw : old);
			for (int k = 0; k < width; k++) dst[k] = src[k];
		}
	}
	void permuteStateRows(std::vector<Scalar>& state, std::vector<Scalar>& camv) const;

	void runDeviceEdgeSort(bool withValues = true);

	std::vector<int> chainOrder(const std::vector<int>& rowptr, const std::vector<int>& colind, const std::vector<int>& prodPtr) const;

	void applyPoseOrder(const std::vector<int>& newOfOld);

	bool tryReorder(int nblk, int farBlocks);

	void ensureHostTopology();

	template <class T> T readBack(const T* dev)
	{
		T v;
		HIP_TRY(hipMemcpyAsync(&v, dev, sizeof(T), hipMemcpyDeviceToHost, stream));
		sync();
		return v;
	}
	void sortTemp(size_t n) { const size_t tb = std::max(topo::sort_temp_bytes(n), topo::scan_temp_bytes(n)); d_topoTemp.resize(std::max(tb, d_topoTemp.size())); }

	void buildStructureDevice();

	struct CallerBlock { uint64_t key; int src; bool transposed; };
	std::vector<CallerBlock> callerBlocks();

	void ensureHostPattern();

	void need()
	{
		if (!haveGraph) throw StateError{ "set_graph must be called first" };
		if (haveStructure && h_relPairs != structRelPairs) haveStructure = false;
		buildStructure(); finishValues(); g.rk[0] = rk[0]; g.rk[1] = rk[1]; st.mixed = mixedPrecision ? 1 : 0;
		uploadPoseFactors();
	}

	PoseFactorSet priorSet, relSet;
	DevicePoseFactors pf;
	const DevicePoseFactors* poseFactors() const { return priorSet.n() + relSet.n() > 0 ? &pf : nullptr; }
	int poseFactorParts() const { return pose_factor_chi2_parts(poseFactors()); }
	void clearPoseFactors()
	{
		for (PoseFactorSet* set : { &priorSet, &relSet }) { set->v = PoseFactorValues(); set->kind.clear(); set->delta.clear(); set->order.clear(); set->uploaded = false; }
		h_relPairs.clear(); pf = DevicePoseFactors();
	}
	void uploadPoseFactors();
	int internalPose(int p) const { return p < Pf && reorderActive ? poseNewOfOld[p] : p; }
	void setPosePriors(int n, const int32_t* pose, const double* q, const double* t, const double* info);
	void priorChiSquares(double* out);
	void setRelativePoseEdges(int n, const int32_t* pi, const int32_t* pj, const double* q, const double* t, const double* info);
	void relativePoseChiSquares(double* out);
	void setPoseFactorRobustKernels(int factorType, int n, const int32_t* kind, const double* delta);
	std::vector<uint64_t> h_relPairs, structRelPairs;
	int64_t relStructure = -1;
	int64_t cntStructureBuilds = 0;
	std::vector<uint64_t> h_relSeeds;
	DevBuf<int> d_relSeedFlag, d_relSeedScan; DevBuf<uint64_t> d_relSeeds; DevBuf<Scalar> d_relRec;
	std::vector<uint64_t> relSeedKeys() const;

	double readSlots(int which)
	{
		sync();
		double s = 0;
		for (int i = 0; i < NSLOT; i++) s += slot(which * NSLOT + i);
		return s;
	}

	double computeErrors();

	void zeroReduced(bool force = false) { waitAssembled(); if (force || partHi >= 0 || !reducedZeroed) { d_red.zero(stream); reducedZeroed = true; } }
	bool reducedZeroed = false;

	void linearize(int mode, double lam, bool withBackup = false);

	void assemble();

	void maxDiagonalParts(double* posePart, double* lmPart);

	void scaleParts(double lam, double* posePart, double* lmPart);

	double maxDiagonal();

	void schur(bool withBackup = false);

	bool lastSolveBrokeDown = false;
	int lastFailCode = 0;
	bool solveReduced();

	bool directFallback = true;
	bool directAlways = false;
	int directAfter = 0;
	int directMaxTiles = 1 << 20;
	int directSlack = -1;
	bool directSticky = false;
	bool directRefused = false;
	bool directPlanValid = false;
	double directSeconds = 0, directPlanSeconds = 0;
	SparseCholPlan directPlan;
	SparseChol directDev;
	DevBuf<Scalar> d_scTiles, d_scTilesT, d_scY, d_scRinv;
	DevBuf<int> d_scInts, d_scFail;
	int64_t cntDirect = 0, cntDirectFailed = 0;
	int64_t directPlanBuilds = 0;
	bool directUsable() const { return directFallback && !directRefused && Pf > 0; }
	int pcgBudget(int maxIter) const;
	bool ensureDirectPlan();
	bool solveDirect();

	SelInvPlan selPlan;
	int64_t selPlanFor = -1;
	SelInv selDev;
	DevBuf<int> d_selInts;
	DevBuf<Scalar> d_sigma, d_covW, d_covPose, d_covBlk, d_covLm;
	bool covBlocksValid = false;
	double covSeconds = 0;
	bool computeCovariance(double* poseCov, double* lmCov);
	void covarianceBlocks(double* out);
	double covWorkspaceMb = 0;
	double covPairsSeconds = 0;
	int covPairChunks = 0;
	PairWork covPairWork;
	DevBuf<Scalar> d_pairOut;
	bool computeCovariancePairs(int n, const int32_t* kindA, const int32_t* indexA, const int32_t* kindB, const int32_t* indexB, double* out);

	struct CoarseJob { cuba_hip_solver* h; int first; bool firstInvCopy; bool ownEvent; };
	void launchCoarseJobs(std::vector<CoarseJob>& jobs, hipEvent_t common = nullptr);
	GjJob* h_gjTab = nullptr; DevBuf<unsigned char> d_gjTab; hipEvent_t evGjTab = nullptr;
	struct SolveCtx
	{
		int maxIter = 0, budget = 0, predicted = 32, k0 = 0, looks = 0, eagerIters = 0;
		int itersDone = -1;
		Scalar tol2 = 0;
		bool twoLevel = false, direct = false, graphs = false, converged = false, result = false;
		bool batched = false;
		std::vector<CoarseJob>* deferCoarse = nullptr;
		bool deferLaunch = false;
		bool deferred = false;
		const Scalar* copySrc = nullptr; Scalar* copyDst = nullptr; size_t copyCount = 0;
		volatile int* hInts = nullptr;
		Clock::time_point tSolve0;
	};
	bool solveBegin(SolveCtx& sc);
	bool solveBrokeDown(SolveCtx& sc);
	bool solveEnd(SolveCtx& sc);
	bool solveReducedOnce();
	bool retryWithFp64Inverse(bool ok);

	void backSubstitute();

	bool solve();

	void update();

	double computeScale(double lam);

	void push() { need(); HIP_TRY(hipMemcpyAsync(d_backup.data(), d_state.data(), d_state.size() * sizeof(Scalar), hipMemcpyDeviceToDevice, stream)); }
	void pop() { need(); HIP_TRY(hipMemcpyAsync(d_state.data(), d_backup.data(), d_state.size() * sizeof(Scalar), hipMemcpyDeviceToDevice, stream)); }

	int optimize(int niter, double* chi2Out);
	int optimizeDeviceDecision(int niter, double* chi2Out);
	struct LmRun
	{
		static constexpr int maxq = 10;
		int niter = 0, enq = 0, seen = 0, done = 0, rejRun = 0;
		bool stop = false;
		double lam = 0, F = 0, tagBase = 0;
		double* chi2Out = nullptr;
		LmDevice lm;
	};
	void lmRunBegin(LmRun& r, int niter, double* chi2Out);
	void lmAbsorb(LmRun& r, int upto);
	bool lmBeforeTrial(LmRun& r);
	bool lmAfterSolveHost(LmRun& r);
	bool lmAfterSolve(LmRun& r, bool ok);
	bool fullyBatchable() const;
	int lmRunEnd(LmRun& r);
	bool batchable() const;
	std::vector<hipEvent_t> batchEvents;
	BatchEntry* h_batchTab = nullptr; int batchTabEntries = 0;
	DevBuf<unsigned char> d_batchTab;
	DevBuf<double> d_lmState; DevBuf<Scalar> d_lamS;
	double* h_lmRing = nullptr; double* lmRingDev = nullptr; uint64_t lmRunNonce = 0; int64_t cntLateRecords = 0;
	int64_t cntHostLooks = 0;

	void enqueueEvaluate(double lam, bool withScale);
	void readEvaluate(bool withScale, double* Fhat, double* scale);
	void evaluateTrial(double lam, bool withScale, double* Fhat, double* scale);


	void timeKernels(int reps, double* msOut);

	void chiSquares(double* out, bool wait = true);
};
```

Before: 792.9 million edge-iterations/s.

## Chain LM iterations on device: device-side init, deferred publish, restore fused into linearize

Moves LM run initialization (initial chi2, max diagonal, lambda) into a device kernel so the run starts without host readbacks. It skips the host-visible report publish on trials where the host will not wait. It folds the rejected-trial state restore into the linearize pass's backup-copy blocks, which then read pose and landmark inputs from the backup when the trial was rejected. It also defers enqueueing the coarse-preconditioner side work until after the first PCG chunk is launched. The aim is to cut host synchronisation and extra kernel launches per iteration, at the cost of more complex device-side control flow and a risk of subtle state-ordering bugs.

Result: faster. 835.3 million edge-iterations/s (median of 6 runs) (+5.3%).

```diff
diff --git a/cuda-bundle-adjustment_amd/csrc/ba_edge.hip b/cuda-bundle-adjustment_amd/csrc/ba_edge.hip
--- a/cuda-bundle-adjustment_amd/csrc/ba_edge.hip
+++ b/cuda-bundle-adjustment_amd/csrc/ba_edge.hip
@@ -241,7 +241,7 @@
 }
 
 __device__ __forceinline__ void reduce_report_body(const DeviceSystem& sys, const Scalar* pA, int nA, Scalar* oA, const Scalar* pB, int nB, Scalar* oB,
-	const Scalar* pC, int nC, Scalar* oC, double* lmState, Scalar* lmLam, double* lmRing)
+	const Scalar* pC, int nC, Scalar* oC, double* lmState, Scalar* lmLam, double* lmRing, int publish)
 {
 	__shared__ Scalar sh[3][16];
 	const Scalar vA = wave_sum(parts_thread_sum(pA, nA)), vB = wave_sum(parts_thread_sum(pB, nB)), vC = wave_sum(parts_thread_sum(pC, nC));
@@ -254,6 +254,7 @@
 		store_slot_group(oA, tA); store_slot_group(oB, tB); store_slot_group(oC, tC);
 		if (lmState && threadIdx.x == 0) lm_decide(lmState, lmLam, lmRing, 1, (double)tA, (double)tB, (double)tC);
 	}
+	if (!publish) return;
 	__threadfence_system();
 	asm volatile("s_waitcnt vmcnt(0) lgkmcnt(0)" ::: "memory");
 	__syncthreads();
@@ -262,9 +263,9 @@
 
 
 __global__ __launch_bounds__(1024) void reduce_report_kernel(DeviceSystem sys, const Scalar* pA, int nA, Scalar* oA, const Scalar* pB, int nB, Scalar* oB,
-	const Scalar* pC, int nC, Scalar* oC, double* lmState, Scalar* lmLam, double* lmRing)
-{
-	reduce_report_body(sys, pA, nA, oA, pB, nB, oB, pC, nC, oC, lmState, lmLam, lmRing);
+	const Scalar* pC, int nC, Scalar* oC, double* lmState, Scalar* lmLam, double* lmRing, int publish)
+{
+	reduce_report_body(sys, pA, nA, oA, pB, nB, oB, pC, nC, oC, lmState, lmLam, lmRing, publish);
 }
 
 __global__ __launch_bounds__(1024) void reduce_report_batch_kernel(const BatchEntry* __restrict__ tab)
@@ -272,7 +273,7 @@
 	const BatchEntry& e = tab[blockIdx.x];
 	const BatchTrial& t = e.t;
 	if (!t.reportOn) return;
-	reduce_report_body(e.sys, t.scParts, t.nA, e.sys.slots + NSLOT, t.chiParts, t.nA, e.sys.slots, t.scaleParts, 4 * t.nScale, e.sys.slots + 3 * NSLOT, t.lmState, t.lmLam, t.lmRing);
+	reduce_report_body(e.sys, t.scParts, t.nA, e.sys.slots + NSLOT, t.chiParts, t.nA, e.sys.slots, t.scaleParts, 4 * t.nScale, e.sys.slots + 3 * NSLOT, t.lmState, t.lmLam, t.lmRing, 1);
 }
 
 __global__ __launch_bounds__(256) void landmark_scale_kernel(DeviceGraph g, DeviceSystem sys, Scalar lambda, Scalar* parts)
@@ -585,7 +586,7 @@
 }
 
 void launch_trial_tail_fused(const DeviceGraph& g, const DeviceStructure& st, const DeviceSystem& sys, Scalar lambda, const Scalar* old, hipStream_t s,
-	const LmDevice* decide, const DevicePoseFactors* pf)
+	const LmDevice* decide, const DevicePoseFactors* pf, int publish)
 {
 	const int nLm = (st.nWaves + LIN_BLOCK / WAVE - 1) / (LIN_BLOCK / WAVE);
 	const int nA = nLm + st.nBig;
@@ -600,7 +601,7 @@
 	if (st.nBig > 0) hipLaunchKernelGGL(big_trial_tail_kernel, dim3(st.nBig), dim3(256), 0, s, g, st, sys, lambda, old, scParts + nLm, chiParts + nLm);
 	if (nPf > 0) launch_pose_factor_chi2(g, *pf, chiParts + nA, s);
 	hipLaunchKernelGGL(reduce_report_kernel, dim3(1), dim3(1024), 0, s, sys, scParts, nA, sys.slots + NSLOT, chiParts, nA + nPf, sys.slots, scaleParts, 4 * nScale, sys.slots + 3 * NSLOT,
-		decide ? decide->state : (double*)nullptr, decide ? decide->lam : (Scalar*)nullptr, decide ? decide->ring : (double*)nullptr);
+		decide ? decide->state : (double*)nullptr, decide ? decide->lam : (Scalar*)nullptr, decide ? decide->ring : (double*)nullptr, publish);
 }
 
 void batch_fill_tail(const DeviceGraph& g, const DeviceStructure& st, const DeviceSystem& sys, const Scalar* old, const LmDevice& lm, Scalar* state, size_t stateCount, BatchTrial& t)
@@ -632,6 +633,25 @@
 	hipLaunchKernelGGL(lm_decide_failed_kernel, dim3(1), dim3(64), 0, s, sys, lm.state, lm.lam, lm.ring);
 }
 
+__global__ void lm_run_init_kernel(const Scalar* __restrict__ chiSlots, const unsigned long long* __restrict__ maxdiag, double* lmState, Scalar* lmLam,
+	double tau, double tagBase, double maxq)
+{
+#pragma clang fp contract(off)
+	if (threadIdx.x != 0 || blockIdx.x != 0) return;
+	double F = 0;
+	for (int i = 0; i < NSLOT; i++) F += (double)chiSlots[i];
+	unsigned long long m = 0;
+	for (int i = 0; i < 64; i++) m = maxdiag[i] > m ? maxdiag[i] : m;
+	const double lam = tau * __longlong_as_double((long long)m);
+	lmState[0] = F; lmState[1] = lam; lmState[2] = 2.0; lmState[3] = 0.0; lmState[4] = 0.0; lmState[5] = 1.0; lmState[6] = 0.0; lmState[7] = maxq; lmState[8] = tagBase;
+	lmLam[0] = (Scalar)lam;
+}
+
+void launch_lm_run_init(const Scalar* chiSlots, const unsigned long long* maxdiag, const LmDevice& lm, double tau, double tagBase, int maxq, hipStream_t s)
+{
+	hipLaunchKernelGGL(lm_run_init_kernel, dim3(1), dim3(64), 0, s, chiSlots, maxdiag, lm.state, lm.lam, tau, tagBase, (double)maxq);
+}
+
 __global__ __launch_bounds__(256) void restore_if_rejected_batch_kernel(const BatchEntry* __restrict__ tab)
 {
 	const BatchTrial& t = tab[blockIdx.y].t;
diff --git a/cuda-bundle-adjustment_amd/csrc/ba_kernels.hpp b/cuda-bundle-adjustment_amd/csrc/ba_kernels.hpp
--- a/cuda-bundle-adjustment_amd/csrc/ba_kernels.hpp
+++ b/cuda-bundle-adjustment_amd/csrc/ba_kernels.hpp
@@ -144,7 +144,7 @@
 
 struct BlockPassRange { int begin, end, heavy; };
 void launch_linearize_dm(const DeviceGraph& g, const DeviceStructure& st, const DeviceSystem& sys, int mode, Scalar lambda, hipStream_t s,
-	const Scalar* backupSrc = nullptr, Scalar* backupDst = nullptr, size_t backupCount = 0, const BlockPassRange* range = nullptr);
+	Scalar* backupSrc = nullptr, Scalar* backupDst = nullptr, size_t backupCount = 0, const BlockPassRange* range = nullptr, const double* restoreFlag = nullptr);
 void launch_block_pass(const DeviceGraph& g, const DeviceStructure& st, const DeviceSystem& sys, const BlockPassRange& range, hipStream_t s);
 
 void launch_pose_maxdiag(const DeviceGraph& g, const DeviceStructure& st, const DeviceSystem& sys, hipStream_t s);
@@ -154,10 +154,11 @@
 void launch_pose_scale(const DeviceGraph& g, const DeviceSystem& sys, Scalar lambda, Scalar* slots, hipStream_t s);
 struct LmDevice;
 void launch_trial_tail_fused(const DeviceGraph& g, const DeviceStructure& st, const DeviceSystem& sys, Scalar lambda, const Scalar* old, hipStream_t s,
-	const LmDevice* decide = nullptr, const DevicePoseFactors* pf = nullptr);
+	const LmDevice* decide = nullptr, const DevicePoseFactors* pf = nullptr, int publish = 1);
 size_t trial_tail_parts(const DeviceGraph& g, const DeviceStructure& st, int factorParts = 0);
 constexpr int LM_REC = 8, LM_RING = 64;
 struct LmDevice { double* state = nullptr; Scalar* lam = nullptr; double* ring = nullptr; };
+void launch_lm_run_init(const Scalar* chiSlots, const unsigned long long* maxdiag, const LmDevice& lm, double tau, double tagBase, int maxq, hipStream_t s);
 void launch_lm_decide_failed(const DeviceSystem& sys, const LmDevice& lm, hipStream_t s);
 void launch_restore_if_rejected(Scalar* state, const Scalar* backup, size_t count, const LmDevice& lm, hipStream_t s);
 void launch_landmark_scale(const DeviceGraph& g, const DeviceSystem& sys, Scalar lambda, Scalar* slots, hipStream_t s);
diff --git a/cuda-bundle-adjustment_amd/csrc/ba_linearize.hip b/cuda-bundle-adjustment_amd/csrc/ba_linearize.hip
--- a/cuda-bundle-adjustment_amd/csrc/ba_linearize.hip
+++ b/cuda-bundle-adjustment_amd/csrc/ba_linearize.hip
@@ -36,15 +36,20 @@
 
 template <int MODE, typename ET>
 __device__ __forceinline__ void lm_pass_body(const DeviceGraph& g, const DeviceStructure& st, const DeviceSystem& sys, Scalar lambda,
-	unsigned nLmGroups, const Scalar* __restrict__ backupSrc, Scalar* __restrict__ backupDst, size_t backupCount, unsigned gridX)
+	unsigned nLmGroups, Scalar* backupSrc, Scalar* backupDst, size_t backupCount, unsigned gridX, const double* restoreFlag)
 {
 	__shared__ Scalar lds_all[(LIN_BLOCK / WAVE) * WAVE * 9];
+	const bool restore = restoreFlag != nullptr && restoreFlag[0] == 0.0;
 	if (blockIdx.x >= nLmGroups)
 	{
 		const size_t stride = (size_t)(gridX - nLmGroups) * LIN_BLOCK;
-		for (size_t i = (size_t)(blockIdx.x - nLmGroups) * LIN_BLOCK + threadIdx.x; i < backupCount; i += stride) backupDst[i] = backupSrc[i];
+		if (restore) for (size_t i = (size_t)(blockIdx.x - nLmGroups) * LIN_BLOCK + threadIdx.x; i < backupCount; i += stride) backupSrc[i] = backupDst[i];
+		else for (size_t i = (size_t)(blockIdx.x - nLmGroups) * LIN_BLOCK + threadIdx.x; i < backupCount; i += stride) backupDst[i] = backupSrc[i];
 		return;
 	}
+	const Scalar* __restrict__ sq = restore ? backupDst : g.q;
+	const Scalar* __restrict__ stt = restore ? backupDst + 4 * (size_t)g.Pt : g.t;
+	const Scalar* __restrict__ sX = restore ? backupDst + 7 * (size_t)g.Pt : g.Xw;
 	lambda = launch_lambda(sys, lambda);
 	const int lane = threadIdx.x & 63;
 	const int wv = threadIdx.x >> 6;
@@ -65,9 +70,14 @@
 		il = g.e_lm[e];
 		Scalar q[4], t[3], cam[5], Xw[3], meas[3], Xc[3];
 		EdgeLin L;
-		load_pose(g, ip, q, t, cam);
-#pragma unroll
-		for (int i = 0; i < 3; i++) Xw[i] = g.Xw[3 * (size_t)il + i];
+#pragma unroll
+		for (int i = 0; i < 4; i++) q[i] = sq[4 * (size_t)ip + i];
+#pragma unroll
+		for (int i = 0; i < 3; i++) t[i] = stt[3 * (size_t)ip + i];
+#pragma unroll
+		for (int i = 0; i < 5; i++) cam[i] = g.cam[5 * (size_t)ip + i];
+#pragma unroll
+		for (int i = 0; i < 3; i++) Xw[i] = sX[3 * (size_t)il + i];
 		meas[0] = g.e_mu[e]; meas[1] = g.e_mv[e]; meas[2] = g.e_mr[e];
 		const Scalar w = g.e_w[e];
 		const Scalar ss = edge_residual(q, t, cam, Xw, meas, stereo, L.r, Xc);
@@ -137,9 +147,9 @@
 
 template <int MODE, typename ET>
 __global__ __launch_bounds__(LIN_BLOCK) void lm_pass_kernel(DeviceGraph g, DeviceStructure st, DeviceSystem sys, Scalar lambda,
-	unsigned nLmGroups, const Scalar* __restrict__ backupSrc, Scalar* __restrict__ backupDst, size_t backupCount)
-{
-	lm_pass_body<MODE, ET>(g, st, sys, lambda, nLmGroups, backupSrc, backupDst, backupCount, gridDim.x);
+	unsigned nLmGroups, Scalar* __restrict__ backupSrc, Scalar* __restrict__ backupDst, size_t backupCount, const double* restoreFlag)
+{
+	lm_pass_body<MODE, ET>(g, st, sys, lambda, nLmGroups, backupSrc, backupDst, backupCount, gridDim.x, restoreFlag);
 }
 
 template <typename ET>
@@ -147,7 +157,7 @@
 {
 	const BatchEntry& e = tab[blockIdx.y];
 	if (blockIdx.x >= e.t.lmGrid) return;
-	lm_pass_body<1, ET>(e.g, e.st, e.sys, Scalar(-1), e.t.lmGroups, e.t.backupSrc, e.t.backupDst, e.t.backupCount, e.t.lmGrid);
+	lm_pass_body<1, ET>(e.g, e.st, e.sys, Scalar(-1), e.t.lmGroups, const_cast<Scalar*>(e.t.backupSrc), e.t.backupDst, e.t.backupCount, e.t.lmGrid, nullptr);
 }
 
 template <int MODE, typename ET>
@@ -502,15 +512,15 @@
 
 template <typename ET>
 static void launch_linearize_dm_t(const DeviceGraph& g, const DeviceStructure& stAll, const DeviceSystem& sys, int mode, Scalar lambda, hipStream_t s,
-	const Scalar* backupSrc, Scalar* backupDst, size_t backupCount, const BlockPassRange* range)
+	Scalar* backupSrc, Scalar* backupDst, size_t backupCount, const BlockPassRange* range, const double* restoreFlag)
 {
 	const DeviceStructure st = range ? block_pass_view(stAll, *range) : stAll;
 	if (st.nWaves > 0)
 	{
 		const unsigned grid = (st.nWaves + (LIN_BLOCK / WAVE) - 1) / (LIN_BLOCK / WAVE);
 		const unsigned nCopy = backupSrc ? (unsigned)std::min<size_t>(512, (backupCount + LIN_BLOCK - 1) / LIN_BLOCK) : 0;
-		if (mode == 0) hipLaunchKernelGGL((lm_pass_kernel<0, ET>), dim3(grid + nCopy), dim3(LIN_BLOCK), 0, s, g, st, sys, lambda, grid, backupSrc, backupDst, backupCount);
-		else hipLaunchKernelGGL((lm_pass_kernel<1, ET>), dim3(grid + nCopy), dim3(LIN_BLOCK), 0, s, g, st, sys, lambda, grid, backupSrc, backupDst, backupCount);
+		if (mode == 0) hipLaunchKernelGGL((lm_pass_kernel<0, ET>), dim3(grid + nCopy), dim3(LIN_BLOCK), 0, s, g, st, sys, lambda, grid, backupSrc, backupDst, backupCount, nCopy ? restoreFlag : nullptr);
+		else hipLaunchKernelGGL((lm_pass_kernel<1, ET>), dim3(grid + nCopy), dim3(LIN_BLOCK), 0, s, g, st, sys, lambda, grid, backupSrc, backupDst, backupCount, nCopy ? restoreFlag : nullptr);
 	}
 	else if (backupSrc && backupCount)
 		(void)hipMemcpyAsync(backupDst, backupSrc, backupCount * sizeof(Scalar), hipMemcpyDeviceToDevice, s);
@@ -536,10 +546,10 @@
 }
 
 void launch_linearize_dm(const DeviceGraph& g, const DeviceStructure& st, const DeviceSystem& sys, int mode, Scalar lambda, hipStream_t s,
-	const Scalar* backupSrc, Scalar* backupDst, size_t backupCount, const BlockPassRange* range)
-{
-	if (st.mixed && sizeof(Scalar) == 8) launch_linearize_dm_t<float>(g, st, sys, mode, lambda, s, backupSrc, backupDst, backupCount, range);
-	else launch_linearize_dm_t<Scalar>(g, st, sys, mode, lambda, s, backupSrc, backupDst, backupCount, range);
+	Scalar* backupSrc, Scalar* backupDst, size_t backupCount, const BlockPassRange* range, const double* restoreFlag)
+{
+	if (st.mixed && sizeof(Scalar) == 8) launch_linearize_dm_t<float>(g, st, sys, mode, lambda, s, backupSrc, backupDst, backupCount, range, restoreFlag);
+	else launch_linearize_dm_t<Scalar>(g, st, sys, mode, lambda, s, backupSrc, backupDst, backupCount, range, restoreFlag);
 }
 
 void batch_fill_linearize(const DeviceGraph& g, const DeviceStructure& st, const Scalar* backupSrc, Scalar* backupDst, size_t backupCount, BatchTrial& t)
diff --git a/cuda-bundle-adjustment_amd/csrc/ba_lm.hip b/cuda-bundle-adjustment_amd/csrc/ba_lm.hip
--- a/cuda-bundle-adjustment_amd/csrc/ba_lm.hip
+++ b/cuda-bundle-adjustment_amd/csrc/ba_lm.hip
@@ -143,7 +143,8 @@
 {
 	waitAssembled();
 	const bool parts = mode == 1 && !redParts.empty();
-	launch_linearize_dm(g, st, sys, mode, lam, stream, withBackup ? d_state.data() : nullptr, d_backup.data(), d_state.size(), parts ? &redParts[0].od : nullptr);
+	launch_linearize_dm(g, st, sys, mode, lam, stream, withBackup ? d_state.data() : nullptr, d_backup.data(), d_state.size(), parts ? &redParts[0].od : nullptr,
+		withBackup ? lmRestoreFlag : nullptr);
 	if (parts && !partsByCaller)
 		for (size_t c = 1; c < redParts.size(); c++) launch_block_pass(g, st, sys, redParts[c].od, stream);
 	if (poseFactors()) launch_pose_factor_linearize(g, st, sys, pf, mode, stream);
@@ -411,21 +412,8 @@
 					sc.deferCoarse->push_back(CoarseJob{ this, first, firstInvPending, !deferred });
 					if (firstInvPending) { firstInvPending = false; firstInvValid = true; }
 				}
-				else
-				{
-					HIP_TRY(hipStreamWaitEvent(gjStream, evSetup, 0));
-					(void)launch_coarse_setup(g, st, sys, d_coarse[first].data(), d_coarse[1 - first].data(), gjStream, evAssembled);
-					if (fp32Inverse()) launch_coarse_to_fp32(d_coarse[0].data(), d_coarse32[1].data(), 6 * sys.cl * sys.nc, gjStream);
-					else launch_coarse_finish(d_coarse[0].data(), d_coarse[0].data(), 6 * sys.cl * sys.nc, gjStream);
-					if (firstInvPending)
-					{
-						if (fp32Inverse()) HIP_TRY(hipMemcpyAsync(d_firstInv32.data(), d_coarse32[1].data(), inv32Count() * sizeof(float), hipMemcpyDeviceToDevice, gjStream));
-						else HIP_TRY(hipMemcpyAsync(d_firstInv.data(), d_coarse[0].data(), invBytes, hipMemcpyDeviceToDevice, gjStream));
-						HIP_TRY(hipEventRecord(evFirstInv, gjStream));
-						firstInvPending = false; firstInvValid = true;
-					}
-					HIP_TRY(hipEventRecord(evInverse, gjStream));
-				}
+				else if (sc.sideLater) sc.sideFirst = first;
+				else enqueueCoarseSide(first);
 				pendingInv = 0;
 				assemblePending = true; cntCoarseRefresh++;
 			}
@@ -458,6 +446,23 @@
 	return false;
 }
 
+void cuba_hip_solver::enqueueCoarseSide(int first)
+{
+	const size_t invBytes = sizeof(Scalar) * (size_t)36 * sys.cl * sys.cl * sys.nc * sys.nc;
+	HIP_TRY(hipStreamWaitEvent(gjStream, evSetup, 0));
+	(void)launch_coarse_setup(g, st, sys, d_coarse[first].data(), d_coarse[1 - first].data(), gjStream, evAssembled);
+	if (fp32Inverse()) launch_coarse_to_fp32(d_coarse[0].data(), d_coarse32[1].data(), 6 * sys.cl * sys.nc, gjStream);
+	else launch_coarse_finish(d_coarse[0].data(), d_coarse[0].data(), 6 * sys.cl * sys.nc, gjStream);
+	if (firstInvPending)
+	{
+		if (fp32Inverse()) HIP_TRY(hipMemcpyAsync(d_firstInv32.data(), d_coarse32[1].data(), inv32Count() * sizeof(float), hipMemcpyDeviceToDevice, gjStream));
+		else HIP_TRY(hipMemcpyAsync(d_firstInv.data(), d_coarse[0].data(), invBytes, hipMemcpyDeviceToDevice, gjStream));
+		HIP_TRY(hipEventRecord(evFirstInv, gjStream));
+		firstInvPending = false; firstInvValid = true;
+	}
+	HIP_TRY(hipEventRecord(evInverse, gjStream));
+}
+
 bool cuba_hip_solver::solveBrokeDown(SolveCtx& sc)
 {
 	lastSolveBrokeDown = true; lastFailCode = sc.hInts[0];
@@ -476,6 +481,7 @@
 {
 	StageTimer tm(this, 6);
 	SolveCtx sc;
+	sc.sideLater = coarseSideLater;
 	if (solveBegin(sc)) return sc.result;
 	const int maxIter = sc.maxIter; const Scalar tol2 = sc.tol2; const bool graphs = sc.graphs; const int predicted = sc.predicted;
 	bool converged = false;
@@ -501,6 +507,7 @@
 				if (graphs) { eagerIters += c; cntPcgPlain += c; }
 			}
 			k0 += c; todo -= c;
+			if (sc.sideFirst >= 0) { enqueueCoarseSide(sc.sideFirst); sc.sideFirst = -1; }
 		}
 		waitReport();
 		if (sc.hInts[0] != 0) return solveBrokeDown(sc);
@@ -575,7 +582,7 @@
 	return a + b;
 }
 
-void cuba_hip_solver::lmRunBegin(LmRun& r, int niter, double* chi2Out)
+void cuba_hip_solver::lmRunBegin(LmRun& r, int niter, double* chi2Out, bool chain)
 {
 	const double tau = 1e-5;
 	if (!h_lmRing)
@@ -587,6 +594,21 @@
 	startRunHistory();
 	r = LmRun();
 	r.niter = niter; r.chi2Out = chi2Out; r.stop = niter <= 0;
+	r.lm.state = d_lmState.data(); r.lm.lam = d_lamS.data(); r.lm.ring = lmRingDev;
+	if (chain && niter > 0)
+	{
+		need();
+		r.chain = true;
+		Scalar* chiSlots = reinterpret_cast<Scalar*>(d_lmState.data() + 16);
+		launch_residual_chi2(g, d_parts.data(), chiSlots, nullptr, stream, poseFactors());
+		zeroReduced(true);
+		d_maxdiag.zero(stream);
+		linearize(0, 0.0);
+		launch_pose_maxdiag(g, st, sys, stream);
+		r.tagBase = 65536.0 * (double)(++lmRunNonce);
+		launch_lm_run_init(chiSlots, d_maxdiag.data(), r.lm, tau, r.tagBase, LmRun::maxq, stream);
+		return;
+	}
 	r.F = computeErrors();
 	r.lam = tau * maxDiagonal();
 	{
@@ -598,7 +620,6 @@
 		HIP_TRY(hipMemcpyAsync(d_lmState.data(), st8, sizeof(double) * 9, hipMemcpyHostToDevice, stream));
 		HIP_TRY(hipMemcpyAsync(d_lamS.data(), l1, sizeof(Scalar), hipMemcpyHostToDevice, stream));
 	}
-	r.lm.state = d_lmState.data(); r.lm.lam = d_lamS.data(); r.lm.ring = lmRingDev;
 }
 
 void cuba_hip_solver::lmAbsorb(LmRun& r, int upto)
@@ -651,10 +672,13 @@
 bool cuba_hip_solver::lmAfterSolve(LmRun& r, bool ok)
 {
 	if (!lmAfterSolveHost(r)) return false;
-	if (ok) launch_trial_tail_fused(g, st, sys, (Scalar)-1, d_backup.data(), stream, &r.lm, poseFactors());
+	const bool waited = !r.chain || !(r.done + 1 < r.niter && r.rejRun + 1 < LmRun::maxq);
+	const bool publish = waited || !ok;
+	if (ok) launch_trial_tail_fused(g, st, sys, (Scalar)-1, d_backup.data(), stream, &r.lm, poseFactors(), publish ? 1 : 0);
 	else launch_lm_decide_failed(sys, r.lm, stream);
-	noteReport();
-	launch_restore_if_rejected(d_state.data(), d_backup.data(), d_state.size(), r.lm, stream);
+	if (publish) noteReport();
+	r.restoreInPass = !publish && st.nWaves > 0;
+	if (!r.restoreInPass) launch_restore_if_rejected(d_state.data(), d_backup.data(), d_state.size(), r.lm, stream);
 	r.enq++;
 	(void)hipStreamQuery(stream);
 	return true;
@@ -670,11 +694,16 @@
 int cuba_hip_solver::optimizeDeviceDecision(int niter, double* chi2Out)
 {
 	LmRun r;
-	lmRunBegin(r, niter, chi2Out);
+	lmRunBegin(r, niter, chi2Out, true);
 	while (lmBeforeTrial(r))
 	{
-		schur(true);
-		const bool ok = solveReduced();
+		lmRestoreFlag = r.restoreInPass ? r.lm.state + 5 : nullptr;
+		try { schur(true); } catch (...) { lmRestoreFlag = nullptr; throw; }
+		lmRestoreFlag = nullptr;
+		coarseSideLater = true;
+		bool ok = false;
+		try { ok = solveReduced(); } catch (...) { coarseSideLater = false; throw; }
+		coarseSideLater = false;
 		if (!lmAfterSolve(r, ok)) break;
 	}
 	return lmRunEnd(r);
diff --git a/cuda-bundle-adjustment_amd/csrc/ba_setup.hip b/cuda-bundle-adjustment_amd/csrc/ba_setup.hip
--- a/cuda-bundle-adjustment_amd/csrc/ba_setup.hip
+++ b/cuda-bundle-adjustment_amd/csrc/ba_setup.hip
@@ -685,7 +685,7 @@
 	d_qpart.resize(agg > 0 ? (size_t)(agg / spmvRows) * 6 * cl * nc : 1); d_gjPivots.resize(2 * 32 * 32); sys.gj_pivots = d_gjPivots.data();
 	sys.qpart = d_qpart.data();
 	d_qpart.zero(stream);
-	d_lamS.resize(1); d_lmState.resize(16); sys.lam_dev = d_lamS.data();
+	d_lamS.resize(1); d_lmState.resize(32); sys.lam_dev = d_lamS.data();
 	sys.upper = agg > 0 && agg <= pcg_rows_max_aggregate() && (spmvUpper < 0 ? spmvRows == 4 : spmvUpper != 0) ? 1 : 0;
 	if (sys.upper)
 	{
diff --git a/cuda-bundle-adjustment_amd/csrc/ba_solver.hpp b/cuda-bundle-adjustment_amd/csrc/ba_solver.hpp
--- a/cuda-bundle-adjustment_amd/csrc/ba_solver.hpp
+++ b/cuda-bundle-adjustment_amd/csrc/ba_solver.hpp
@@ -559,11 +559,15 @@
 		std::vector<CoarseJob>* deferCoarse = nullptr;
 		bool deferLaunch = false;
 		bool deferred = false;
+		bool sideLater = false;
+		int sideFirst = -1;
 		const Scalar* copySrc = nullptr; Scalar* copyDst = nullptr; size_t copyCount = 0;
 		volatile int* hInts = nullptr;
 		Clock::time_point tSolve0;
 	};
 	bool solveBegin(SolveCtx& sc);
+	void enqueueCoarseSide(int first);
+	bool coarseSideLater = false;
 	bool solveBrokeDown(SolveCtx& sc);
 	bool solveEnd(SolveCtx& sc);
 	bool solveReducedOnce();
@@ -587,11 +591,14 @@
 		static constexpr int maxq = 10;
 		int niter = 0, enq = 0, seen = 0, done = 0, rejRun = 0;
 		bool stop = false;
+		bool chain = false;
+		bool restoreInPass = false;
 		double lam = 0, F = 0, tagBase = 0;
 		double* chi2Out = nullptr;
 		LmDevice lm;
 	};
-	void lmRunBegin(LmRun& r, int niter, double* chi2Out);
+	void lmRunBegin(LmRun& r, int niter, double* chi2Out, bool chain = false);
+	const double* lmRestoreFlag = nullptr;
 	void lmAbsorb(LmRun& r, int upto);
 	bool lmBeforeTrial(LmRun& r);
 	bool lmAfterSolveHost(LmRun& r);
```
